# diff7/tts-king

Measured on AMD Instinct MI355X. Metric: FS2 train mel-frames/sec/GPU + HiFi-GAN RTF (22.05 kHz), batch=16, higher is better.
Workload: dtype bf16

## Files before the change

tts_king_amd/csrc/batchnorm.hip:

```cpp
#include "common.h"

namespace {

struct BnCommon {
  const void* x;
  const float* mean;
  const float* rstd;
  const float* gamma;
  const float* beta;
  const uint64_t* rng;
  int rows, C, use_tanh;
  float p;
  unsigned site;
  int x_f32;
  const int* frame_limit;
  int seg_len;
  uint8_t* keep;
  const long long* lens;
};
__device__ __forceinline__ float tanh_fast(float x) { return 1.f - 2.f * __frcp_rn(__expf(2.f * x) + 1.f); }
__device__ __forceinline__ bool bn_live(const int* frame_limit, int seg_len, int r) {
  return !frame_limit || (r % seg_len) < frame_limit[0];
}
__device__ __forceinline__ int bn_rows(const int* frame_limit, int seg_len, int rows) {
  return frame_limit ? (rows / seg_len) * frame_limit[0] : rows;
}

__device__ __forceinline__ void ld4(const bf16_t* p, float v[4]) {
  const uint2 u = *(const uint2*)p;
  v[0] = __uint_as_float(u.x << 16); v[1] = __uint_as_float(u.x & 0xFFFF0000u);
  v[2] = __uint_as_float(u.y << 16); v[3] = __uint_as_float(u.y & 0xFFFF0000u);
}
__device__ __forceinline__ void ldx4(const void* x, int x_f32, int64_t off, float v[4]) {
  if (x_f32) {
    const f32x4 t = *(const f32x4*)((const float*)x + off);
    v[0] = t[0]; v[1] = t[1]; v[2] = t[2]; v[3] = t[3];
  } else {
    ld4((const bf16_t*)x + off, v);
  }
}
__device__ __forceinline__ uint4 bits4(const uint64_t* rng, unsigned site, unsigned e4) {
  const uint64_t seed = rng[0], step = rng[1];
  return Philox::gen(make_uint2((unsigned)seed, (unsigned)(seed >> 32)), make_uint4(e4, site, (unsigned)step, (unsigned)(step >> 32)));
}

__global__ __launch_bounds__(256) void bn_stats_kernel(const void* __restrict__ x, int x_f32, int rows, int C, float* __restrict__ partials,
                                                       const int* __restrict__ frame_limit, int seg_len) {
  extern __shared__ float red[];
  const int tpr = C >> 2, rpi = 256 / tpr;
  const int r0 = threadIdx.x / tpr, c4 = (threadIdx.x % tpr) * 4;
  const int per = (rows + gridDim.x - 1) / gridDim.x;
  const int rb = blockIdx.x * per;
  const int re = min(rb + per, rows);
  float s[4] = {0, 0, 0, 0}, q[4] = {0, 0, 0, 0};
  if (r0 < rpi)
    for (int r = rb + r0; r < re; r += rpi) {
      if (!bn_live(frame_limit, seg_len, r)) continue;
      float v[4];
      ldx4(x, x_f32, (int64_t)r * C + c4, v);
#pragma unroll
      for (int e = 0; e < 4; ++e) { s[e] += v[e]; q[e] += v[e] * v[e]; }
    }
  if (r0 < rpi) {
#pragma unroll
    for (int e = 0; e < 4; ++e) { red[r0 * C + c4 + e] = s[e]; red[rpi * C + r0 * C + c4 + e] = q[e]; }
  }
  __syncthreads();
  for (int c = threadIdx.x; c < C; c += 256) {
    float a = 0.f, b = 0.f;
    for (int k = 0; k < rpi; ++k) { a += red[k * C + c]; b += red[rpi * C + k * C + c]; }
    partials[(int64_t)blockIdx.x * 2 * C + c] = a;
    partials[(int64_t)blockIdx.x * 2 * C + C + c] = b;
  }
}

__global__ __launch_bounds__(256) void bn_finalize_kernel(const float* __restrict__ partials, int nblk, int C, int rows_all, float eps,
                                                          float momentum, float* __restrict__ mean, float* __restrict__ rstd,
                                                          float* __restrict__ run_mean, float* __restrict__ run_var,
                                                          long long* __restrict__ nbt, const int* __restrict__ frame_limit, int seg_len) {
  const int rows = bn_rows(frame_limit, seg_len, rows_all);
  __shared__ double rs[16][17], rq[16][17];
  const int cx = threadIdx.x & 15, gy = threadIdx.x >> 4;
  const int c = blockIdx.x * 16 + cx;
  if (blockIdx.x == 0 && threadIdx.x == 0 && nbt) nbt[0] += 1;
  double s = 0.0, q = 0.0;
  if (c < C) {
    double s1 = 0.0, q1 = 0.0, s2 = 0.0, q2 = 0.0, s3 = 0.0, q3 = 0.0;
    int b = gy;
    for (; b + 48 < nblk; b += 64) {
      const float a0 = partials[(int64_t)b * 2 * C + c], b0 = partials[(int64_t)b * 2 * C + C + c];
      const float a1 = partials[(int64_t)(b + 16) * 2 * C + c], b1 = partials[(int64_t)(b + 16) * 2 * C + C + c];
      const float a2 = partials[(int64_t)(b + 32) * 2 * C + c], b2 = partials[(int64_t)(b + 32) * 2 * C + C + c];
      const float a3 = partials[(int64_t)(b + 48) * 2 * C + c], b3 = partials[(int64_t)(b + 48) * 2 * C + C + c];
      s += a0; q += b0; s1 += a1; q1 += b1; s2 += a2; q2 += b2; s3 += a3; q3 += b3;
    }
    for (; b < nblk; b += 16) { s += partials[(int64_t)b * 2 * C + c]; q += partials[(int64_t)b * 2 * C + C + c]; }
    s = (s + s1) + (s2 + s3);
    q = (q + q1) + (q2 + q3);
  }
  rs[gy][cx] = s;
  rq[gy][cx] = q;
  __syncthreads();
  if (gy != 0 || c >= C) return;
  s = 0.0; q = 0.0;
#pragma unroll
  for (int k = 0; k < 16; ++k) { s += rs[k][cx]; q += rq[k][cx]; }
  const double m = s / rows;
  double var = q / rows - m * m;
  if (var < 0.0) var = 0.0;
  mean[c] = (float)m;
  rstd[c] = (float)(1.0 / sqrt(var + (double)eps));
  if (run_mean) {
    run_mean[c] = (1.f - momentum) * run_mean[c] + momentum * (float)m;
    run_var[c] = (1.f - momentum) * run_var[c] + momentum * (float)(var * rows / (rows > 1 ? rows - 1 : 1));
  }
}

__global__ __launch_bounds__(256) void rsqrt_eps_kernel(const float* __restrict__ var, float eps, float* __restrict__ rstd, int n) {
  const int i = blockIdx.x * 256 + threadIdx.x;
  if (i < n) rstd[i] = 1.f / sqrtf(var[i] + eps);
}

template <bool LENS>
__global__ __launch_bounds__(256) void bn_apply_kernel(const BnCommon a, const float* __restrict__ resid, bf16_t* __restrict__ out16,
                                                       float* __restrict__ out32) {
  const int tpr = a.C >> 2;
  const int64_t n = (int64_t)a.rows * tpr;
  const unsigned thr = keep_threshold(a.p);
  const float scale = a.p > 0.f ? 1.f / (1.f - a.p) : 1.f;
  for (int64_t i = blockIdx.x * 256 + threadIdx.x; i < n; i += (int64_t)gridDim.x * 256) {
    const int r = (int)(i / tpr), c4 = (int)(i - (int64_t)r * tpr) * 4;
    bool live = bn_live(a.frame_limit, a.seg_len, r);
    if (LENS) {
      const int u = r / a.seg_len;
      const long long len = a.lens[u];
      live = live && (r - u * a.seg_len) < (len < 0 ? 0 : (len > a.seg_len ? (long long)a.seg_len : len));
    }
    if (!live) {
      if (out16) *(uint2*)(out16 + (int64_t)r * a.C + c4) = make_uint2(0u, 0u);
      if (out32) *(f32x4*)(out32 + (int64_t)r * a.C + c4) = f32x4{0.f, 0.f, 0.f, 0.f};
      continue;
    }
    float v[4];
    ldx4(a.x, a.x_f32, (int64_t)r * a.C + c4, v);
    const f32x4 m = *(const f32x4*)(a.mean + c4), rs = *(const f32x4*)(a.rstd + c4);
    const f32x4 g = *(const f32x4*)(a.gamma + c4), b = *(const f32x4*)(a.beta + c4);
#pragma unroll
    for (int e = 0; e < 4; ++e) {
      v[e] = (v[e] - m[e]) * rs[e] * g[e] + b[e];
      if (a.use_tanh) v[e] = tanh_fast(v[e]);
    }
    if (a.p > 0.f) {
      const uint4 bb = bits4(a.rng, a.site, (unsigned)i);
      v[0] = bb.x >= thr ? v[0] * scale : 0.f; v[1] = bb.y >= thr ? v[1] * scale : 0.f;
      v[2] = bb.z >= thr ? v[2] * scale : 0.f; v[3] = bb.w >= thr ? v[3] * scale : 0.f;
    }
    if (resid) {
      const f32x4 rr = *(const f32x4*)(resid + (int64_t)r * a.C + c4);
#pragma unroll
      for (int e = 0; e < 4; ++e) v[e] += rr[e];
    }
    if (out16) *(uint2*)(out16 + (int64_t)r * a.C + c4) = make_uint2(pack_bf2(v[0], v[1]), pack_bf2(v[2], v[3]));
    if (out32) *(f32x4*)(out32 + (int64_t)r * a.C + c4) = f32x4{v[0], v[1], v[2], v[3]};
  }
}

__device__ __forceinline__ void bn_dy(const BnCommon& a, const void* dout, int dout_f32, int r, int c4, int64_t i, unsigned thr,
                                      float scale, float xh[4], float dy[4]) {
  float v[4];
  ldx4(a.x, a.x_f32, (int64_t)r * a.C + c4, v);
  const f32x4 m = *(const f32x4*)(a.mean + c4), rs = *(const f32x4*)(a.rstd + c4);
  if (dout_f32) {
    const f32x4 d = *(const f32x4*)((const float*)dout + (int64_t)r * a.C + c4);
    dy[0] = d[0]; dy[1] = d[1]; dy[2] = d[2]; dy[3] = d[3];
  } else {
    ld4((const bf16_t*)dout + (int64_t)r * a.C + c4, dy);
  }
  if (a.p > 0.f) {
    if (a.keep) {
      const unsigned kb = a.keep[i];
#pragma unroll
      for (int e = 0; e < 4; ++e) dy[e] = ((kb >> e) & 1u) ? dy[e] * scale : 0.f;
    } else {
      const uint4 bb = bits4(a.rng, a.site, (unsigned)i);
      dy[0] = bb.x >= thr ? dy[0] * scale : 0.f; dy[1] = bb.y >= thr ? dy[1] * scale : 0.f;
      dy[2] = bb.z >= thr ? dy[2] * scale : 0.f; dy[3] = bb.w >= thr ? dy[3] * scale : 0.f;
    }
  }
#pragma unroll
  for (int e = 0; e < 4; ++e) xh[e] = (v[e] - m[e]) * rs[e];
  if (a.use_tanh) {
    const f32x4 g = *(const f32x4*)(a.gamma + c4), b = *(const f32x4*)(a.beta + c4);
#pragma unroll
    for (int e = 0; e < 4; ++e) { const float t = tanh_fast(xh[e] * g[e] + b[e]); dy[e] *= 1.f - t * t; }
  }
  if (!bn_live(a.frame_limit, a.seg_len, r)) {
#pragma unroll
    for (int e = 0; e < 4; ++e) { xh[e] = 0.f; dy[e] = 0.f; }
  }
}

__global__ __launch_bounds__(256) void bn_bwd_stats_kernel(const BnCommon a, const void* __restrict__ dout, int dout_f32,
                                                           float* __restrict__ partials) {
  extern __shared__ float red[];
  const int C = a.C, tpr = C >> 2, rpi = 256 / tpr;
  const int r0 = threadIdx.x / tpr, c4 = (threadIdx.x % tpr) * 4;
  const int per = (a.rows + gridDim.x - 1) / gridDim.x;
  const int rb = blockIdx.x * per;
  const int re = min(rb + per, a.rows);
  const unsigned thr = keep_threshold(a.p);
  const float scale = a.p > 0.f ? 1.f / (1.f - a.p) : 1.f;
  float s[4] = {0, 0, 0, 0}, q[4] = {0, 0, 0, 0};
  if (r0 < rpi)
    for (int r = rb + r0; r < re; r += rpi) {
      float xh[4], dy[4];
      bn_dy(a, dout, dout_f32, r, c4, (int64_t)r * tpr + (c4 >> 2), thr, scale, xh, dy);
#pragma unroll
      for (int e = 0; e < 4; ++e) { s[e] += dy[e]; q[e] += dy[e] * xh[e]; }
    }
  if (r0 < rpi) {
#pragma unroll
    for (int e = 0; e < 4; ++e) { red[r0 * C + c4 + e] = s[e]; red[rpi * C + r0 * C + c4 + e] = q[e]; }
  }
  __syncthreads();
  for (int c = threadIdx.x; c < C; c += 256) {
    float x1 = 0.f, x2 = 0.f;
    for (int k = 0; k < rpi; ++k) { x1 += red[k * C + c]; x2 += red[rpi * C + k * C + c]; }
    partials[(int64_t)blockIdx.x * 2 * C + c] = x1;
    partials[(int64_t)blockIdx.x * 2 * C + C + c] = x2;
  }
}

__global__ __launch_bounds__(256) void bn_bwd_apply_kernel(const BnCommon a, const void* __restrict__ dout, int dout_f32,
                                                           const float* __restrict__ sums, bf16_t* __restrict__ dx,
                                                           float* __restrict__ dgamma, float* __restrict__ dbeta, int accumulate) {
  const int tpr = a.C >> 2;
  const int64_t n = (int64_t)a.rows * tpr;
  const unsigned thr = keep_threshold(a.p);
  const float scale = a.p > 0.f ? 1.f / (1.f - a.p) : 1.f;
  const float inv_n = 1.f / bn_rows(a.frame_limit, a.seg_len, a.rows);
  if (blockIdx.x == 0 && dgamma)
    for (int c = threadIdx.x; c < a.C; c += 256) {
      dbeta[c] = accumulate ? dbeta[c] + sums[c] : sums[c];
      dgamma[c] = accumulate ? dgamma[c] + sums[a.C + c] : sums[a.C + c];
    }
  for (int64_t i = blockIdx.x * 256 + threadIdx.x; i < n; i += (int64_t)gridDim.x * 256) {
    const int r = (int)(i / tpr), c4 = (int)(i - (int64_t)r * tpr) * 4;
    float xh[4], dy[4];
    bn_dy(a, dout, dout_f32, r, c4, i, thr, scale, xh, dy);
    const f32x4 g = *(const f32x4*)(a.gamma + c4), rs = *(const f32x4*)(a.rstd + c4);
    const f32x4 s1 = *(const f32x4*)(sums + c4), s2 = *(const f32x4*)(sums + a.C + c4);
    float o[4];
#pragma unroll
    for (int e = 0; e < 4; ++e) o[e] = g[e] * rs[e] * (dy[e] - s1[e] * inv_n - xh[e] * s2[e] * inv_n);
    if (!bn_live(a.frame_limit, a.seg_len, r)) o[0] = o[1] = o[2] = o[3] = 0.f;
    *(uint2*)(dx + (int64_t)r * a.C + c4) = make_uint2(pack_bf2(o[0], o[1]), pack_bf2(o[2], o[3]));
  }
}


constexpr int BN_MAX_CHUNKS = 64;
__host__ __device__ inline int bn_slab(int C) { return (C % 64 == 0) ? 64 : C; }

struct BnSlab {
  int c0, slab, tpr, rpi, r_in, cq, rb, re;
  __device__ BnSlab(int C, int rows) {
    slab = bn_slab(C);
    c0 = blockIdx.x * slab;
    tpr = slab >> 2;
    rpi = 256 / tpr;
    r_in = threadIdx.x / tpr;
    cq = threadIdx.x % tpr;
    const int per = (rows + gridDim.y - 1) / gridDim.y;
    rb = blockIdx.y * per;
    re = min(rb + per, rows);
  }
};

__device__ __forceinline__ void bn_slab_store(const BnSlab& g, int C, const float s[4], const float q[4], float* red, float* partials) {
  if (g.r_in < g.rpi) {
#pragma unroll
    for (int e = 0; e < 4; ++e) { red[g.r_in * g.slab + g.cq * 4 + e] = s[e]; red[(g.rpi + g.r_in) * g.slab + g.cq * 4 + e] = q[e]; }
  }
  __syncthreads();
  for (int v = threadIdx.x; v < 2 * g.slab; v += 256) {
    const int half = v >= g.slab, c = v - half * g.slab;
    float acc = 0.f;
    for (int k = 0; k < g.rpi; ++k) acc += red[(half * g.rpi + k) * g.slab + c];
    partials[(int64_t)blockIdx.y * 2 * C + half * C + g.c0 + c] = acc;
  }
}

constexpr int BN_TOT = 256 + 1024;
__device__ __forceinline__ void bn_slab_totals(const float* __restrict__ partials, int nblk, int C, int c0, int slab, double* tot ) {
  const int nq = slab >> 1, groups = 256 / nq;
  const int t = threadIdx.x;
  if (t < groups * nq) {
    const int q = t % nq, g0 = t / nq;
    const int v0 = q * 4;
    const int col = v0 < slab ? c0 + v0 : C + c0 + (v0 - slab);
    double a[4] = {0.0, 0.0, 0.0, 0.0};
    for (int b = g0; b < nblk; b += 16 * groups) {
      f32x4 f[16];
#pragma unroll
      for (int u = 0; u < 16; ++u) {
        const int bb = b + u * groups;
        f[u] = *(const f32x4*)(partials + (int64_t)min(bb, nblk - 1) * 2 * C + col);
        if (bb >= nblk) f[u] = f32x4{0.f, 0.f, 0.f, 0.f};
      }
#pragma unroll
      for (int u = 0; u < 16; ++u)
#pragma unroll
        for (int e = 0; e < 4; ++e) a[e] += f[u][e];
    }
#pragma unroll
    for (int e = 0; e < 4; ++e) tot[256 + t * 4 + e] = a[e];
  }
  __syncthreads();
  if (t < 2 * slab) {
    double sum = 0.0;
    for (int k = 0; k < groups; ++k) sum += tot[256 + (k * nq + (t >> 2)) * 4 + (t & 3)];
    tot[t] = sum;
  }
  __syncthreads();
}

__global__ __launch_bounds__(256) void bn_stats2_kernel(const void* __restrict__ x, int x_f32, int rows, int C, float* __restrict__ partials,
                                                        const int* __restrict__ frame_limit, int seg_len) {
  extern __shared__ float red[];
  const BnSlab g(C, rows);
  const int c4 = g.c0 + g.cq * 4;
  float s[4] = {0, 0, 0, 0}, q[4] = {0, 0, 0, 0};
  if (g.r_in < g.rpi)
    for (int r0 = g.rb + g.r_in; r0 < g.re; r0 += 8 * g.rpi) {
      float v[8][4];
#pragma unroll
      for (int u = 0; u < 8; ++u) {
        const int r = r0 + u * g.rpi, rc = min(r, g.re - 1);
        ldx4(x, x_f32, (int64_t)rc * C + c4, v[u]);
        if (r >= g.re || !bn_live(frame_limit, seg_len, rc)) v[u][0] = v[u][1] = v[u][2] = v[u][3] = 0.f;
      }
#pragma unroll
      for (int u = 0; u < 8; ++u)
#pragma unroll
        for (int e = 0; e < 4; ++e) { s[e] += v[u][e]; q[e] += v[u][e] * v[u][e]; }
    }
  bn_slab_store(g, C, s, q, red, partials);
}

struct BnTrain {
  const float* partials;
  int nblk;
  float eps, momentum;
  float* mean;
  float* rstd;
  float* run_mean;
  float* run_var;
  long long* nbt;
};

template <bool RESID>
__global__ __launch_bounds__(256, RESID ? 3 : 4) void bn_apply2_kernel(const BnCommon a, const BnTrain t, const float* __restrict__ resid,
                                                        bf16_t* __restrict__ out16, float* __restrict__ out32) {
  __shared__ double tot[BN_TOT];
  __shared__ float ms[128], rs[128];
  const BnSlab g(a.C, a.rows);
  const int cl = g.cq * 4, c4 = g.c0 + cl, tprC = a.C >> 2;
  const bool act = g.r_in < g.rpi;
  float v[4][4], rr[RESID ? 4 : 1][4];
  bool live[4];
#pragma unroll
  for (int u = 0; u < 4; ++u) {
    const int r = g.rb + g.r_in + u * g.rpi, rc = max(min(r, g.re - 1), 0);
    live[u] = act && r < g.re && bn_live(a.frame_limit, a.seg_len, r);
    if (act) {
      ldx4(a.x, a.x_f32, (int64_t)rc * a.C + c4, v[u]);
      if constexpr (RESID) { const f32x4 q = *(const f32x4*)(resid + (int64_t)rc * a.C + c4); rr[u][0] = q[0]; rr[u][1] = q[1]; rr[u][2] = q[2]; rr[u][3] = q[3]; }
    }
  }
  f32x4 gm = f32x4{0.f, 0.f, 0.f, 0.f}, bt = gm;
  if (act) { gm = *(const f32x4*)(a.gamma + c4); bt = *(const f32x4*)(a.beta + c4); }
  bn_slab_totals(t.partials, t.nblk, a.C, g.c0, g.slab, tot);
  if ((int)threadIdx.x < g.slab) {
    const int c = threadIdx.x;
    const int n = bn_rows(a.frame_limit, a.seg_len, a.rows);
    const double m = tot[c] / n;
    double var = tot[g.slab + c] / n - m * m;
    if (var < 0.0) var = 0.0;
    ms[c] = (float)m;
    rs[c] = (float)(1.0 / sqrt(var + (double)t.eps));
    if (blockIdx.y == 0) {
      t.mean[g.c0 + c] = ms[c];
      t.rstd[g.c0 + c] = rs[c];
      if (t.run_mean) {
        t.run_mean[g.c0 + c] = (1.f - t.momentum) * t.run_mean[g.c0 + c] + t.momentum * (float)m;
        t.run_var[g.c0 + c] = (1.f - t.momentum) * t.run_var[g.c0 + c] + t.momentum * (float)(var * n / (n > 1 ? n - 1 : 1));
      }
      if (blockIdx.x == 0 && c == 0 && t.nbt) t.nbt[0] += 1;
    }
  }
  __syncthreads();
  if (!act) return;
  const unsigned thr = keep_threshold(a.p);
  const float scale = a.p > 0.f ? 1.f / (1.f - a.p) : 1.f;
#pragma unroll
  for (int u = 0; u < 4; ++u) {
    const int r = g.rb + g.r_in + u * g.rpi;
    if (r >= g.re) break;
    const int64_t i = (int64_t)r * tprC + (c4 >> 2);
    if (!live[u]) {
      if (out16) *(uint2*)(out16 + (int64_t)r * a.C + c4) = make_uint2(0u, 0u);
      if (out32) *(f32x4*)(out32 + (int64_t)r * a.C + c4) = f32x4{0.f, 0.f, 0.f, 0.f};
      if (a.keep) a.keep[i] = 0;
      continue;
    }
#pragma unroll
    for (int e = 0; e < 4; ++e) {
      v[u][e] = (v[u][e] - ms[cl + e]) * rs[cl + e] * gm[e] + bt[e];
      if (a.use_tanh) v[u][e] = tanh_fast(v[u][e]);
    }
    if (a.p > 0.f) {
      const uint4 bb = bits4(a.rng, a.site, (unsigned)i);
      const bool k0 = bb.x >= thr, k1 = bb.y >= thr, k2 = bb.z >= thr, k3 = bb.w >= thr;
      v[u][0] = k0 ? v[u][0] * scale : 0.f; v[u][1] = k1 ? v[u][1] * scale : 0.f;
      v[u][2] = k2 ? v[u][2] * scale : 0.f; v[u][3] = k3 ? v[u][3] * scale : 0.f;
      if (a.keep) a.keep[i] = (uint8_t)((int)k0 | ((int)k1 << 1) | ((int)k2 << 2) | ((int)k3 << 3));
    }
    if constexpr (RESID) {
#pragma unroll
      for (int e = 0; e < 4; ++e) v[u][e] += rr[u][e];
    }
    if (out16) *(uint2*)(out16 + (int64_t)r * a.C + c4) = make_uint2(pack_bf2(v[u][0], v[u][1]), pack_bf2(v[u][2], v[u][3]));
    if (out32) *(f32x4*)(out32 + (int64_t)r * a.C + c4) = f32x4{v[u][0], v[u][1], v[u][2], v[u][3]};
  }
}

__global__ __launch_bounds__(256) void bn_bwd_stats2_kernel(const BnCommon a, const void* __restrict__ dout, int dout_f32,
                                                            float* __restrict__ partials) {
  extern __shared__ float red[];
  const BnSlab g(a.C, a.rows);
  const int c4 = g.c0 + g.cq * 4, tprC = a.C >> 2;
  const unsigned thr = keep_threshold(a.p);
  const float scale = a.p > 0.f ? 1.f / (1.f - a.p) : 1.f;
  float s[4] = {0, 0, 0, 0}, q[4] = {0, 0, 0, 0};
  if (g.r_in < g.rpi)
    for (int r0 = g.rb + g.r_in; r0 < g.re; r0 += 8 * g.rpi) {
      float xh[8][4], dy[8][4];
#pragma unroll
      for (int u = 0; u < 8; ++u) {
        const int r = r0 + u * g.rpi, rc = min(r, g.re - 1);
        bn_dy(a, dout, dout_f32, rc, c4, (int64_t)rc * tprC + (c4 >> 2), thr, scale, xh[u], dy[u]);
        if (r >= g.re) { xh[u][0] = xh[u][1] = xh[u][2] = xh[u][3] = 0.f; dy[u][0] = dy[u][1] = dy[u][2] = dy[u][3] = 0.f; }
      }
#pragma unroll
      for (int u = 0; u < 8; ++u)
#pragma unroll
        for (int e = 0; e < 4; ++e) { s[e] += dy[u][e]; q[e] += dy[u][e] * xh[u][e]; }
    }
  bn_slab_store(g, a.C, s, q, red, partials);
}

__global__ __launch_bounds__(256, 4) void bn_bwd_apply2_kernel(const BnCommon a, const void* __restrict__ dout, int dout_f32,
                                                            const float* __restrict__ partials, int nblk, bf16_t* __restrict__ dx,
                                                            float* __restrict__ dgamma, float* __restrict__ dbeta, int accumulate) {
  __shared__ double tot[BN_TOT];
  __shared__ float s1s[128], s2s[128];
  const BnSlab g(a.C, a.rows);
  const int cl = g.cq * 4, c4 = g.c0 + cl, tprC = a.C >> 2;
  const bool act = g.r_in < g.rpi;
  const unsigned thr = keep_threshold(a.p);
  const float scale = a.p > 0.f ? 1.f / (1.f - a.p) : 1.f;
  float xh[4][4], dy[4][4];
#pragma unroll
  for (int u = 0; u < 4; ++u) {
    const int rc = max(min(g.rb + g.r_in + u * g.rpi, g.re - 1), 0);
    if (act) bn_dy(a, dout, dout_f32, rc, c4, (int64_t)rc * tprC + (c4 >> 2), thr, scale, xh[u], dy[u]);
  }
  bn_slab_totals(partials, nblk, a.C, g.c0, g.slab, tot);
  if ((int)threadIdx.x < g.slab) {
    const int c = threadIdx.x;
    s1s[c] = (float)tot[c];
    s2s[c] = (float)tot[g.slab + c];
    if (blockIdx.y == 0 && dgamma) {
      dbeta[g.c0 + c] = accumulate ? dbeta[g.c0 + c] + s1s[c] : s1s[c];
      dgamma[g.c0 + c] = accumulate ? dgamma[g.c0 + c] + s2s[c] : s2s[c];
    }
  }
  __syncthreads();
  if (!act) return;
  const float inv_n = 1.f / bn_rows(a.frame_limit, a.seg_len, a.rows);
  const f32x4 gm = *(const f32x4*)(a.gamma + c4), rsd = *(const f32x4*)(a.rstd + c4);
#pragma unroll
  for (int u = 0; u < 4; ++u) {
    const int r = g.rb + g.r_in + u * g.rpi;
    if (r >= g.re) break;
    float o[4];
#pragma unroll
    for (int e = 0; e < 4; ++e) o[e] = gm[e] * rsd[e] * (dy[u][e] - s1s[cl + e] * inv_n - xh[u][e] * s2s[cl + e] * inv_n);
    if (!bn_live(a.frame_limit, a.seg_len, r)) o[0] = o[1] = o[2] = o[3] = 0.f;
    *(uint2*)(dx + (int64_t)r * a.C + c4) = make_uint2(pack_bf2(o[0], o[1]), pack_bf2(o[2], o[3]));
  }
}

inline int bn_chunks(int rows) { int n = (rows + 15) / 16; return n > BN_MAX_CHUNKS ? BN_MAX_CHUNKS : (n < 1 ? 1 : n); }
inline int bn_apply_chunks(int rows, int C) { const int rpi = 256 / (bn_slab(C) >> 2); int n = (rows + 4 * rpi - 1) / (4 * rpi); return n < 1 ? 1 : n; }

inline int bn_blocks(int rows) { int n = (rows + 15) / 16; return n > 1024 ? 1024 : (n < 1 ? 1 : n); }

}

extern "C" int ttsk_bn_nblocks(int rows) { return bn_blocks(rows); }

static int bn_check(int rows, int C) {
  TTSK_REQUIRE(rows > 0 && C >= 4 && C <= 1024 && (C & 3) == 0, "batchnorm: C must be a multiple of 4, <= 1024 (got %d)", C);
  return 0;
}

static int limit_check(const int32_t* frame_limit, int seg_len, int rows) {
  TTSK_REQUIRE(!frame_limit || (seg_len > 0 && rows % seg_len == 0), "batchnorm: frame_limit needs rows %% seg_len == 0");
  return 0;
}

extern "C" int ttsk_bn_stats(const void* x, int x_is_f32, int rows, int C, float* partials, const int32_t* frame_limit, int seg_len,
                             void* stream) {
  TTSK_REQUIRE(x && partials, "bn_stats: null pointer");
  if (int rc = limit_check(frame_limit, seg_len, rows)) return rc;
  if (int rc = bn_check(rows, C)) return rc;
  const int rpi = 256 / (C >> 2);
  hipLaunchKernelGGL(bn_stats_kernel, dim3(bn_blocks(rows)), dim3(256), 2 * rpi * C * sizeof(float), (hipStream_t)stream,
                     x, x_is_f32, rows, C, partials, frame_limit, seg_len > 0 ? seg_len : 1);
  TTSK_CHECK_LAUNCH();
  return TTSK_OK;
}

extern "C" int ttsk_bn_finalize(const float* partials, int nblk, int C, int rows, float eps, float momentum, float* mean,
                                float* rstd, float* running_mean, float* running_var, int64_t* num_batches_tracked,
                                const int32_t* frame_limit, int seg_len, void* stream) {
  if (int rc = limit_check(frame_limit, seg_len, rows)) return rc;
  TTSK_REQUIRE(partials && mean && rstd && nblk > 0, "bn_finalize: null pointer");
  TTSK_REQUIRE((running_mean == nullptr) == (running_var == nullptr), "bn_finalize: running stats come in pairs");
  hipLaunchKernelGGL(bn_finalize_kernel, dim3((C + 15) / 16), dim3(256), 0, (hipStream_t)stream, partials, nblk, C, rows, eps,
                     momentum, mean, rstd, running_mean, running_var, (long long*)num_batches_tracked, frame_limit, seg_len > 0 ? seg_len : 1);
  TTSK_CHECK_LAUNCH();
  return TTSK_OK;
}

extern "C" int ttsk_rsqrt_eps(const float* var, float eps, float* rstd, int n, void* stream) {
  TTSK_REQUIRE(var && rstd && n > 0, "rsqrt_eps: bad arguments");
  hipLaunchKernelGGL(rsqrt_eps_kernel, dim3((n + 255) / 256), dim3(256), 0, (hipStream_t)stream, var, eps, rstd, n);
  TTSK_CHECK_LAUNCH();
  return TTSK_OK;
}

extern "C" int ttsk_bn_apply(const void* x, int x_is_f32, const float* mean, const float* rstd, const float* gamma, const float* beta,
                             int rows, int C, int use_tanh, float p, uint32_t site, const uint64_t* rng, const float* resid_f32,
                             void* out_bf16, float* out_f32, const int32_t* frame_limit, int seg_len, void* stream) {
  if (int rc = limit_check(frame_limit, seg_len, rows)) return rc;
  TTSK_REQUIRE(x && mean && rstd && gamma && beta && (out_bf16 || out_f32), "bn_apply: null pointer");
  TTSK_REQUIRE(p == 0.f || rng, "bn_apply: dropout needs rng");
  if (int rc = bn_check(rows, C)) return rc;
  BnCommon a{x, mean, rstd, gamma, beta, rng, rows, C, use_tanh, p, site, x_is_f32, frame_limit, seg_len > 0 ? seg_len : 1};
  int64_t n = (int64_t)rows * (C >> 2);
  int blocks = (int)((n + 255) / 256);
  if (blocks > 4096) blocks = 4096;
  hipLaunchKernelGGL(bn_apply_kernel<false>, dim3(blocks), dim3(256), 0, (hipStream_t)stream, a, resid_f32, (bf16_t*)out_bf16, out_f32);
  TTSK_CHECK_LAUNCH();
  return TTSK_OK;
}

extern "C" int ttsk_bn_apply_lens(const void* x, int x_is_f32, const float* mean, const float* rstd, const float* gamma, const float* beta,
                                  int rows, int C, int use_tanh, const float* resid_f32, void* out_bf16, float* out_f32,
                                  const int64_t* lens, int seg_len, void* stream) {
  TTSK_REQUIRE(x && mean && rstd && gamma && beta && lens && (out_bf16 || out_f32), "bn_apply_lens: null pointer");
  TTSK_REQUIRE(seg_len > 0 && rows % seg_len == 0, "bn_apply_lens: rows %% seg_len != 0");
  if (int rc = bn_check(rows, C)) return rc;
  BnCommon a{x, mean, rstd, gamma, beta, nullptr, rows, C, use_tanh, 0.f, 0u, x_is_f32, nullptr, seg_len, nullptr, (const long long*)lens};
  int64_t n = (int64_t)rows * (C >> 2);
  int blocks = (int)((n + 255) / 256);
  if (blocks > 4096) blocks = 4096;
  hipLaunchKernelGGL(bn_apply_kernel<true>, dim3(blocks), dim3(256), 0, (hipStream_t)stream, a, resid_f32, (bf16_t*)out_bf16, out_f32);
  TTSK_CHECK_LAUNCH();
  return TTSK_OK;
}

extern "C" int ttsk_bn_bwd_stats(const void* dout, int dout_is_f32, const void* x, int x_is_f32, const float* mean, const float* rstd,
                                 const float* gamma, const float* beta, int rows, int C, int use_tanh, float p, uint32_t site,
                                 const uint64_t* rng, float* partials, const int32_t* frame_limit, int seg_len, void* stream) {
  if (int rc = limit_check(frame_limit, seg_len, rows)) return rc;
  TTSK_REQUIRE(dout && x && mean && rstd && gamma && beta && partials, "bn_bwd_stats: null pointer");
  TTSK_REQUIRE(p == 0.f || rng, "bn_bwd_stats: dropout needs rng");
  if (int rc = bn_check(rows, C)) return rc;
  BnCommon a{x, mean, rstd, gamma, beta, rng, rows, C, use_tanh, p, site, x_is_f32, frame_limit, seg_len > 0 ? seg_len : 1};
  const int rpi = 256 / (C >> 2);
  hipLaunchKernelGGL(bn_bwd_stats_kernel, dim3(bn_blocks(rows)), dim3(256), 2 * rpi * C * sizeof(float), (hipStream_t)stream, a,
                     dout, dout_is_f32, partials);
  TTSK_CHECK_LAUNCH();
  return TTSK_OK;
}

extern "C" int ttsk_bn_bwd_apply(const void* dout, int dout_is_f32, const void* x, int x_is_f32, const float* mean, const float* rstd,
                                 const float* gamma, const float* beta, int rows, int C, int use_tanh, float p, uint32_t site,
                                 const uint64_t* rng, const float* sums, void* dx_bf16, float* dgamma, float* dbeta, int accumulate,
                                 const int32_t* frame_limit, int seg_len, void* stream) {
  if (int rc = limit_check(frame_limit, seg_len, rows)) return rc;
  TTSK_REQUIRE(dout && x && mean && rstd && gamma && beta && sums && dx_bf16, "bn_bwd_apply: null pointer");
  TTSK_REQUIRE((dgamma == nullptr) == (dbeta == nullptr), "bn_bwd_apply: dgamma/dbeta come in pairs");
  if (int rc = bn_check(rows, C)) return rc;
  BnCommon a{x, mean, rstd, gamma, beta, rng, rows, C, use_tanh, p, site, x_is_f32, frame_limit, seg_len > 0 ? seg_len : 1};
  int64_t n = (int64_t)rows * (C >> 2);
  int blocks = (int)((n + 255) / 256);
  if (blocks > 4096) blocks = 4096;
  hipLaunchKernelGGL(bn_bwd_apply_kernel, dim3(blocks), dim3(256), 0, (hipStream_t)stream, a, dout, dout_is_f32, sums,
                     (bf16_t*)dx_bf16, dgamma, dbeta, accumulate);
  TTSK_CHECK_LAUNCH();
  return TTSK_OK;
}

static int bn2_check(int rows, int C) {
  if (int rc = bn_check(rows, C)) return rc;
  TTSK_REQUIRE(C % 64 == 0 || C <= 128, "batchnorm (slab path): C must be a multiple of 64 or <= 128 (got %d)", C);
  return 0;
}

extern "C" int ttsk_bn_nchunks(int rows) { return bn_chunks(rows); }

extern "C" int ttsk_bn_stats_slab(const void* x, int x_is_f32, int rows, int C, float* partials, const int32_t* frame_limit, int seg_len,
                                  void* stream) {
  TTSK_REQUIRE(x && partials, "bn_stats_slab: null pointer");
  if (int rc = limit_check(frame_limit, seg_len, rows)) return rc;
  if (int rc = bn2_check(rows, C)) return rc;
  const int slab = bn_slab(C), rpi = 256 / (slab >> 2);
  hipLaunchKernelGGL(bn_stats2_kernel, dim3(C / slab, bn_chunks(rows)), dim3(256), 2 * rpi * slab * sizeof(float), (hipStream_t)stream,
                     x, x_is_f32, rows, C, partials, frame_limit, seg_len > 0 ? seg_len : 1);
  TTSK_CHECK_LAUNCH();
  return TTSK_OK;
}

extern "C" int ttsk_bn_train_apply(const void* x, int x_is_f32, const float* partials, int nblk, float eps, float momentum, float* mean,
                                   float* rstd, float* running_mean, float* running_var, int64_t* num_batches_tracked,
                                   const float* gamma, const float* beta, int rows, int C, int use_tanh, float p, uint32_t site,
                                   const uint64_t* rng, const float* resid_f32, void* out_bf16, float* out_f32, uint8_t* keep_out,
                                   const int32_t* frame_limit, int seg_len, void* stream) {
  if (int rc = limit_check(frame_limit, seg_len, rows)) return rc;
  TTSK_REQUIRE(x && partials && nblk > 0 && mean && rstd && gamma && beta && (out_bf16 || out_f32), "bn_train_apply: null pointer");
  TTSK_REQUIRE((running_mean == nullptr) == (running_var == nullptr), "bn_train_apply: running stats come in pairs");
  TTSK_REQUIRE(p == 0.f || rng, "bn_train_apply: dropout needs rng");
  if (int rc = bn2_check(rows, C)) return rc;
  BnCommon a{x, nullptr, nullptr, gamma, beta, rng, rows, C, use_tanh, p, site, x_is_f32, frame_limit, seg_len > 0 ? seg_len : 1, keep_out};
  BnTrain t{partials, nblk, eps, momentum, mean, rstd, running_mean, running_var, (long long*)num_batches_tracked};
  const dim3 grid(C / bn_slab(C), bn_apply_chunks(rows, C));
  if (resid_f32) hipLaunchKernelGGL(bn_apply2_kernel<true>, grid, dim3(256), 0, (hipStream_t)stream, a, t, resid_f32, (bf16_t*)out_bf16, out_f32);
  else hipLaunchKernelGGL(bn_apply2_kernel<false>, grid, dim3(256), 0, (hipStream_t)stream, a, t, resid_f32, (bf16_t*)out_bf16, out_f32);
  TTSK_CHECK_LAUNCH();
  return TTSK_OK;
}

extern "C" int ttsk_bn_bwd_stats_slab(const void* dout, int dout_is_f32, const void* x, int x_is_f32, const float* mean, const float* rstd,
                                      const float* gamma, const float* beta, int rows, int C, int use_tanh, float p, uint32_t site,
                                      const uint64_t* rng, const uint8_t* keep, float* partials, const int32_t* frame_limit, int seg_len,
                                      void* stream) {
  if (int rc = limit_check(frame_limit, seg_len, rows)) return rc;
  TTSK_REQUIRE(dout && x && mean && rstd && gamma && beta && partials, "bn_bwd_stats_slab: null pointer");
  TTSK_REQUIRE(p == 0.f || rng || keep, "bn_bwd_stats_slab: dropout needs rng or the forward's keep bits");
  if (int rc = bn2_check(rows, C)) return rc;
  BnCommon a{x, mean, rstd, gamma, beta, rng, rows, C, use_tanh, p, site, x_is_f32, frame_limit, seg_len > 0 ? seg_len : 1, (uint8_t*)keep};
  const int slab = bn_slab(C), rpi = 256 / (slab >> 2);
  hipLaunchKernelGGL(bn_bwd_stats2_kernel, dim3(C / slab, bn_chunks(rows)), dim3(256), 2 * rpi * slab * sizeof(float), (hipStream_t)stream,
                     a, dout, dout_is_f32, partials);
  TTSK_CHECK_LAUNCH();
  return TTSK_OK;
}

extern "C" int ttsk_bn_bwd_apply_slab(const void* dout, int dout_is_f32, const void* x, int x_is_f32, const float* mean, const float* rstd,
                                      const float* gamma, const float* beta, int rows, int C, int use_tanh, float p, uint32_t site,
                                      const uint64_t* rng, const uint8_t* keep, const float* partials, int nblk, void* dx_bf16, float* dgamma,
                                      float* dbeta, int accumulate, const int32_t* frame_limit, int seg_len, void* stream) {
  if (int rc = limit_check(frame_limit, seg_len, rows)) return rc;
  TTSK_REQUIRE(dout && x && mean && rstd && gamma && beta && partials && nblk > 0 && dx_bf16, "bn_bwd_apply_slab: null pointer");
  TTSK_REQUIRE((dgamma == nullptr) == (dbeta == nullptr), "bn_bwd_apply_slab: dgamma/dbeta come in pairs");
  TTSK_REQUIRE(p == 0.f || rng || keep, "bn_bwd_apply_slab: dropout needs rng or the forward's keep bits");
  if (int rc = bn2_check(rows, C)) return rc;
  BnCommon a{x, mean, rstd, gamma, beta, rng, rows, C, use_tanh, p, site, x_is_f32, frame_limit, seg_len > 0 ? seg_len : 1, (uint8_t*)keep};
  hipLaunchKernelGGL(bn_bwd_apply2_kernel, dim3(C / bn_slab(C), bn_apply_chunks(rows, C)), dim3(256), 0, (hipStream_t)stream, a, dout,
                     dout_is_f32, partials, nblk, (bf16_t*)dx_bf16, dgamma, dbeta, accumulate);
  TTSK_CHECK_LAUNCH();
  return TTSK_OK;
}
```

tts_king_amd/csrc/common.h:

```cpp
#pragma once
#include <hip/hip_runtime.h>
#include <stdint.h>
#include <stdio.h>
#include <stdarg.h>
#include "../../include/ttsk.h"

typedef unsigned short bf16_t;
typedef __attribute__((ext_vector_type(8))) short bf16x8;
typedef __attribute__((ext_vector_type(4))) short bf16x4;
typedef __attribute__((ext_vector_type(4))) float f32x4;

__device__ __forceinline__ float bf2f(bf16_t v) { return __uint_as_float(((unsigned)v) << 16); }
__device__ __forceinline__ bf16_t f2bf(float f) {
  __bf16 b = (__bf16)f;
  return *reinterpret_cast<bf16_t*>(&b);
}
__device__ __forceinline__ unsigned pack_bf2(float a, float b) {
  return (unsigned)f2bf(a) | ((unsigned)f2bf(b) << 16);
}
template <int CTRL>
__device__ __forceinline__ float dpp_f32(float v) {
  return __builtin_bit_cast(float, __builtin_amdgcn_update_dpp(0, __builtin_bit_cast(int, v), CTRL, 0xF, 0xF, true));
}
__device__ __forceinline__ float quad16_max(float v) {
  v = fmaxf(v, dpp_f32<0xB1>(v));
  v = fmaxf(v, dpp_f32<0x4E>(v));
  v = fmaxf(v, dpp_f32<0x141>(v));
  v = fmaxf(v, dpp_f32<0x140>(v));
  return v;
}
__device__ __forceinline__ float quad16_sum(float v) {
  v += dpp_f32<0xB1>(v);
  v += dpp_f32<0x4E>(v);
  v += dpp_f32<0x141>(v);
  v += dpp_f32<0x140>(v);
  return v;
}

__device__ __forceinline__ float wave_sum(float v) {
  v = quad16_sum(v);
  v += __shfl_xor(v, 16, 64);
  v += __shfl_xor(v, 32, 64);
  return v;
}
__device__ __forceinline__ float wave_max(float v) {
  v = quad16_max(v);
  v = fmaxf(v, __shfl_xor(v, 16, 64));
  v = fmaxf(v, __shfl_xor(v, 32, 64));
  return v;
}

typedef _Float16 half8 __attribute__((ext_vector_type(8)));
typedef _Float16 half2v __attribute__((ext_vector_type(2)));
template <bool F16> __device__ __forceinline__ void unpack2(unsigned w, float& lo, float& hi) {
  if constexpr (F16) {
    const half2v h = __builtin_bit_cast(half2v, w);
    lo = (float)h[0]; hi = (float)h[1];
  } else {
    lo = __uint_as_float(w << 16); hi = __uint_as_float(w & 0xFFFF0000u);
  }
}
template <bool F16> __device__ __forceinline__ unsigned pack2(float lo, float hi) {
  if constexpr (F16) {
    half2v h; h[0] = (_Float16)lo; h[1] = (_Float16)hi;
    return __builtin_bit_cast(unsigned, h);
  } else {
    return pack_bf2(lo, hi);
  }
}
template <bool F16> __device__ __forceinline__ float unpack1(bf16_t v) {
  if constexpr (F16) return (float)__builtin_bit_cast(_Float16, v);
  else return bf2f(v);
}
template <bool F16> __device__ __forceinline__ bf16_t pack1(float f) {
  if constexpr (F16) return __builtin_bit_cast(bf16_t, (_Float16)f);
  else return f2bf(f);
}
template <bool F16> __device__ __forceinline__ unsigned lrelu2(unsigned w, float sl) {
  float lo, hi;
  unpack2<F16>(w, lo, hi);
  lo = lo > 0.f ? lo : lo * sl;
  hi = hi > 0.f ? hi : hi * sl;
  return pack2<F16>(lo, hi);
}
template <bool F16> __device__ __forceinline__ uint4 lrelu8(uint4 v, float sl) {
  return make_uint4(lrelu2<F16>(v.x, sl), lrelu2<F16>(v.y, sl), lrelu2<F16>(v.z, sl), lrelu2<F16>(v.w, sl));
}
template <bool F16> __device__ __forceinline__ unsigned lrelu2_fast(unsigned w, float sl) {
  if constexpr (F16) {
    float lo, hi;
    asm("v_fma_mix_f32 %0, %1, %2, 0 op_sel_hi:[1,0,0]" : "=v"(lo) : "v"(w), "v"(sl));
    asm("v_fma_mix_f32 %0, %1, %2, 0 op_sel:[1,0,0] op_sel_hi:[1,0,0]" : "=v"(hi) : "v"(w), "v"(sl));
    const unsigned p = pack2<true>(lo, hi);
    unsigned r;
    asm("v_pk_max_f16 %0, %1, %2" : "=v"(r) : "v"(w), "v"(p));
    return r;
  } else {
    return lrelu2<false>(w, sl);
  }
}

template <bool F16> __device__ __forceinline__ uint4 lrelu8_fast(uint4 v, float sl) {
  return make_uint4(lrelu2_fast<F16>(v.x, sl), lrelu2_fast<F16>(v.y, sl), lrelu2_fast<F16>(v.z, sl), lrelu2_fast<F16>(v.w, sl));
}
template <bool F16> __device__ __forceinline__ f32x4 mfma16(bf16x8 a, bf16x8 b, f32x4 c) {
  if constexpr (F16) return __builtin_amdgcn_mfma_f32_16x16x32_f16(__builtin_bit_cast(half8, a), __builtin_bit_cast(half8, b), c, 0, 0, 0);
  else return __builtin_amdgcn_mfma_f32_16x16x32_bf16(a, b, c, 0, 0, 0);
}

struct Philox {
  __device__ static __forceinline__ uint4 gen(uint2 key, uint4 ctr) {
#pragma unroll
    for (int r = 0; r < 10; ++r) {
      unsigned hi0 = __umulhi(0xD2511F53u, ctr.x), lo0 = 0xD2511F53u * ctr.x;
      unsigned hi1 = __umulhi(0xCD9E8D57u, ctr.z), lo1 = 0xCD9E8D57u * ctr.z;
      ctr = make_uint4(hi1 ^ ctr.y ^ key.x, lo1, hi0 ^ ctr.w ^ key.y, lo0);
      key.x += 0x9E3779B9u;
      key.y += 0xBB67AE85u;
    }
    return ctr;
  }
};
__device__ __forceinline__ uint4 dropout_bits(uint64_t seed, unsigned site, unsigned e4) {
  return Philox::gen(make_uint2((unsigned)seed, (unsigned)(seed >> 32)), make_uint4(e4, site, 0x5eedu, 0u));
}
__device__ __forceinline__ unsigned keep_threshold(float p) {
  double t = (double)p * 4294967296.0;
  return t >= 4294967295.0 ? 0xFFFFFFFFu : (unsigned)t;
}

void ttsk_set_error(const char* fmt, ...);
#define TTSK_REQUIRE(cond, ...)                 \
  do {                                          \
    if (!(cond)) {                              \
      ttsk_set_error(__VA_ARGS__);              \
      return TTSK_EINVAL;                       \
    }                                           \
  } while (0)
#define TTSK_CHECK_LAUNCH()                                                    \
  do {                                                                         \
    hipError_t e__ = hipGetLastError();                                        \
    if (e__ != hipSuccess) {                                                   \
      ttsk_set_error("%s: launch failed: %s", __func__, hipGetErrorString(e__)); \
      return TTSK_ELAUNCH;                                                     \
    }                                                                          \
  } while (0)
```

tts_king_amd/csrc/cwt.hip:

```cpp
#include "common.h"
#include <math.h>

namespace {

constexpr int NH = TTSK_CWT_CHANNELS;
constexpr int NBIN = TTSK_CNNSCALAR_BINS;
constexpr int O_W1 = 0, O_B1 = 256, O_G1 = 264, O_BE1 = 296, O_W2 = 328, O_B2 = 344, O_G2 = 352, O_BE2 = 384, O_LW = 416, O_LB = 448;
static_assert(O_LB + 8 == TTSK_CNNSCALAR_FLOATS, "CNNscalar block layout");

__device__ __forceinline__ void load4(const bf16_t* p, float v[4]) {
  const uint2 u = *(const uint2*)p;
  v[0] = __uint_as_float(u.x << 16); v[1] = __uint_as_float(u.x & 0xFFFF0000u);
  v[2] = __uint_as_float(u.y << 16); v[3] = __uint_as_float(u.y & 0xFFFF0000u);
}
__device__ __forceinline__ void store4(bf16_t* p, const float v[4]) {
  *(uint2*)p = make_uint2(pack_bf2(v[0], v[1]), pack_bf2(v[2], v[3]));
}
__device__ __forceinline__ void drop4(float v[4], uint64_t seed, uint64_t step, unsigned site, unsigned e4, unsigned thr, float scale) {
  const uint4 b = Philox::gen(make_uint2((unsigned)seed, (unsigned)(seed >> 32)),
                              make_uint4(e4, site, (unsigned)step, (unsigned)(step >> 32)));
  v[0] = b.x >= thr ? v[0] * scale : 0.f;
  v[1] = b.y >= thr ? v[1] * scale : 0.f;
  v[2] = b.z >= thr ? v[2] * scale : 0.f;
  v[3] = b.w >= thr ? v[3] * scale : 0.f;
}

struct HeadArgs {
  const bf16_t* y;
  const float* gamma; const float* beta;
  const long long* lens;
  const uint64_t* rng;
  const float* head_w;
  const float* head_b;
  float* mean; float* rstd;
  float* head_out;
  int rows, seg_len;
  float p_post, eps;
  unsigned site_post;
};

__global__ __launch_bounds__(256) void ln_head_fwd_kernel(const HeadArgs a) {
  const int lane = threadIdx.x & 63;
  const int row = blockIdx.x * 4 + (threadIdx.x >> 6);
  if (row >= a.rows) return;
  constexpr int D = 256;
  const uint64_t seed = a.rng ? a.rng[0] : 0, step = a.rng ? a.rng[1] : 0;
  const int c = lane * 4;
  float z[4];
  load4(a.y + (int64_t)row * D + c, z);
  const float mean = wave_sum(z[0] + z[1] + z[2] + z[3]) / D;
  float q = 0.f;
#pragma unroll
  for (int e = 0; e < 4; ++e) { const float d = z[e] - mean; q += d * d; }
  const float rstd = rsqrtf(wave_sum(q) / D + a.eps);
  if (lane == 0) { a.mean[row] = mean; a.rstd[row] = rstd; }
  const int b = row / a.seg_len, t = row - b * a.seg_len;
  const bool masked = t >= a.lens[b];
  const f32x4 g = *(const f32x4*)(a.gamma + c), bt = *(const f32x4*)(a.beta + c);
  float o[4];
#pragma unroll
  for (int e = 0; e < 4; ++e) o[e] = (z[e] - mean) * rstd * g[e] + bt[e];
  if (a.p_post > 0.f)
    drop4(o, seed, step, a.site_post, (unsigned)(((int64_t)row * D + c) >> 2), keep_threshold(a.p_post), 1.f / (1.f - a.p_post));
#pragma unroll
  for (int k = 0; k < NH; ++k) {
    const f32x4 w = *(const f32x4*)(a.head_w + k * D + c);
    const float hs = wave_sum(o[0] * w[0] + o[1] * w[1] + o[2] * w[2] + o[3] * w[3]);
    if (lane == 0) a.head_out[(int64_t)row * NH + k] = masked ? 0.f : hs + a.head_b[k];
  }
}

struct HeadBwdArgs {
  const float* dhead;
  const float* head_w;
  const bf16_t* z;
  const float* mean; const float* rstd;
  const float* gamma; const float* beta;
  const long long* lens;
  const uint64_t* rng;
  bf16_t* dz;
  float* partials;
  int rows, seg_len;
  float p_post;
  unsigned site_post;
};

constexpr int HB_WAVES = 4;
constexpr int HB_NCOL = (3 + NH) * 256 + NH;

__global__ __launch_bounds__(HB_WAVES * 64) void ln_head_bwd_kernel(const HeadBwdArgs a) {
  __shared__ float red[HB_WAVES][256];
  __shared__ float redb[HB_WAVES][NH];
  constexpr int D = 256;
  const int lane = threadIdx.x & 63, wave = threadIdx.x >> 6;
  const uint64_t seed = a.rng ? a.rng[0] : 0, step = a.rng ? a.rng[1] : 0;
  const int c = lane * 4;
  float dg[4] = {0, 0, 0, 0}, db[4] = {0, 0, 0, 0}, dbias[4] = {0, 0, 0, 0};
  float dhw[NH][4];
  float dhb[NH];
#pragma unroll
  for (int k = 0; k < NH; ++k) { dhb[k] = 0.f; dhw[k][0] = dhw[k][1] = dhw[k][2] = dhw[k][3] = 0.f; }
  const f32x4 gm = *(const f32x4*)(a.gamma + c), bt = *(const f32x4*)(a.beta + c);
  for (int row = blockIdx.x * HB_WAVES + wave; row < a.rows; row += gridDim.x * HB_WAVES) {
    const int b = row / a.seg_len, t = row - b * a.seg_len;
    const bool masked = t >= a.lens[b];
    const float mean = a.mean[row], rstd = a.rstd[row];
    float zz[4];
    load4(a.z + (int64_t)row * D + c, zz);
    float xh[4], o[4], d[4] = {0, 0, 0, 0};
#pragma unroll
    for (int e = 0; e < 4; ++e) { xh[e] = (zz[e] - mean) * rstd; o[e] = xh[e] * gm[e] + bt[e]; }
    if (a.p_post > 0.f)
      drop4(o, seed, step, a.site_post, (unsigned)(((int64_t)row * D + c) >> 2), keep_threshold(a.p_post), 1.f / (1.f - a.p_post));
#pragma unroll
    for (int k = 0; k < NH; ++k) {
      const float dh = masked ? 0.f : a.dhead[(int64_t)row * NH + k];
      const f32x4 w = *(const f32x4*)(a.head_w + k * D + c);
#pragma unroll
      for (int e = 0; e < 4; ++e) { d[e] += dh * w[e]; dhw[k][e] += dh * o[e]; }
      dhb[k] += dh;
    }
    if (a.p_post > 0.f)
      drop4(d, seed, step, a.site_post, (unsigned)(((int64_t)row * D + c) >> 2), keep_threshold(a.p_post), 1.f / (1.f - a.p_post));
    float g[4], c1 = 0.f, c2 = 0.f;
#pragma unroll
    for (int e = 0; e < 4; ++e) {
      dg[e] += d[e] * xh[e];
      db[e] += d[e];
      g[e] = d[e] * gm[e];
      c1 += g[e];
      c2 += g[e] * xh[e];
    }
    c1 = wave_sum(c1) / D;
    c2 = wave_sum(c2) / D;
    float dzv[4];
#pragma unroll
    for (int e = 0; e < 4; ++e) {
      dzv[e] = zz[e] > 0.f ? rstd * (g[e] - c1 - xh[e] * c2) : 0.f;
      dbias[e] += dzv[e];
    }
    store4(a.dz + (int64_t)row * D + c, dzv);
  }
  float* P = a.partials + (int64_t)blockIdx.x * HB_NCOL;
  for (int qn = 0; qn < 3 + NH; ++qn) {
#pragma unroll
    for (int e = 0; e < 4; ++e) {
      float v;
      if (qn == 0) v = dbias[e];
      else if (qn == 1) v = dg[e];
      else if (qn == 2) v = db[e];
      else {
        v = 0.f;
#pragma unroll
        for (int k = 0; k < NH; ++k) if (qn == 3 + k) v = dhw[k][e];
      }
      red[wave][c + e] = v;
    }
    __syncthreads();
    {
      const int cc = threadIdx.x;
      float t = 0.f;
#pragma unroll
      for (int w = 0; w < HB_WAVES; ++w) t += red[w][cc];
      P[qn * D + cc] = t;
    }
    __syncthreads();
  }
  if (lane == 0) {
#pragma unroll
    for (int k = 0; k < NH; ++k) redb[wave][k] = dhb[k];
  }
  __syncthreads();
  if (threadIdx.x < NH) {
    float t = 0.f;
#pragma unroll
    for (int w = 0; w < HB_WAVES; ++w) t += redb[w][threadIdx.x];
    P[(3 + NH) * D + threadIdx.x] = t;
  }
}

__device__ __forceinline__ int bin_start(int i, int L) { return (int)(((int64_t)i * L) / NBIN); }
__device__ __forceinline__ int bin_end(int i, int L) { return (int)((((int64_t)(i + 1)) * L + NBIN - 1) / NBIN); }

struct CnnArgs {
  const bf16_t* x;
  const float* cwt;
  const float* params;
  float* rowdot;
  float* pooled;
  float* stats;
  float* pre;
  float* out;
  const float* dout;
  float* partials;
  int B, L;
};

__global__ __launch_bounds__(256) void cnn_heads_fwd_kernel(const CnnArgs a) {
  __shared__ float sp[4][NBIN];
  const int b = blockIdx.x, L = a.L;
  const int lane = threadIdx.x & 63, wave = threadIdx.x >> 6;
  const float* P0 = a.params;
  const float* P1 = a.params + TTSK_CNNSCALAR_FLOATS;
  float* rd = a.rowdot + (int64_t)b * 4 * L;
  const int c = lane * 4;
  const f32x4 w0 = *(const f32x4*)(P0 + O_W1 + c), w1 = *(const f32x4*)(P1 + O_W1 + c);
  for (int l = wave; l < L; l += 4) {
    float v[4];
    load4(a.x + ((int64_t)b * L + l) * 256 + c, v);
    const float s0 = wave_sum(v[0] * w0[0] + v[1] * w0[1] + v[2] * w0[2] + v[3] * w0[3]);
    const float s1 = wave_sum(v[0] * w1[0] + v[1] * w1[1] + v[2] * w1[2] + v[3] * w1[3]);
    if (lane == 0) { rd[0 * L + l] = s0 + P0[O_B1]; rd[2 * L + l] = s1 + P1[O_B1]; }
  }
  for (int l = threadIdx.x; l < L; l += 256) {
    const float* cr = a.cwt + ((int64_t)b * L + l) * NH;
    float s0 = 0.f, s1 = 0.f;
#pragma unroll
    for (int k = 0; k < NH; ++k) { const float v = cr[k]; s0 += v * P0[O_W2 + k]; s1 += v * P1[O_W2 + k]; }
    rd[1 * L + l] = s0 + P0[O_B2]; rd[3 * L + l] = s1 + P1[O_B2];
  }
  __syncthreads();
  if (threadIdx.x < 4 * NBIN) {
    const int q = threadIdx.x / NBIN, i = threadIdx.x - q * NBIN;
    const int s = bin_start(i, L), e = bin_end(i, L);
    float t = 0.f;
    for (int l = s; l < e; ++l) t += rd[q * L + l];
    t /= (float)(e - s);
    sp[q][i] = t;
    a.pooled[((int64_t)b * 4 + q) * NBIN + i] = t;
  }
  __syncthreads();
  {
    const int q = wave;
    const float* Pq = (q >> 1) ? P1 : P0;
    const int og = (q & 1) ? O_G2 : O_G1, ob = (q & 1) ? O_BE2 : O_BE1;
    const float v = lane < NBIN ? sp[q][lane] : 0.f;
    const float mean = wave_sum(v) / NBIN;
    const float d = lane < NBIN ? v - mean : 0.f;
    const float rstd = rsqrtf(wave_sum(d * d) / NBIN + 1e-5f);
    __syncthreads();
    if (lane < NBIN) sp[q][lane] = fmaxf(d * rstd * Pq[og + lane] + Pq[ob + lane], 0.f);
    if (lane == 0) { a.stats[((int64_t)b * 4 + q) * 2] = mean; a.stats[((int64_t)b * 4 + q) * 2 + 1] = rstd; }
  }
  __syncthreads();
  if (wave < 2) {
    const int h = wave;
    const float* Ph = h ? P1 : P0;
    const float v = lane < NBIN ? (sp[2 * h][lane] + sp[2 * h + 1][lane]) * Ph[O_LW + lane] : 0.f;
    const float pre = wave_sum(v) + Ph[O_LB];
    if (lane == 0) { a.pre[b * 2 + h] = pre; a.out[h * a.B + b] = fmaxf(pre, 0.f); }
  }
}

__global__ __launch_bounds__(256) void cnn_heads_bwd_kernel(const CnnArgs a) {
  __shared__ float dp[4][NBIN];
  __shared__ float red[4][2][256];
  __shared__ float red2[2][NH + 1][4];
  const int b = blockIdx.x, L = a.L;
  const int lane = threadIdx.x & 63, wave = threadIdx.x >> 6;
  const float* P0 = a.params;
  const float* P1 = a.params + TTSK_CNNSCALAR_FLOATS;
  float* part = a.partials + (int64_t)b * 2 * TTSK_CNNSCALAR_FLOATS;
  float* rd = a.rowdot + (int64_t)b * 4 * L;
  for (int i = threadIdx.x; i < 2 * TTSK_CNNSCALAR_FLOATS; i += 256) part[i] = 0.f;
  __syncthreads();
  {
    const int q = wave, h = q >> 1, f = q & 1;
    const float* Ph = h ? P1 : P0;
    float* ph = part + h * TTSK_CNNSCALAR_FLOATS;
    const int og = f ? O_G2 : O_G1, ob = f ? O_BE2 : O_BE1;
    const float pre = a.pre[b * 2 + h];
    const float dpre = pre > 0.f ? a.dout[h * a.B + b] : 0.f;
    const float mean = a.stats[((int64_t)b * 4 + q) * 2], rstd = a.stats[((int64_t)b * 4 + q) * 2 + 1];
    const bool on = lane < NBIN;
    const float p = on ? a.pooled[((int64_t)b * 4 + q) * NBIN + lane] : 0.f;
    const float gam = on ? Ph[og + lane] : 0.f, bet = on ? Ph[ob + lane] : 0.f;
    const float xh = on ? (p - mean) * rstd : 0.f;
    const float y = xh * gam + bet;
    const float dy = (on && y > 0.f) ? dpre * Ph[O_LW + lane] : 0.f;
    const float gx = dy * gam;
    const float c1 = wave_sum(gx) / NBIN, c2 = wave_sum(gx * xh) / NBIN;
    if (on) {
      ph[og + lane] = dy * xh;
      ph[ob + lane] = dy;
      const int cnt = bin_end(lane, L) - bin_start(lane, L);
      dp[q][lane] = rstd * (gx - c1 - xh * c2) / (float)cnt;
    }
    if (f == 0) {
      const int q2 = q + 1;
      const float m2 = a.stats[((int64_t)b * 4 + q2) * 2], r2 = a.stats[((int64_t)b * 4 + q2) * 2 + 1];
      const float p2 = on ? a.pooled[((int64_t)b * 4 + q2) * NBIN + lane] : 0.f;
      const float y2 = on ? (p2 - m2) * r2 * Ph[O_G2 + lane] + Ph[O_BE2 + lane] : 0.f;
      if (on) ph[O_LW + lane] = dpre * (fmaxf(y, 0.f) + fmaxf(y2, 0.f));
      if (lane == 0) ph[O_LB] = dpre;
    }
  }
  __syncthreads();
  for (int l = threadIdx.x; l < L; l += 256) {
    float t[4] = {0.f, 0.f, 0.f, 0.f};
    for (int i = 0; i < NBIN; ++i)
      if (l >= bin_start(i, L) && l < bin_end(i, L)) {
#pragma unroll
        for (int q = 0; q < 4; ++q) t[q] += dp[q][i];
      }
#pragma unroll
    for (int q = 0; q < 4; ++q) rd[q * L + l] = t[q];
  }
  __syncthreads();
  {
    const int c = lane * 4;
    float acc0[4] = {0, 0, 0, 0}, acc1[4] = {0, 0, 0, 0};
    for (int l = wave; l < L; l += 4) {
      float v[4];
      load4(a.x + ((int64_t)b * L + l) * 256 + c, v);
      const float d0 = rd[0 * L + l], d1 = rd[2 * L + l];
#pragma unroll
      for (int e = 0; e < 4; ++e) { acc0[e] += d0 * v[e]; acc1[e] += d1 * v[e]; }
    }
#pragma unroll
    for (int e = 0; e < 4; ++e) { red[wave][0][c + e] = acc0[e]; red[wave][1][c + e] = acc1[e]; }
    if (lane <= NH) {
      float s0 = 0.f, s1 = 0.f, t0 = 0.f, t1 = 0.f;
      for (int l = wave; l < L; l += 4) {
        const float d0 = rd[1 * L + l], d1 = rd[3 * L + l];
        if (lane < NH) {
          const float v = a.cwt[((int64_t)b * L + l) * NH + lane];
          s0 += d0 * v; s1 += d1 * v;
        } else {
          s0 += d0; s1 += d1; t0 += rd[0 * L + l]; t1 += rd[2 * L + l];
        }
      }
      red2[0][lane][wave] = s0; red2[1][lane][wave] = s1;
      if (lane == NH) { dp[0][wave] = t0; dp[1][wave] = t1; }
    }
  }
  __syncthreads();
  {
    const int cc = threadIdx.x;
#pragma unroll
    for (int h = 0; h < 2; ++h)
      part[h * TTSK_CNNSCALAR_FLOATS + O_W1 + cc] = red[0][h][cc] + red[1][h][cc] + red[2][h][cc] + red[3][h][cc];
    if (cc < 2 * (NH + 1)) {
      const int h = cc / (NH + 1), k = cc - h * (NH + 1);
      const float t = red2[h][k][0] + red2[h][k][1] + red2[h][k][2] + red2[h][k][3];
      part[h * TTSK_CNNSCALAR_FLOATS + (k < NH ? O_W2 + k : O_B2)] = t;
    }
    if (cc < 2) part[cc * TTSK_CNNSCALAR_FLOATS + O_B1] = dp[cc][0] + dp[cc][1] + dp[cc][2] + dp[cc][3];
  }
}

struct CwtW { double w[10]; };

__device__ __forceinline__ double cwt_sum(const float* __restrict__ c, const CwtW& w) {
  double s = 0.0;
#pragma unroll
  for (int i = 0; i < 10; ++i) s += (double)c[i] * w.w[i];
  return s;
}

__device__ __forceinline__ void cwt_pitch_row(double s, double m, double sd, int b, int l, const float* __restrict__ heads, const float* __restrict__ bins,
                                              int nb, float p_control, float* __restrict__ pitch, int* __restrict__ idx, int B, int L) {
  const double z = (s - m) / sd;
  const float p = (float)(z * (double)heads[B + b] + (double)heads[b]);
  pitch[(int64_t)b * L + l] = p;
  const float x = p * p_control;
  int lo = 0, hi = nb;
  while (lo < hi) { const int mid = (lo + hi) >> 1; if (bins[mid] < x) lo = mid + 1; else hi = mid; }
  idx[(int64_t)b * L + l] = (x != x) ? nb : lo;
}

constexpr int CP_WAVES = 8, CP_MAXB = 64;
__global__ __launch_bounds__(64 * CP_WAVES) void cwt_pitch_lds_kernel(const float* __restrict__ cwt, const float* __restrict__ heads,
                                                                      const float* __restrict__ bins, int nb, float p_control,
                                                                      float* __restrict__ pitch, int* __restrict__ idx, int B, int L, const CwtW w) {
  __shared__ double sdat[CP_MAXB][64];
  const int lane = threadIdx.x & 63, wave = threadIdx.x >> 6;
  const int l = blockIdx.x * 64 + lane;
  const bool on = l < L;
  for (int b = wave; b < B; b += CP_WAVES) sdat[b][lane] = on ? cwt_sum(cwt + ((int64_t)b * L + l) * NH, w) : 0.0;
  __syncthreads();
  if (!on) return;
  double m = 0.0;
  for (int b = 0; b < B; ++b) m += sdat[b][lane];
  m /= (double)B;
  double v = 0.0;
  for (int b = 0; b < B; ++b) { const double d = sdat[b][lane] - m; v += d * d; }
  const double sd = sqrt(v / (double)B) + 1e-12;
  for (int b = wave; b < B; b += CP_WAVES) cwt_pitch_row(sdat[b][lane], m, sd, b, l, heads, bins, nb, p_control, pitch, idx, B, L);
}

__global__ __launch_bounds__(64) void cwt_pitch_kernel(const float* __restrict__ cwt, const float* __restrict__ heads, const float* __restrict__ bins,
                                                       int nb, float p_control, float* __restrict__ pitch, int* __restrict__ idx, int B, int L,
                                                       const CwtW w) {
  const int l = blockIdx.x * 64 + threadIdx.x;
  if (l >= L) return;
  double m = 0.0;
  for (int b = 0; b < B; ++b) m += cwt_sum(cwt + ((int64_t)b * L + l) * NH, w);
  m /= (double)B;
  double v = 0.0;
  for (int b = 0; b < B; ++b) { const double d = cwt_sum(cwt + ((int64_t)b * L + l) * NH, w) - m; v += d * d; }
  const double sd = sqrt(v / (double)B) + 1e-12;
  for (int b = 0; b < B; ++b)
    cwt_pitch_row(cwt_sum(cwt + ((int64_t)b * L + l) * NH, w), m, sd, b, l, heads, bins, nb, p_control, pitch, idx, B, L);
}

constexpr int CL_WAVES = 16;
__global__ __launch_bounds__(64 * CL_WAVES) void cwt_loss_kernel(const float* __restrict__ cwt, const float* __restrict__ cwt_t,
                                                                 const float* __restrict__ heads, const float* __restrict__ mean_t,
                                                                 const float* __restrict__ std_t, const long long* __restrict__ src_lens, int B, int L,
                                                                 float grad_scale, float* __restrict__ dcwt, float* __restrict__ dheads,
                                                                 float* __restrict__ losses) {
  __shared__ double red[3][CL_WAVES];
  const int lane = threadIdx.x & 63, wave = threadIdx.x >> 6;
  float nv = 0.f;
  for (int b = 0; b < B; ++b) nv += (float)src_lens[b];
  const float gv = grad_scale * 2.f / (nv * NH);
  const float gh = grad_scale * 2.f / (float)B;
  float acc = 0.f, am = 0.f, as = 0.f;
  const int rows = B * L;
  for (int r = threadIdx.x; r < rows; r += 64 * CL_WAVES) {
    const int b = r / L, l = r - b * L;
    const bool ok = l < src_lens[b];
    const float* c = cwt + (int64_t)r * NH;
    const float* t = cwt_t + (int64_t)r * NH;
    float* g = dcwt + (int64_t)r * NH;
#pragma unroll
// ... 103 lines not shown
```

tts_king_amd/csrc/gemm_ln.hip:

```cpp
#include "gemm_common.h"
#include "proj32.h"
#include "tapring.h"

namespace {

constexpr int BM = 32, BN = 256, BK = 64, NSTAGE = 4;
constexpr int A_BYTES = BM * BK * 2;
constexpr int B_BYTES = BN * BK * 2;
constexpr int STAGE = A_BYTES + B_BYTES;
constexpr int CS_LD = 260;
constexpr int SMEM = NSTAGE * STAGE;
constexpr int OOB = 0x7FFFFFFF;
constexpr int WL_SPLIT_MAX_TILES = 64;

struct GemmLnArgs {
  const bf16_t* A;
  const bf16_t* W;
  const float* bias;
  const bf16_t* res;
  const float* gamma;
  const float* beta;
  bf16_t* out;
  bf16_t* z_save;
  float* mean;
  float* rstd;
  const long long* lens;
  const uint64_t* rng;
  int M, K, lda, ldw, seg_len;
  float p_pre, eps;
  unsigned site_pre;
  const bf16_t* pw;
  const float* pbias;
  bf16_t* pout;
  int pCout;
#ifdef TTSK_STAMPS
  unsigned long long* stamps;
#endif
};
#ifdef TTSK_STAMPS
#define WL_STAMP(i)                                                                                              \
  do {                                                                                                           \
    if (a.stamps && threadIdx.x == 0) a.stamps[(int64_t)blockIdx.x * 8 + (i)] = __builtin_amdgcn_s_memrealtime(); \
  } while (0)
#else
#define WL_STAMP(i) do {} while (0)
#endif

__device__ __forceinline__ void drop4(float v[4], uint64_t seed, uint64_t step, unsigned site, unsigned e4, unsigned thr, float scale) {
  const uint4 b = Philox::gen(make_uint2((unsigned)seed, (unsigned)(seed >> 32)),
                              make_uint4(e4, site, (unsigned)step, (unsigned)(step >> 32)));
  v[0] = b.x >= thr ? v[0] * scale : 0.f;
  v[1] = b.y >= thr ? v[1] * scale : 0.f;
  v[2] = b.z >= thr ? v[2] * scale : 0.f;
  v[3] = b.w >= thr ? v[3] * scale : 0.f;
}

template <int RW>
__device__ __forceinline__ void ln_rows_epilogue(const GemmLnArgs& a, const float* cs, int m0, int wave, int lane, const uint2 (&resv)[RW],
                                                 unsigned char* xs2 = nullptr, bool write = true ) {
  const int M = a.M, c = lane * 4;
  const uint64_t seed = a.rng ? a.rng[0] : 0, step = a.rng ? a.rng[1] : 0;
  const f32x4 bi = *(const f32x4*)(a.bias + c);
  const f32x4 g = *(const f32x4*)(a.gamma + c), bt = *(const f32x4*)(a.beta + c);
  const unsigned thr = keep_threshold(a.p_pre);
  const float scale = 1.f / (1.f - a.p_pre);
  float z[RW][4];
  float s[RW];
#pragma unroll
  for (int rr = 0; rr < RW; ++rr) {
    const int lr = wave * RW + rr;
    const int row = m0 + lr;
    const bool live = row < M;
    const f32x4 v = *(const f32x4*)(cs + lr * CS_LD + c);
#pragma unroll
    for (int e = 0; e < 4; ++e) z[rr][e] = v[e] + bi[e];
    if (a.p_pre > 0.f) drop4(z[rr], seed, step, a.site_pre, (unsigned)(((int64_t)row * BN + c) >> 2), thr, scale);
    z[rr][0] += __uint_as_float(resv[rr].x << 16); z[rr][1] += __uint_as_float(resv[rr].x & 0xFFFF0000u);
    z[rr][2] += __uint_as_float(resv[rr].y << 16); z[rr][3] += __uint_as_float(resv[rr].y & 0xFFFF0000u);
    if (a.z_save && live && write) *(uint2*)(a.z_save + (int64_t)row * BN + c) = make_uint2(pack_bf2(z[rr][0], z[rr][1]), pack_bf2(z[rr][2], z[rr][3]));
    s[rr] = z[rr][0] + z[rr][1] + z[rr][2] + z[rr][3];
  }
#pragma unroll
  for (int rr = 0; rr < RW; ++rr) s[rr] = wave_sum(s[rr]);
  float q[RW];
#pragma unroll
  for (int rr = 0; rr < RW; ++rr) {
    s[rr] *= (1.f / BN);
    q[rr] = 0.f;
#pragma unroll
    for (int e = 0; e < 4; ++e) { const float d = z[rr][e] - s[rr]; q[rr] += d * d; }
  }
#pragma unroll
  for (int rr = 0; rr < RW; ++rr) q[rr] = wave_sum(q[rr]);
#pragma unroll
  for (int rr = 0; rr < RW; ++rr) {
    const int row = m0 + wave * RW + rr;
    if (row >= M) {
      if (xs2) *(uint2*)(xs2 + (wave * RW + rr) * P32_RS + c * 2) = make_uint2(0u, 0u);
      continue;
    }
    const float mean = s[rr], rstd = rsqrtf(q[rr] * (1.f / BN) + a.eps);
    if (lane == 0 && write) { a.mean[row] = mean; a.rstd[row] = rstd; }
    bool masked = false;
    if (a.lens) { const int b = row / a.seg_len, t = row - b * a.seg_len; masked = t >= a.lens[b]; }
    float o4[4];
#pragma unroll
    for (int e = 0; e < 4; ++e) o4[e] = masked ? 0.f : (z[rr][e] - mean) * rstd * g[e] + bt[e];
    const uint2 ov = make_uint2(pack_bf2(o4[0], o4[1]), pack_bf2(o4[2], o4[3]));
    if (write) *(uint2*)(a.out + (int64_t)row * BN + c) = ov;
    if (xs2) *(uint2*)(xs2 + (wave * RW + rr) * P32_RS + c * 2) = ov;
  }
}

template <int NW, bool STAGGER>
__global__ __launch_bounds__(NW * 64, 1) void gemm_ln_kernel(const GemmLnArgs a) {
  constexpr int WC = BN / NW;
  constexpr int NJ = WC / 16;
  constexpr int NBP = 32 / NW;
  constexpr int RW = BM / NW;
  __shared__ __attribute__((aligned(16))) unsigned char smem[SMEM];
  const int tid = threadIdx.x, lane = tid & 63, wave = tid >> 6;
  const int l15 = lane & 15, lg = lane >> 4;
  const int m0 = blockIdx.x * BM;
  const int M = a.M, K = a.K;
  const int K8 = (K + 7) & ~7;
  const __amdgpu_buffer_rsrc_t rsA = __builtin_amdgcn_make_buffer_rsrc((void*)a.A, 0, 0x7FFFFFF0, 0x00020000);
  const __amdgpu_buffer_rsrc_t rsW = __builtin_amdgcn_make_buffer_rsrc((void*)a.W, 0, 0x7FFFFFF0, 0x00020000);
  const int nk = (K + BK - 1) / BK;
  const int c = lane * 4;

  uint2 resv[RW];
#pragma unroll
  for (int rr = 0; rr < RW; ++rr) {
    const int row = m0 + wave * RW + rr;
    resv[rr] = (a.res && row < M) ? *(const uint2*)(a.res + (int64_t)row * BN + c) : make_uint2(0u, 0u);
  }

  const int prow = lane >> 3, kch = ((lane & 7) ^ (lane >> 3)) * 8;
  const int a_row = m0 + (wave & 3) * 8 + prow;
  const int a_off = a_row < M ? (a_row * a.lda + kch) * 2 : OOB;
  int w_off[NBP];
#pragma unroll
  for (int i = 0; i < NBP; ++i) w_off[i] = (((i * NW + wave) * 8 + prow) * a.ldw + kch) * 2;
  const unsigned lds0 = __builtin_amdgcn_readfirstlane((unsigned)(uintptr_t)(lds_ptr)smem + wave * 1024);
  const bool has_a = wave < 4;
  const int kshift = STAGGER ? (int)((blockIdx.x * 5u) % (unsigned)nk) : 0;

  auto issue_tile = [&](int kt) __attribute__((always_inline)) {
    const unsigned st = lds0 + (kt % NSTAGE) * STAGE;
    int kk = kt + kshift;
    if (kk >= nk) kk -= nk;
    const int kbase = kk * BK;
    const bool kok = kbase + kch < K8;
    if (has_a) dma16(rsA, st, (kok && a_off != OOB) ? a_off + kbase * 2 : OOB);
#pragma unroll
    for (int i = 0; i < NBP; ++i) dma16(rsW, st + A_BYTES + i * (NW * 1024), kok ? w_off[i] + kbase * 2 : OOB);
  };

  f32x4 acc[2][NJ];
#pragma unroll
  for (int i = 0; i < 2; ++i)
#pragma unroll
    for (int j = 0; j < NJ; ++j) acc[i][j] = f32x4{0.f, 0.f, 0.f, 0.f};

#pragma unroll
  for (int t = 0; t < NSTAGE - 1; ++t)
    if (t < nk) issue_tile(t);

  for (int kt = 0; kt < nk; ++kt) {
    const int younger = nk - 1 - kt;
    if (younger >= 2) {
      if (has_a) asm volatile("s_waitcnt vmcnt(%0)" ::"n"(2 * (NBP + 1)) : "memory");
      else asm volatile("s_waitcnt vmcnt(%0)" ::"n"(2 * NBP) : "memory");
    } else if (younger == 1) {
      if (has_a) asm volatile("s_waitcnt vmcnt(%0)" ::"n"(NBP + 1) : "memory");
      else asm volatile("s_waitcnt vmcnt(%0)" ::"n"(NBP) : "memory");
    } else asm volatile("s_waitcnt vmcnt(0)" ::: "memory");
    __builtin_amdgcn_s_barrier();
    if (kt + NSTAGE - 1 < nk) issue_tile(kt + NSTAGE - 1);
    const unsigned char* sa = smem + (kt % NSTAGE) * STAGE;
    const unsigned char* sb = sa + A_BYTES;
#pragma unroll
    for (int ks = 0; ks < 2; ++ks) {
      bf16x8 af[2], bfr[NJ];
#pragma unroll
      for (int i = 0; i < 2; ++i) {
        const int row = i * 16 + l15;
        af[i] = *(const bf16x8*)(sa + row * 128 + (((ks * 4 + lg) ^ (row & 7)) << 4));
      }
#pragma unroll
      for (int j = 0; j < NJ; ++j) {
        const int row = wave * WC + j * 16 + l15;
        bfr[j] = *(const bf16x8*)(sb + row * 128 + (((ks * 4 + lg) ^ (row & 7)) << 4));
      }
#pragma unroll
      for (int i = 0; i < 2; ++i)
#pragma unroll
        for (int j = 0; j < NJ; ++j) acc[i][j] = __builtin_amdgcn_mfma_f32_16x16x32_bf16(af[i], bfr[j], acc[i][j], 0, 0, 0);
    }
  }
  __syncthreads();

  float* cs = (float*)smem;
#pragma unroll
  for (int i = 0; i < 2; ++i)
#pragma unroll
    for (int j = 0; j < NJ; ++j)
#pragma unroll
      for (int r = 0; r < 4; ++r) cs[(i * 16 + lg * 4 + r) * CS_LD + wave * WC + j * 16 + l15] = acc[i][j][r];
  __syncthreads();

  ln_rows_epilogue<RW>(a, cs, m0, wave, lane, resv);
}


template <int CIN, bool PROJ, int SPLIT = 1>
__global__ __launch_bounds__(512, (CIN == 256 && !PROJ) ? 2 : 1) void win_ln_kernel(const GemmLnArgs a) {
  constexpr int TT = BM, RS = CIN * 2 + 32, NT = 512, CH8 = CIN / 8, KH = 4, CT = 2, NF = TT / 16, NS = CIN / 128, RW = BM / 8;
  constexpr int XBYTES = TT * RS, CBYTES = BM * CS_LD * 4;
  static_assert(BM == P32_TT && BN == P32_D && NT == P32_NT, "proj32.h tile");
  __shared__ __attribute__((aligned(16))) unsigned char smem[XBYTES > CBYTES ? XBYTES : CBYTES];
  __shared__ __attribute__((aligned(16))) unsigned char ptile[PROJ ? 2 * P32_TT * P32_RS : 16];
  const int tid = threadIdx.x, lane = tid & 63, wave = tid >> 6;
  const int l15 = lane & 15, q = lane >> 4;
  const int part = SPLIT > 1 ? (int)blockIdx.x % SPLIT : 0;
  const int m0 = (SPLIT > 1 ? (int)blockIdx.x / SPLIT : (int)blockIdx.x) * BM;
  const int M = a.M;
  WL_STAMP(0);
  const __amdgpu_buffer_rsrc_t wres = weights_rsrc(a.W, CIN * BN * 2);
  const int wlane = (wave * CT) * 1024 + lane * 16;
  constexpr int kstep_bytes = (BN / 16) * 1024;
  bf16x8 wa[KH][CT], wb[KH][CT], wc[KH][CT];
  auto load_w = [&](int g, bf16x8 (&w)[KH][CT]) __attribute__((always_inline)) { frags_load<KH, CT>(w, wres, wlane, g * KH * kstep_bytes, kstep_bytes); };
  uint2 resv[RW];
  {
    constexpr int NCH = (TT * CH8 + NT - 1) / NT;
    uint4 xv[NCH];
#pragma unroll
    for (int it = 0; it < NCH; ++it) {
      const int idx = it * NT + tid;
      const int row = idx / CH8, ch = idx - row * CH8;
      xv[it] = make_uint4(0, 0, 0, 0);
      if (idx < TT * CH8 && m0 + row < M) xv[it] = *(const uint4*)(a.A + (int64_t)(m0 + row) * a.lda + ch * 8);
    }
    load_w(0, wa);
    if (1 < NS) load_w(1, wb);
    if (2 < NS) load_w(2, wc);
#pragma unroll
    for (int rr = 0; rr < RW; ++rr) {
      const int row = m0 + wave * RW + rr;
      resv[rr] = (a.res && row < M) ? *(const uint2*)(a.res + (int64_t)row * BN + lane * 4) : make_uint2(0u, 0u);
    }
#pragma unroll
    for (int it = 0; it < NCH; ++it) {
      const int idx = it * NT + tid;
      const int row = idx / CH8, ch = idx - row * CH8;
      if (idx < TT * CH8) *(uint4*)(smem + row * RS + ch * 16) = xv[it];
    }
  }
  WL_STAMP(1);
  __syncthreads();
  WL_STAMP(2);
  f32x4 acc[CT][NF];
#pragma unroll
  for (int cc = 0; cc < CT; ++cc)
#pragma unroll
    for (int i = 0; i < NF; ++i) acc[cc][i] = f32x4{0.f, 0.f, 0.f, 0.f};
  {
    const int inl = l15 * RS + q * 16;
    bf16x8 ring[KH][NF];
    ring_prime_step<NF, RS, KH>(ring, smem, inl);
    auto step = [&](int g, const bf16x8 (&w)[KH][CT]) __attribute__((always_inline)) {
      tap_ring_step<false, KH, CT, NF, RS>(acc, ring, w, smem, inl + (g + 1 < NS ? g + 1 : g) * (KH * 64));
    };
#pragma unroll
    for (int g = 0; g < NS; g += 3) {
      step(g, wa);
      __builtin_amdgcn_sched_barrier(0);
      if (g + 3 < NS) load_w(g + 3, wa);
      __builtin_amdgcn_sched_barrier(0);
      if (g + 1 < NS) {
        step(g + 1, wb);
        __builtin_amdgcn_sched_barrier(0);
        if (g + 4 < NS) load_w(g + 4, wb);
        __builtin_amdgcn_sched_barrier(0);
      }
      if (g + 2 < NS) {
        step(g + 2, wc);
        __builtin_amdgcn_sched_barrier(0);
        if (g + 5 < NS) load_w(g + 5, wc);
        __builtin_amdgcn_sched_barrier(0);
      }
    }
  }
  WL_STAMP(3);
  Proj32W PW;
  if (PROJ) proj32_prefetch(a.pw, a.pCout, wave, lane, PW, part * (3 / SPLIT));
  __syncthreads();
  WL_STAMP(4);
  float* cs = (float*)smem;
#pragma unroll
  for (int i = 0; i < NF; ++i)
#pragma unroll
    for (int cc = 0; cc < CT; ++cc) *(f32x4*)(cs + (i * 16 + l15) * CS_LD + (wave * CT + cc) * 16 + q * 4) = acc[cc][i];
  __syncthreads();
  ln_rows_epilogue<RW>(a, cs, m0, wave, lane, resv, PROJ ? ptile : nullptr, part == 0);
  WL_STAMP(5);
  if (PROJ) {
    __syncthreads();
    proj32_run<3 / SPLIT>(ptile, ptile + P32_TT * P32_RS, a.pw, a.pCout, a.pbias, PW, tid, [&](int cg, int rr, int ch, uint4 v, int) __attribute__((always_inline)) {
      if (m0 + rr < M) *(uint4*)(a.pout + (int64_t)(m0 + rr) * a.pCout + cg * BN + ch * 8) = v;
    }, Proj32NoPre(), part * (3 / SPLIT));
  }
  WL_STAMP(6);
}

}

#ifdef TTSK_STAMPS
static unsigned long long* g_wl_stamps = nullptr;
extern "C" int ttsk_win_ln_set_stamps(void* dev_buffer) {
  g_wl_stamps = (unsigned long long*)dev_buffer;
  return TTSK_OK;
}
#endif

extern "C" int ttsk_gemm_ln_fwd(const void* A, int lda, const void* W, int ldw, const float* bias, const void* res,
                                const float* gamma, const float* beta, void* out, void* z_save, float* mean, float* rstd,
                                const int64_t* lens, int seg_len, int M, int K, int D, float eps, float p_pre, uint32_t site_pre,
                                const void* rng, void* stream) {
  TTSK_REQUIRE(A && W && bias && gamma && beta && out && mean && rstd, "ttsk_gemm_ln_fwd: null pointer");
  TTSK_REQUIRE(D == BN, "ttsk_gemm_ln_fwd: the fused kernel is built for D = 256 (got %d); use ttsk_gemm + ttsk_layernorm_fwd", D);
  TTSK_REQUIRE(M > 0 && K > 0 && (K & 7) == 0 && (lda & 7) == 0 && (ldw & 7) == 0, "ttsk_gemm_ln_fwd: K, lda, ldw must be multiples of 8");
  TTSK_REQUIRE((((uintptr_t)A | (uintptr_t)W | (uintptr_t)out | (uintptr_t)res | (uintptr_t)z_save) & 15) == 0, "ttsk_gemm_ln_fwd: operands must be 16-byte aligned");
  TTSK_REQUIRE(((int64_t)M * lda + K) * 2 < ((int64_t)1 << 31) && ((int64_t)BN * ldw + K) * 2 < ((int64_t)1 << 31), "ttsk_gemm_ln_fwd: operand extent exceeds 2 GiB");
  TTSK_REQUIRE(!(p_pre > 0.f) || rng, "ttsk_gemm_ln_fwd: dropout needs the rng state");
  TTSK_REQUIRE(p_pre >= 0.f && p_pre < 1.f, "ttsk_gemm_ln_fwd: p_pre must be in [0, 1)");
  TTSK_REQUIRE(!lens || (seg_len > 0 && M % seg_len == 0), "ttsk_gemm_ln_fwd: lens needs M %% seg_len == 0");
  GemmLnArgs a{(const bf16_t*)A, (const bf16_t*)W, bias, (const bf16_t*)res, gamma, beta, (bf16_t*)out, (bf16_t*)z_save, mean, rstd,
               (const long long*)lens, (const uint64_t*)rng, M, K, lda, ldw, seg_len > 0 ? seg_len : 1, p_pre, eps, site_pre};
  hipLaunchKernelGGL((gemm_ln_kernel<8, true>), dim3((M + BM - 1) / BM), dim3(512), 0, (hipStream_t)stream, a);
  TTSK_CHECK_LAUNCH();
  return TTSK_OK;
}

extern "C" int ttsk_win_ln_supported(int K, int D) { return D == BN && (K == 256 || K == 1024); }

static int win_ln_launch(const void* A, int lda, const void* W_packed, const float* bias, const void* res, const float* gamma,
                         const float* beta, void* out, void* z_save, float* mean, float* rstd, const int64_t* lens, int seg_len, int M,
                         int K, int D, float eps, float p_pre, uint32_t site_pre, const void* rng, const void* proj_w, const float* proj_bias,
                         int proj_Cout, void* proj_out, void* stream) {
  TTSK_REQUIRE(A && W_packed && bias && gamma && beta && out && mean && rstd, "ttsk_win_ln_fwd: null pointer");
  TTSK_REQUIRE(ttsk_win_ln_supported(K, D), "ttsk_win_ln_fwd: built for D = 256, K = 256 or 1024 (got K=%d D=%d)", K, D);
  TTSK_REQUIRE(M > 0 && (lda & 7) == 0 && lda >= K, "ttsk_win_ln_fwd: bad M / lda");
  TTSK_REQUIRE((((uintptr_t)A | (uintptr_t)W_packed | (uintptr_t)out | (uintptr_t)res | (uintptr_t)z_save) & 15) == 0, "ttsk_win_ln_fwd: operands must be 16-byte aligned");
  TTSK_REQUIRE(!(p_pre > 0.f) || rng, "ttsk_win_ln_fwd: dropout needs the rng state");
  TTSK_REQUIRE(p_pre >= 0.f && p_pre < 1.f, "ttsk_win_ln_fwd: p_pre must be in [0, 1)");
  TTSK_REQUIRE(!lens || (seg_len > 0 && M % seg_len == 0), "ttsk_win_ln_fwd: lens needs M %% seg_len == 0");
  TTSK_REQUIRE(!proj_w || (proj_out && proj_Cout == 768 && (((uintptr_t)proj_w | (uintptr_t)proj_out | (uintptr_t)proj_bias) & 15) == 0),
               "ttsk_win_ln_proj_fwd: the projection is built for 768 output channels (q|k|v), 16-byte aligned operands");
  GemmLnArgs a{(const bf16_t*)A, (const bf16_t*)W_packed, bias, (const bf16_t*)res, gamma, beta, (bf16_t*)out, (bf16_t*)z_save, mean, rstd,
               (const long long*)lens, (const uint64_t*)rng, M, K, lda, 0, seg_len > 0 ? seg_len : 1, p_pre, eps, site_pre,
               (const bf16_t*)proj_w, proj_bias, (bf16_t*)proj_out, proj_Cout};
#ifdef TTSK_STAMPS
  a.stamps = g_wl_stamps;
#endif
  const dim3 grid((M + BM - 1) / BM);
  if (proj_w) {
    if (K == 256) hipLaunchKernelGGL((win_ln_kernel<256, true>), grid, dim3(512), 0, (hipStream_t)stream, a);
    else if (grid.x <= WL_SPLIT_MAX_TILES) hipLaunchKernelGGL((win_ln_kernel<1024, true, 3>), dim3(grid.x * 3), dim3(512), 0, (hipStream_t)stream, a);
    else hipLaunchKernelGGL((win_ln_kernel<1024, true>), grid, dim3(512), 0, (hipStream_t)stream, a);
  } else {
    if (K == 256) hipLaunchKernelGGL((win_ln_kernel<256, false>), grid, dim3(512), 0, (hipStream_t)stream, a);
    else hipLaunchKernelGGL((win_ln_kernel<1024, false>), grid, dim3(512), 0, (hipStream_t)stream, a);
  }
  TTSK_CHECK_LAUNCH();
  return TTSK_OK;
}

extern "C" int ttsk_win_ln_fwd(const void* A, int lda, const void* W_packed, const float* bias, const void* res, const float* gamma,
                               const float* beta, void* out, void* z_save, float* mean, float* rstd, const int64_t* lens, int seg_len, int M,
                               int K, int D, float eps, float p_pre, uint32_t site_pre, const void* rng, void* stream) {
  return win_ln_launch(A, lda, W_packed, bias, res, gamma, beta, out, z_save, mean, rstd, lens, seg_len, M, K, D, eps, p_pre, site_pre, rng,
                       nullptr, nullptr, 0, nullptr, stream);
}

extern "C" int ttsk_win_ln_proj_fwd(const void* A, int lda, const void* W_packed, const float* bias, const void* res, const float* gamma,
                                    const float* beta, void* out, void* z_save, float* mean, float* rstd, const int64_t* lens, int seg_len,
                                    int M, int K, int D, float eps, float p_pre, uint32_t site_pre, const void* rng, const void* proj_w_packed,
                                    const float* proj_bias, int proj_Cout, void* proj_out, void* stream) {
  TTSK_REQUIRE(proj_w_packed && proj_out, "ttsk_win_ln_proj_fwd: null pointer");
  return win_ln_launch(A, lda, W_packed, bias, res, gamma, beta, out, z_save, mean, rstd, lens, seg_len, M, K, D, eps, p_pre, site_pre, rng,
                       proj_w_packed, proj_bias, proj_Cout, proj_out, stream);
}
```

tts_king_amd/csrc/layernorm.hip:

```cpp
#include "common.h"
#include "proj32.h"

namespace {

constexpr int MAXJ = 4;

struct LnArgs {
  const bf16_t* y;
  const bf16_t* res;
  const float* gamma;
  const float* beta;
  bf16_t* out;
  bf16_t* z_save;
  float* mean;
  float* rstd;
  const long long* lens;
  const uint64_t* rng;
  const float* head_w;
  const float* head_b;
  float* head_out;
  int rows, D, seg_len;
  float p_pre, p_post, eps;
  unsigned site_pre, site_post;
  int group_rows;
  long long pstride;
  unsigned site_stride;
};

__device__ __forceinline__ void load4(const bf16_t* p, float v[4]) {
  const uint2 u = *(const uint2*)p;
  v[0] = __uint_as_float(u.x << 16); v[1] = __uint_as_float(u.x & 0xFFFF0000u);
  v[2] = __uint_as_float(u.y << 16); v[3] = __uint_as_float(u.y & 0xFFFF0000u);
}
__device__ __forceinline__ void store4(bf16_t* p, const float v[4]) {
  *(uint2*)p = make_uint2(pack_bf2(v[0], v[1]), pack_bf2(v[2], v[3]));
}
__device__ __forceinline__ void drop4(float v[4], uint64_t seed, uint64_t step, unsigned site, unsigned e4, unsigned thr, float scale) {
  const uint4 b = Philox::gen(make_uint2((unsigned)seed, (unsigned)(seed >> 32)),
                              make_uint4(e4, site, (unsigned)step, (unsigned)(step >> 32)));
  v[0] = b.x >= thr ? v[0] * scale : 0.f;
  v[1] = b.y >= thr ? v[1] * scale : 0.f;
  v[2] = b.z >= thr ? v[2] * scale : 0.f;
  v[3] = b.w >= thr ? v[3] * scale : 0.f;
}

__global__ __launch_bounds__(256) void ln_fwd_kernel(const LnArgs a) {
  const int lane = threadIdx.x & 63;
  const int row = blockIdx.x * 4 + (threadIdx.x >> 6);
  if (row >= a.rows) return;
  const int D = a.D, nj = D >> 8;
  const uint64_t seed = a.rng ? a.rng[0] : 0, step = a.rng ? a.rng[1] : 0;
  const int grp = a.group_rows > 0 ? row / a.group_rows : 0;
  const int lrow = row - grp * a.group_rows;
  const float* gamma = a.gamma + grp * a.pstride;
  const float* beta = a.beta + grp * a.pstride;
  const unsigned site_pre = a.site_pre + grp * a.site_stride, site_post = a.site_post + grp * a.site_stride;
  float z[MAXJ][4];
  float s = 0.f;
#pragma unroll
  for (int j = 0; j < MAXJ; ++j) {
    if (j < nj) {
      const int c = j * 256 + lane * 4;
      load4(a.y + (int64_t)row * D + c, z[j]);
      if (a.p_pre > 0.f)
        drop4(z[j], seed, step, site_pre, (unsigned)(((int64_t)lrow * D + c) >> 2), keep_threshold(a.p_pre), 1.f / (1.f - a.p_pre));
      if (a.res) {
        float r[4];
        load4(a.res + (int64_t)row * D + c, r);
#pragma unroll
        for (int e = 0; e < 4; ++e) z[j][e] += r[e];
      }
      if (a.z_save) {
        store4(a.z_save + (int64_t)row * D + c, z[j]);
      }
      s += z[j][0] + z[j][1] + z[j][2] + z[j][3];
    }
  }
  const float mean = wave_sum(s) / D;
  float q = 0.f;
#pragma unroll
  for (int j = 0; j < MAXJ; ++j)
    if (j < nj)
#pragma unroll
      for (int e = 0; e < 4; ++e) { const float d = z[j][e] - mean; q += d * d; }
  const float rstd = rsqrtf(wave_sum(q) / D + a.eps);
  if (lane == 0) { a.mean[row] = mean; a.rstd[row] = rstd; }
  bool masked = false;
  if (a.lens) { const int b = lrow / a.seg_len, t = lrow - b * a.seg_len; masked = t >= a.lens[b]; }
  float hs = 0.f;
#pragma unroll
  for (int j = 0; j < MAXJ; ++j) {
    if (j < nj) {
      const int c = j * 256 + lane * 4;
      const f32x4 g = *(const f32x4*)(gamma + c), bt = *(const f32x4*)(beta + c);
      float o[4];
#pragma unroll
      for (int e = 0; e < 4; ++e) o[e] = (z[j][e] - mean) * rstd * g[e] + bt[e];
      if (a.p_post > 0.f)
        drop4(o, seed, step, site_post, (unsigned)(((int64_t)lrow * D + c) >> 2), keep_threshold(a.p_post), 1.f / (1.f - a.p_post));
      if (masked) o[0] = o[1] = o[2] = o[3] = 0.f;
      if (a.out) store4(a.out + (int64_t)row * D + c, o);
      if (a.head_w) {
        const f32x4 w = *(const f32x4*)(a.head_w + grp * a.pstride + c);
        hs += o[0] * w[0] + o[1] * w[1] + o[2] * w[2] + o[3] * w[3];
      }
    }
  }
  if (a.head_w) {
    hs = wave_sum(hs);
    if (lane == 0) a.head_out[row] = masked ? 0.f : hs + a.head_b[grp * a.pstride];
  }
}

struct LnBwdArgs {
  const bf16_t* dout;
  const float* dhead;
  const float* head_w;
  const bf16_t* z;
  const float* mean;
  const float* rstd;
  const float* gamma;
  const float* beta;
  const long long* lens;
  const uint64_t* rng;
  bf16_t* dz;
  bf16_t* dy;
  float* partials;
  int rows, D, seg_len, relu_in;
  float p_pre, p_post;
  unsigned site_pre, site_post;
  int group_rows, nblk_group;
  long long pstride;
  unsigned site_stride;
  const float* slabs;
  const bf16_t* R;
  long long slab_stride;
  int nsplit;
};

constexpr int LNB_WAVES = 8;
template <int MJ>
__global__ __launch_bounds__(LNB_WAVES * 64) void ln_bwd_kernel(const LnBwdArgs a) {
  __shared__ float red[LNB_WAVES][MJ * 256];
  __shared__ float redb[LNB_WAVES];
  const int lane = threadIdx.x & 63, wave = threadIdx.x >> 6;
  const int D = a.D, nj = D >> 8;
  const uint64_t seed = a.rng ? a.rng[0] : 0, step = a.rng ? a.rng[1] : 0;
  const bool head = a.dhead != nullptr;
  float dg[MJ][4], db[MJ][4], dbias[MJ][4], dhw[MJ][4];
  float dhb = 0.f;
#pragma unroll
  for (int j = 0; j < MJ; ++j)
#pragma unroll
    for (int e = 0; e < 4; ++e) dg[j][e] = db[j][e] = dbias[j][e] = dhw[j][e] = 0.f;

  const int grp = a.group_rows > 0 ? blockIdx.x / a.nblk_group : 0;
  const int lblk = blockIdx.x - grp * a.nblk_group;
  const int grows = a.group_rows > 0 ? a.group_rows : a.rows;
  const float* gamma = a.gamma + grp * a.pstride;
  const float* beta = a.beta ? a.beta + grp * a.pstride : nullptr;
  const float* head_w = a.head_w ? a.head_w + grp * a.pstride : nullptr;
  const unsigned site_pre = a.site_pre + grp * a.site_stride, site_post = a.site_post + grp * a.site_stride;
  struct RowIn { uint2 z[MJ]; f32x4 d[MJ]; float mean, rstd, dh; bool masked; };
  auto fetch = [&](int lr, RowIn& r) __attribute__((always_inline)) {
    const int rw = grp * grows + lr;
    r.masked = false;
    if (a.lens) { const int b = lr / a.seg_len, t = lr - b * a.seg_len; r.masked = t >= a.lens[b]; }
    r.mean = a.mean[rw]; r.rstd = a.rstd[rw];
    r.dh = head ? (r.masked ? 0.f : a.dhead[rw]) : 0.f;
#pragma unroll
    for (int j = 0; j < MJ; ++j)
      if (j < nj) {
        const int c = j * 256 + lane * 4;
        r.z[j] = *(const uint2*)(a.z + (int64_t)rw * D + c);
        f32x4 d = {0.f, 0.f, 0.f, 0.f};
        if (!r.masked) {
          if (a.slabs) {
            const float* sp = a.slabs + (int64_t)rw * D + c;
            for (int q = 0; q < a.nsplit; ++q) d += *(const f32x4*)(sp + q * a.slab_stride);
            if (a.R) {
              const uint2 u = *(const uint2*)(a.R + (int64_t)rw * D + c);
              d += f32x4{__uint_as_float(u.x << 16), __uint_as_float(u.x & 0xFFFF0000u), __uint_as_float(u.y << 16), __uint_as_float(u.y & 0xFFFF0000u)};
            }
          } else if (a.dout) {
            const uint2 u = *(const uint2*)(a.dout + (int64_t)rw * D + c);
            d = f32x4{__uint_as_float(u.x << 16), __uint_as_float(u.x & 0xFFFF0000u), __uint_as_float(u.y << 16), __uint_as_float(u.y & 0xFFFF0000u)};
          }
        }
        r.d[j] = d;
      }
  };
  const int rstride = a.nblk_group * LNB_WAVES;
  RowIn cur;
  if (lblk * LNB_WAVES + wave < grows) fetch(lblk * LNB_WAVES + wave, cur);
  for (int lrow = lblk * LNB_WAVES + wave; lrow < grows; lrow += rstride) {
    const int row = grp * grows + lrow;
    RowIn nxt;
    const bool more = lrow + rstride < grows;
    if (more) fetch(lrow + rstride, nxt);
    const bool masked = cur.masked;
    const float mean = cur.mean, rstd = cur.rstd, dh = cur.dh;
    float xh[MJ][4], g[MJ][4];
    float c1 = 0.f, c2 = 0.f;
    unsigned closed = 0;
#pragma unroll
    for (int j = 0; j < MJ; ++j) {
      if (j < nj) {
        const int c = j * 256 + lane * 4;
        const float zz[4] = {__uint_as_float(cur.z[j].x << 16), __uint_as_float(cur.z[j].x & 0xFFFF0000u),
                             __uint_as_float(cur.z[j].y << 16), __uint_as_float(cur.z[j].y & 0xFFFF0000u)};
        float d[4] = {cur.d[j][0], cur.d[j][1], cur.d[j][2], cur.d[j][3]};
        const f32x4 gm = *(const f32x4*)(gamma + c);
#pragma unroll
        for (int e = 0; e < 4; ++e) xh[j][e] = (zz[e] - mean) * rstd;
        if (head) {
          const f32x4 w = *(const f32x4*)(head_w + c), bt = *(const f32x4*)(beta + c);
          float o[4];
#pragma unroll
          for (int e = 0; e < 4; ++e) { o[e] = xh[j][e] * gm[e] + bt[e]; d[e] += dh * w[e]; }
          if (a.p_post > 0.f)
            drop4(o, seed, step, site_post, (unsigned)(((int64_t)lrow * D + c) >> 2), keep_threshold(a.p_post), 1.f / (1.f - a.p_post));
#pragma unroll
          for (int e = 0; e < 4; ++e) dhw[j][e] += dh * o[e];
        }
        if (a.p_post > 0.f)
          drop4(d, seed, step, site_post, (unsigned)(((int64_t)lrow * D + c) >> 2), keep_threshold(a.p_post), 1.f / (1.f - a.p_post));
#pragma unroll
        for (int e = 0; e < 4; ++e) {
          dg[j][e] += d[e] * xh[j][e];
          db[j][e] += d[e];
          g[j][e] = d[e] * gm[e];
          c1 += g[j][e];
          c2 += g[j][e] * xh[j][e];
        }
        if (a.relu_in) {
#pragma unroll
          for (int e = 0; e < 4; ++e) if (!(zz[e] > 0.f)) closed |= 1u << (j * 4 + e);
        }
      }
    }
    if (lane == 0) dhb += dh;
    c1 = wave_sum(c1) / D;
    c2 = wave_sum(c2) / D;
#pragma unroll
    for (int j = 0; j < MJ; ++j) {
      if (j < nj) {
        const int c = j * 256 + lane * 4;
        float dzv[4];
#pragma unroll
        for (int e = 0; e < 4; ++e) {
          dzv[e] = ((closed >> (j * 4 + e)) & 1u) ? 0.f : rstd * (g[j][e] - c1 - xh[j][e] * c2);
        }
        if (a.dz) store4(a.dz + (int64_t)row * D + c, dzv);
        if (a.p_pre > 0.f) {
          drop4(dzv, seed, step, site_pre, (unsigned)(((int64_t)lrow * D + c) >> 2), keep_threshold(a.p_pre), 1.f / (1.f - a.p_pre));
          if (a.dy) store4(a.dy + (int64_t)row * D + c, dzv);
        }
#pragma unroll
        for (int e = 0; e < 4; ++e) dbias[j][e] += dzv[e];
      }
    }
    if (more) cur = nxt;
  }
  const int nq = head ? 4 : 3;
  float* P = a.partials + (int64_t)blockIdx.x * (nq * D + (head ? 1 : 0));
  for (int qn = 0; qn < nq; ++qn) {
#pragma unroll
    for (int j = 0; j < MJ; ++j)
      if (j < nj)
#pragma unroll
        for (int e = 0; e < 4; ++e) {
          const float v = qn == 0 ? dbias[j][e] : qn == 1 ? dg[j][e] : qn == 2 ? db[j][e] : dhw[j][e];
          red[wave][j * 256 + lane * 4 + e] = v;
        }
    __syncthreads();
    for (int c = threadIdx.x; c < D; c += LNB_WAVES * 64) {
      float t = 0.f;
#pragma unroll
      for (int w = 0; w < LNB_WAVES; ++w) t += red[w][c];
      P[qn * D + c] = t;
    }
    __syncthreads();
  }
  if (head) {
    dhb = wave_sum(dhb);
    if (lane == 0) redb[wave] = dhb;
    __syncthreads();
    if (threadIdx.x == 0) {
      float t = 0.f;
#pragma unroll
      for (int w = 0; w < LNB_WAVES; ++w) t += redb[w];
      P[nq * D] = t;
    }
  }
}

__device__ __forceinline__ void unpack8(uint4 u, float* v) {
  v[0] = __uint_as_float(u.x << 16); v[1] = __uint_as_float(u.x & 0xFFFF0000u);
  v[2] = __uint_as_float(u.y << 16); v[3] = __uint_as_float(u.y & 0xFFFF0000u);
  v[4] = __uint_as_float(u.z << 16); v[5] = __uint_as_float(u.z & 0xFFFF0000u);
  v[6] = __uint_as_float(u.w << 16); v[7] = __uint_as_float(u.w & 0xFFFF0000u);
}
__device__ __forceinline__ uint4 pack8f(const float* v) {
  return make_uint4(pack_bf2(v[0], v[1]), pack_bf2(v[2], v[3]), pack_bf2(v[4], v[5]), pack_bf2(v[6], v[7]));
}
__device__ __forceinline__ float group16_sum(float v) { return quad16_sum(v); }

__device__ __forceinline__ void lnb256_row(const LnBwdArgs& a, int row, int c0, const float gam[16], uint64_t seed, uint64_t step,
                                           unsigned thr, float dscale, float sbias[16], float sgam[16], float sbeta[16], float dzv[16],
                                           const float* dl = nullptr ) {
  constexpr int D = 256;
  const bool live = row < a.rows;
  bool masked = !live;
  if (live && a.lens) { const int b = row / a.seg_len, t = row - b * a.seg_len; masked = t >= a.lens[b]; }
  float zz[16], d[16];
#pragma unroll
  for (int e = 0; e < 16; ++e) { zz[e] = 0.f; d[e] = 0.f; }
  float mean = 0.f, rstd = 0.f;
  if (live) {
    const bf16_t* zp = a.z + (int64_t)row * D + c0;
    unpack8(*(const uint4*)zp, zz); unpack8(*(const uint4*)(zp + 8), zz + 8);
    mean = a.mean[row]; rstd = a.rstd[row];
    if (!masked) {
      if (dl || a.slabs) {
        if (dl) {
#pragma unroll
          for (int i = 0; i < 4; ++i) {
            const f32x4 t = *(const f32x4*)(dl + c0 + 4 * i);
            d[4 * i] = t[0]; d[4 * i + 1] = t[1]; d[4 * i + 2] = t[2]; d[4 * i + 3] = t[3];
          }
        } else {
          const float* sp = a.slabs + (int64_t)row * D + c0;
          for (int q = 0; q < a.nsplit; ++q) {
#pragma unroll
            for (int i = 0; i < 4; ++i) {
              const f32x4 t = *(const f32x4*)(sp + q * a.slab_stride + 4 * i);
              d[4 * i] += t[0]; d[4 * i + 1] += t[1]; d[4 * i + 2] += t[2]; d[4 * i + 3] += t[3];
            }
          }
        }
        if (a.R) {
          float r[16];
          const bf16_t* rp = a.R + (int64_t)row * D + c0;
          unpack8(*(const uint4*)rp, r); unpack8(*(const uint4*)(rp + 8), r + 8);
#pragma unroll
          for (int e = 0; e < 16; ++e) d[e] += r[e];
        }
      } else {
        const bf16_t* dp = a.dout + (int64_t)row * D + c0;
        unpack8(*(const uint4*)dp, d); unpack8(*(const uint4*)(dp + 8), d + 8);
      }
    }
  }
  float xh[16], g[16];
  float c1 = 0.f, c2 = 0.f;
#pragma unroll
  for (int e = 0; e < 16; ++e) {
    xh[e] = __fmul_rn(__fsub_rn(zz[e], mean), rstd);
    g[e] = __fmul_rn(d[e], gam[e]);
    c1 = __fadd_rn(c1, g[e]); c2 = __fmaf_rn(g[e], xh[e], c2);
    sgam[e] = __fmaf_rn(d[e], xh[e], sgam[e]);
    sbeta[e] = __fadd_rn(sbeta[e], d[e]);
  }
  c1 = __fmul_rn(group16_sum(c1), 1.f / D);
  c2 = __fmul_rn(group16_sum(c2), 1.f / D);
#pragma unroll
  for (int e = 0; e < 16; ++e) dzv[e] = __fmul_rn(rstd, __fmaf_rn(-xh[e], c2, __fsub_rn(g[e], c1)));
  if (live && a.dz) {
    bf16_t* op = a.dz + (int64_t)row * D + c0;
    *(uint4*)op = pack8f(dzv); *(uint4*)(op + 8) = pack8f(dzv + 8);
  }
  if (a.p_pre > 0.f) {
#pragma unroll
    for (int i = 0; i < 4; ++i) drop4(dzv + 4 * i, seed, step, a.site_pre, (unsigned)(((int64_t)row * D + c0 + 4 * i) >> 2), thr, dscale);
    if (live && a.dy) {
      bf16_t* op = a.dy + (int64_t)row * D + c0;
      *(uint4*)op = pack8f(dzv); *(uint4*)(op + 8) = pack8f(dzv + 8);
    }
  }
  if (live) {
#pragma unroll
    for (int e = 0; e < 16; ++e) sbias[e] += dzv[e];
  }
}

__device__ __forceinline__ float rows4_sum(float v) {
  const unsigned u = __float_as_uint(v);
  const auto r = __builtin_amdgcn_permlane16_swap(u, u, false, false);
  const unsigned w = __float_as_uint(__uint_as_float(r[0]) + __uint_as_float(r[1]));
  const auto q = __builtin_amdgcn_permlane32_swap(w, w, false, false);
  return __uint_as_float(q[0]) + __uint_as_float(q[1]);
}

constexpr int LNB_RED_LD = 16 * 17, LNB_RED = 3 * LNB_RED_LD;
__device__ __forceinline__ void lnb256_partials(const LnBwdArgs& a, float sbias[16], float sgam[16], float sbeta[16], float (*red)[LNB_RED],
                                                int wave, int grp, int c0, int pblock = -1, bool write = true) {
  constexpr int D = 256;
#pragma unroll
  for (int e = 0; e < 16; ++e) { sbias[e] = rows4_sum(sbias[e]); sgam[e] = rows4_sum(sgam[e]); sbeta[e] = rows4_sum(sbeta[e]); }
  const int l = c0 >> 4;
#pragma unroll
  for (int g = 0; g < 4; ++g) {
    if (grp == g) {
#pragma unroll
      for (int j = 0; j < 4; ++j) {
        const int e = 4 * g + j;
        red[wave][e * 17 + l] = sbias[e]; red[wave][LNB_RED_LD + e * 17 + l] = sgam[e]; red[wave][2 * LNB_RED_LD + e * 17 + l] = sbeta[e];
      }
    }
  }
  __syncthreads();
  if (!write) return;
  float* P = a.partials + (int64_t)(pblock < 0 ? (int)blockIdx.x : pblock) * 3 * D;
  for (int c = threadIdx.x; c < 3 * D; c += LNB_WAVES * 64) {
    const int pos = (c >> 8) * LNB_RED_LD + (c & 15) * 17 + ((c & 255) >> 4);
    float t = 0.f;
#pragma unroll
    for (int w = 0; w < LNB_WAVES; ++w) t += red[w][pos];
    P[c] = t;
  }
}

__global__ __launch_bounds__(LNB_WAVES * 64) void ln_bwd256_kernel(const LnBwdArgs a) {
  constexpr int D = 256;
  __shared__ float red[LNB_WAVES][LNB_RED];
  const int lane = threadIdx.x & 63, wave = threadIdx.x >> 6;
  const int grp = lane >> 4, l = lane & 15, c0 = l * 16;
  const uint64_t seed = a.rng ? a.rng[0] : 0, step = a.rng ? a.rng[1] : 0;
  const unsigned thr = keep_threshold(a.p_pre);
  const float dscale = a.p_pre > 0.f ? 1.f / (1.f - a.p_pre) : 1.f;
  float gam[16];
#pragma unroll
  for (int i = 0; i < 4; ++i) { const f32x4 t = *(const f32x4*)(a.gamma + c0 + 4 * i); gam[4 * i] = t[0]; gam[4 * i + 1] = t[1]; gam[4 * i + 2] = t[2]; gam[4 * i + 3] = t[3]; }
  float sbias[16], sgam[16], sbeta[16];
#pragma unroll
  for (int e = 0; e < 16; ++e) sbias[e] = sgam[e] = sbeta[e] = 0.f;
  const int rows_per_sweep = gridDim.x * LNB_WAVES * 4;
  for (int row = (blockIdx.x * LNB_WAVES + wave) * 4 + grp; row < a.rows + 3; row += rows_per_sweep) {
    float dzv[16];
    lnb256_row(a, row, c0, gam, seed, step, thr, dscale, sbias, sgam, sbeta, dzv);
  }
  lnb256_partials(a, sbias, sgam, sbeta, red, wave, grp, c0);
}

constexpr int PRE_K = 768, PRE_RS = PRE_K * 2 + 32, PRE_DT_LD = 260;
__device__ __forceinline__ void pre768_gemm(const bf16_t* __restrict__ pre_x, const bf16_t* __restrict__ pre_w, int m0, int rows,
                                            unsigned char* as, float* dtile) {
  constexpr int D = 256, PK = PRE_K, PRS = PRE_RS, DT_LD = PRE_DT_LD;
  constexpr int KH = P32_KH, CT = P32_CT, NS = PK / 128, NF = P32_TT / 16, CH8 = PK / 8;
  const int tid = threadIdx.x, lane = tid & 63, wave = tid >> 6;
  const int l15 = lane & 15, q = lane >> 4;
  const bf16_t* wrow[CT];
#pragma unroll
  for (int cc = 0; cc < CT; ++cc) wrow[cc] = pre_w + ((int64_t)(wave * CT + cc) * 64 + lane) * 8;
  constexpr int64_t kstep_stride = (D / 16) * 512;
  constexpr int NCH = P32_TT * CH8 / P32_NT;
  uint4 xv[NCH];
#pragma unroll
  for (int it = 0; it < NCH; ++it) {
    const int idx = it * P32_NT + tid, row = idx / CH8, ch = idx - row * CH8;
    xv[it] = make_uint4(0, 0, 0, 0);
    if (m0 + row < rows) xv[it] = *(const uint4*)(pre_x + (int64_t)(m0 + row) * PK + ch * 8);
  }
  bf16x8 wv[NS][KH][CT];
#pragma unroll
  for (int g = 0; g < NS; ++g)
#pragma unroll
    for (int ks = 0; ks < KH; ++ks)
#pragma unroll
      for (int cc = 0; cc < CT; ++cc) wv[g][ks][cc] = *(const bf16x8*)(wrow[cc] + (int64_t)(g * KH + ks) * kstep_stride);
#pragma unroll
  for (int it = 0; it < NCH; ++it) {
    const int idx = it * P32_NT + tid, row = idx / CH8, ch = idx - row * CH8;
    *(uint4*)(as + row * PRS + ch * 16) = xv[it];
  }
  __syncthreads();
  f32x4 acc[CT][NF];
#pragma unroll
  for (int cc = 0; cc < CT; ++cc)
#pragma unroll
    for (int i = 0; i < NF; ++i) acc[cc][i] = f32x4{0.f, 0.f, 0.f, 0.f};
  const unsigned char* inl = as + l15 * PRS + q * 16;
  {
    FragStream<NS * KH * NF, 4, 1, CT> bs;
    auto frag = [&](int i) __attribute__((always_inline)) { return *(const bf16x8*)(inl + (i % NF) * 16 * PRS + (i / NF) * 64); };
    bs.prime(frag);
    bs.run(frag, [&](int i, bf16x8 Bf) __attribute__((always_inline)) {
      const int nf = i % NF, ks = (i / NF) % KH, g = i / (NF * KH);
#pragma unroll
      for (int cc = 0; cc < CT; ++cc) acc[cc][nf] = __builtin_amdgcn_mfma_f32_16x16x32_bf16(wv[g][ks][cc], Bf, acc[cc][nf], 0, 0, 0);
    });
  }
#pragma unroll
  for (int i = 0; i < NF; ++i)
#pragma unroll
    for (int cc = 0; cc < CT; ++cc) *(f32x4*)(dtile + (i * 16 + l15) * DT_LD + (wave * CT + cc) * 16 + q * 4) = acc[cc][i];
  __syncthreads();
}

__global__ __launch_bounds__(LNB_WAVES * 64, 1) void pre768_kernel(const bf16_t* __restrict__ x, const bf16_t* __restrict__ w,
                                                                   const bf16_t* __restrict__ R, bf16_t* __restrict__ out, int rows) {
  __shared__ __attribute__((aligned(16))) unsigned char as[P32_TT * PRE_RS];
  __shared__ __attribute__((aligned(16))) float dtile[P32_TT * PRE_DT_LD];
  const int m0 = blockIdx.x * P32_TT;
  pre768_gemm(x, w, m0, rows, as, dtile);
  const int rl = threadIdx.x >> 4, c0 = (threadIdx.x & 15) * 16, row = m0 + rl;
  if (row >= rows) return;
  float v[16];
#pragma unroll
  for (int i = 0; i < 4; ++i) {
    const f32x4 t = *(const f32x4*)(dtile + rl * PRE_DT_LD + c0 + 4 * i);
    v[4 * i] = t[0]; v[4 * i + 1] = t[1]; v[4 * i + 2] = t[2]; v[4 * i + 3] = t[3];
  }
  if (R) {
    float r[16];
    const bf16_t* rp = R + (int64_t)row * 256 + c0;
    unpack8(*(const uint4*)rp, r); unpack8(*(const uint4*)(rp + 8), r + 8);
#pragma unroll
    for (int e = 0; e < 16; ++e) v[e] += r[e];
  }
  bf16_t* op = out + (int64_t)row * 256 + c0;
  *(uint4*)op = pack8f(v); *(uint4*)(op + 8) = pack8f(v + 8);
}

struct LnbProjArgs {
  LnBwdArgs ln;
  const bf16_t* w;
  bf16_t* out;
  const bf16_t* gate;
  const float* o32;
  float* delta;
  int Cout;
  const bf16_t* pre_x;
  const bf16_t* pre_w;
#ifdef TTSK_STAMPS
  unsigned long long* stamps;
#endif
};
#ifdef TTSK_STAMPS
#define LNB_STAMP(i)                                                                                   \
  do {                                                                                                 \
    if (SPLIT == 1 && p.stamps && threadIdx.x == 0) p.stamps[(int64_t)blockIdx.x * 8 + (i)] = __builtin_amdgcn_s_memrealtime();  \
  } while (0)
#else
#define LNB_STAMP(i) do {} while (0)
#endif

constexpr int LNB_SPLIT_MAX_TILES = 63, LNB_SPLIT = 2;
template <int NG, bool PRE, int SPLIT = 1>
__global__ __launch_bounds__(LNB_WAVES * 64, 1) void ln_bwd256_proj_kernel(const LnbProjArgs p) {
  constexpr int D = 256;
  static_assert(LNB_WAVES * 64 == P32_NT && P32_D == D, "proj32.h is built for 8 waves and 256 channels");
  constexpr int PRS = PRE_RS, DT_LD = PRE_DT_LD;
  constexpr int MAIN_BYTES = LNB_WAVES * LNB_RED * 4 + 2 * P32_TT * P32_RS;
  constexpr int PRE_BYTES = P32_TT * PRS;
  __shared__ __attribute__((aligned(16))) unsigned char smem[(PRE && PRE_BYTES > MAIN_BYTES) ? PRE_BYTES : MAIN_BYTES];
  __shared__ __attribute__((aligned(16))) float dtile[PRE ? P32_TT * DT_LD : 4];
  float (*red)[LNB_RED] = (float (*)[LNB_RED])smem;
  unsigned char* xs = smem + LNB_WAVES * LNB_RED * 4;
  unsigned char* os = xs + P32_TT * P32_RS;
  static_assert(NG % SPLIT == 0, "whole groups per workgroup");
  const int part = (int)blockIdx.x % SPLIT, tile = (int)blockIdx.x / SPLIT;
  LnBwdArgs a = p.ln;
  if (SPLIT > 1 && part != 0) a.dz = a.dy = nullptr;
  const int tid = threadIdx.x, lane = tid & 63, wave = tid >> 6;
  const int grp = lane >> 4, l = lane & 15, c0 = l * 16;
  const int m0 = tile * P32_TT;
  Proj32W W;
  LNB_STAMP(0);
  if (PRE) pre768_gemm(p.pre_x, p.pre_w, m0, a.rows, smem, dtile);
  LNB_STAMP(1);
  {
    const uint64_t seed = a.rng ? a.rng[0] : 0, step = a.rng ? a.rng[1] : 0;
    const unsigned thr = keep_threshold(a.p_pre);
    const float dscale = a.p_pre > 0.f ? 1.f / (1.f - a.p_pre) : 1.f;
    float gam[16];
#pragma unroll
    for (int i = 0; i < 4; ++i) { const f32x4 t = *(const f32x4*)(a.gamma + c0 + 4 * i); gam[4 * i] = t[0]; gam[4 * i + 1] = t[1]; gam[4 * i + 2] = t[2]; gam[4 * i + 3] = t[3]; }
    float sbias[16], sgam[16], sbeta[16], dzv[16];
#pragma unroll
    for (int e = 0; e < 16; ++e) sbias[e] = sgam[e] = sbeta[e] = 0.f;
    const int rl = wave * 4 + grp;
    lnb256_row(a, m0 + rl, c0, gam, seed, step, thr, dscale, sbias, sgam, sbeta, dzv, PRE ? dtile + rl * DT_LD : nullptr);
    {
      const uint4 lo = pack8f(dzv), hi = pack8f(dzv + 8);
      const int up = (l >> 2) & 1;
      unsigned char* dst = xs + rl * P32_RS + c0 * 2;
      *(uint4*)(dst + up * 16) = up ? hi : lo;
      *(uint4*)(dst + (up ^ 1) * 16) = up ? lo : hi;
    }
    LNB_STAMP(2);
    proj32_prefetch(p.w, p.Cout, wave, lane, W, part * (NG / SPLIT));
    lnb256_partials(a, sbias, sgam, sbeta, red, wave, grp, c0, tile, part == 0);
    LNB_STAMP(3);
  }
  uint4 gpre[2] = {make_uint4(0, 0, 0, 0), make_uint4(0, 0, 0, 0)};
  f32x4 ypre[2][2];
#pragma unroll
  for (int it = 0; it < 2; ++it) { ypre[it][0] = f32x4{0.f, 0.f, 0.f, 0.f}; ypre[it][1] = f32x4{0.f, 0.f, 0.f, 0.f}; }
  auto pre = [&](int cg) __attribute__((always_inline)) {
    if (NG == 1 && p.delta) {
#pragma unroll
      for (int it = 0; it < 2; ++it) {
        const int idx = it * P32_NT + tid, rr = idx >> 5, ch = idx & 31;
        if (m0 + rr < a.rows) {
          const float* op = p.o32 + (int64_t)(m0 + rr) * D + ch * 8;
          ypre[it][0] = *(const f32x4*)op; ypre[it][1] = *(const f32x4*)(op + 4);
        }
      }
    }
    if (p.gate) {
#pragma unroll
      for (int it = 0; it < 2; ++it) {
        const int idx = it * P32_NT + tid, rr = idx >> 5, ch = idx & 31;
        if (m0 + rr < a.rows) gpre[it] = *(const uint4*)(p.gate + (int64_t)(m0 + rr) * p.Cout + cg * D + ch * 8);
      }
    }
  };
  proj32_run<NG / SPLIT>(xs, os, p.w, p.Cout, nullptr, W, tid, [&](int cg, int rr, int ch, uint4 v, int it) __attribute__((always_inline)) {
    const int row = m0 + rr;
    float dacc = 0.f;
    if (row < a.rows) {
      if (p.gate) {
        const uint4 gt = gpre[it];
        auto keep = [](unsigned w) {
          const unsigned lo = w & 0xFFFFu, hi = w >> 16;
          return ((lo - 1u) < 0x7FFFu ? 0xFFFFu : 0u) | ((hi - 1u) < 0x7FFFu ? 0xFFFF0000u : 0u);
        };
        v.x &= keep(gt.x); v.y &= keep(gt.y); v.z &= keep(gt.z); v.w &= keep(gt.w);
      }
      *(uint4*)(p.out + (int64_t)row * p.Cout + cg * D + ch * 8) = v;
      if (NG == 1 && p.delta) {
        const f32x4 y0 = ypre[it][0], y1 = ypre[it][1];
        dacc = __uint_as_float(v.x << 16) * y0[0] + __uint_as_float(v.x & 0xFFFF0000u) * y0[1] + __uint_as_float(v.y << 16) * y0[2] +
               __uint_as_float(v.y & 0xFFFF0000u) * y0[3] + __uint_as_float(v.z << 16) * y1[0] + __uint_as_float(v.z & 0xFFFF0000u) * y1[1] +
               __uint_as_float(v.w << 16) * y1[2] + __uint_as_float(v.w & 0xFFFF0000u) * y1[3];
      }
    }
    if (NG == 1 && p.delta) {
      dacc = quad16_sum(dacc);
      if (row < a.rows && (ch & 15) == 0) {
        const int b = row / a.seg_len, t = row - b * a.seg_len;
        p.delta[((int64_t)b * 2 + (ch >> 4)) * a.seg_len + t] = dacc;
      }
    }
  }, pre, part * (NG / SPLIT));
  LNB_STAMP(4);
}

__global__ __launch_bounds__(256) void colsum_finalize_kernel(const float* __restrict__ partials, int nblk, int ncols,
                                                              int ld, float* __restrict__ dst, int accumulate, float scale) {
  __shared__ float red[16][17];
  const int cx = threadIdx.x & 15, gy = threadIdx.x >> 4;
  const int c = blockIdx.x * 16 + cx;
  float s0 = 0.f, s1 = 0.f, s2 = 0.f, s3 = 0.f;
  if (c < ncols) {
    int b = gy;
    for (; b + 48 < nblk; b += 64) {
      s0 += partials[(int64_t)b * ld + c];
      s1 += partials[(int64_t)(b + 16) * ld + c];
      s2 += partials[(int64_t)(b + 32) * ld + c];
      s3 += partials[(int64_t)(b + 48) * ld + c];
    }
    for (; b < nblk; b += 16) s0 += partials[(int64_t)b * ld + c];
  }
  red[gy][cx] = (s0 + s1) + (s2 + s3);
  __syncthreads();
  if (gy == 0 && c < ncols) {
    float t = 0.f;
#pragma unroll
    for (int k = 0; k < 16; ++k) t += red[k][cx];
    t *= scale;
    dst[c] = accumulate ? dst[c] + t : t;
  }
}

struct FinalizeBatch {
  ttsk_finalize_item it[64];
};
__global__ __launch_bounds__(256) void colsum_finalize_batch_kernel(const FinalizeBatch fb) {
  __shared__ float red[16][17];
  const ttsk_finalize_item& it = fb.it[blockIdx.y];
  const int cx = threadIdx.x & 15, gy = threadIdx.x >> 4;
  for (int c0 = blockIdx.x * 16; c0 < it.ncols; c0 += gridDim.x * 16) {
    const int c = c0 + cx;
    float s0 = 0.f, s1 = 0.f, s2 = 0.f, s3 = 0.f;
    if (c < it.ncols) {
      int b = gy;
      for (; b + 48 < it.nblk; b += 64) {
        s0 += it.partials[(int64_t)b * it.ld + c];
        s1 += it.partials[(int64_t)(b + 16) * it.ld + c];
        s2 += it.partials[(int64_t)(b + 32) * it.ld + c];
        s3 += it.partials[(int64_t)(b + 48) * it.ld + c];
      }
      for (; b < it.nblk; b += 16) s0 += it.partials[(int64_t)b * it.ld + c];
    }
    red[gy][cx] = (s0 + s1) + (s2 + s3);
    __syncthreads();
    if (gy == 0 && c < it.ncols) {
      float t = 0.f;
#pragma unroll
      for (int k = 0; k < 16; ++k) t += red[k][cx];
      t *= it.scale;
      it.dst[c] = it.accumulate ? it.dst[c] + t : t;
    }
    __syncthreads();
  }
}

__device__ __forceinline__ int colsum_vec(int C, int ld, const void* x, bool f32) {
  return (!f32 && (C & 7) == 0 && (ld & 7) == 0 && (((uintptr_t)x) & 15) == 0) ? 8 : 4;
}
template <typename T>
__device__ __forceinline__ void colsum_body(const T* __restrict__ x, int rows, int C, int ld, float* __restrict__ partials, int blk, int nblk,
                                            float* red) {
  const int V = colsum_vec(C, ld, x, sizeof(T) == 4);
  const int tpr = (C + V - 1) / V;
  const int rpi = 256 / tpr;
  const int r0 = threadIdx.x / tpr, c0 = (threadIdx.x % tpr) * V;
  const int per = (rows + nblk - 1) / nblk;
  const int rb = blk * per;
  const int re = min(rb + per, rows);
  float s[8] = {0.f, 0.f, 0.f, 0.f, 0.f, 0.f, 0.f, 0.f};
  if (r0 < rpi) {
    if constexpr (sizeof(T) == 2) {
      if (V == 8) {
        auto add = [&](const uint4 u) __attribute__((always_inline)) {
          s[0] += __uint_as_float(u.x << 16); s[1] += __uint_as_float(u.x & 0xFFFF0000u);
          s[2] += __uint_as_float(u.y << 16); s[3] += __uint_as_float(u.y & 0xFFFF0000u);
          s[4] += __uint_as_float(u.z << 16); s[5] += __uint_as_float(u.z & 0xFFFF0000u);
          s[6] += __uint_as_float(u.w << 16); s[7] += __uint_as_float(u.w & 0xFFFF0000u);
        };
        typedef __attribute__((ext_vector_type(4))) unsigned u32x4_;
        const bf16_t* xp = (const bf16_t*)x + c0;
        int r = rb + r0;
        for (; r + 3 * rpi < re; r += 4 * rpi) {
          const u32x4_ a0 = __builtin_nontemporal_load((const u32x4_*)(xp + (int64_t)r * ld));
          const u32x4_ a1 = __builtin_nontemporal_load((const u32x4_*)(xp + (int64_t)(r + rpi) * ld));
          const u32x4_ a2 = __builtin_nontemporal_load((const u32x4_*)(xp + (int64_t)(r + 2 * rpi) * ld));
          const u32x4_ a3 = __builtin_nontemporal_load((const u32x4_*)(xp + (int64_t)(r + 3 * rpi) * ld));
          add(make_uint4(a0[0], a0[1], a0[2], a0[3])); add(make_uint4(a1[0], a1[1], a1[2], a1[3]));
          add(make_uint4(a2[0], a2[1], a2[2], a2[3])); add(make_uint4(a3[0], a3[1], a3[2], a3[3]));
        }
        for (; r < re; r += rpi) {
          const u32x4_ a0 = __builtin_nontemporal_load((const u32x4_*)(xp + (int64_t)r * ld));
          add(make_uint4(a0[0], a0[1], a0[2], a0[3]));
        }
      } else {
        for (int r = rb + r0; r < re; r += rpi) {
          const uint2 u = *(const uint2*)((const bf16_t*)x + (int64_t)r * ld + c0);
          s[0] += __uint_as_float(u.x << 16); s[1] += __uint_as_float(u.x & 0xFFFF0000u);
          s[2] += __uint_as_float(u.y << 16); s[3] += __uint_as_float(u.y & 0xFFFF0000u);
        }
      }
    } else {
      const float* xp = (const float*)x + c0;
      int r = rb + r0;
      for (; r + 3 * rpi < re; r += 4 * rpi) {
        const f32x4 a0 = __builtin_nontemporal_load((const f32x4*)(xp + (int64_t)r * ld));
        const f32x4 a1 = __builtin_nontemporal_load((const f32x4*)(xp + (int64_t)(r + rpi) * ld));
        const f32x4 a2 = __builtin_nontemporal_load((const f32x4*)(xp + (int64_t)(r + 2 * rpi) * ld));
        const f32x4 a3 = __builtin_nontemporal_load((const f32x4*)(xp + (int64_t)(r + 3 * rpi) * ld));
#pragma unroll
        for (int e = 0; e < 4; ++e) { s[e] += a0[e]; s[e] += a1[e]; s[e] += a2[e]; s[e] += a3[e]; }
      }
      for (; r < re; r += rpi) {
        const f32x4 u = __builtin_nontemporal_load((const f32x4*)(xp + (int64_t)r * ld));
#pragma unroll
        for (int e = 0; e < 4; ++e) s[e] += u[e];
      }
    }
    for (int e = 0; e < V; ++e) red[r0 * C + c0 + e] = s[e];
  }
  __syncthreads();
  for (int c = threadIdx.x; c < C; c += 256) {
    float t = 0.f;
    for (int k = 0; k < rpi; ++k) t += red[k * C + c];
    partials[(int64_t)blk * C + c] = t;
  }
}

template <typename T>
__global__ __launch_bounds__(256) void colsum_kernel(const T* __restrict__ x, int rows, int C, int ld, float* __restrict__ partials) {
  extern __shared__ float red[];
  colsum_body<T>(x, rows, C, ld, partials, blockIdx.x, gridDim.x, red);
}

struct ColsumBatch {
  ttsk_colsum_item it[64];
};
__global__ __launch_bounds__(256) void colsum_batch_kernel(const ColsumBatch cb) {
  extern __shared__ float red[];
  const ttsk_colsum_item& it = cb.it[blockIdx.y];
  if ((int)blockIdx.x >= it.nblk) return;
  if (it.is_f32) colsum_body<float>((const float*)it.x, it.rows, it.C, it.ld, it.partials, blockIdx.x, it.nblk, red);
  else colsum_body<bf16_t>((const bf16_t*)it.x, it.rows, it.C, it.ld, it.partials, blockIdx.x, it.nblk, red);
}

}

extern "C" int ttsk_layernorm_fwd(const void* y, const void* res, const float* gamma, const float* beta, void* out,
                                  void* z_save, float* mean, float* rstd, const int64_t* lens, int seg_len, int rows, int D,
                                  float eps, float p_pre, uint32_t site_pre, float p_post, uint32_t site_post,
                                  const uint64_t* rng, const float* head_w, const float* head_b, float* head_out,
                                  void* stream) {
  TTSK_REQUIRE(y && gamma && beta && mean && rstd, "layernorm_fwd: null pointer");
  TTSK_REQUIRE(rows > 0 && D >= 256 && D <= 1024 && (D & 255) == 0, "layernorm_fwd: D must be 256..1024 step 256 (got %d)", D);
  TTSK_REQUIRE(!lens || seg_len > 0, "layernorm_fwd: lens needs seg_len");
  TTSK_REQUIRE((p_pre == 0.f && p_post == 0.f) || rng, "layernorm_fwd: dropout needs rng state");
  TTSK_REQUIRE(!head_w || (head_b && head_out), "layernorm_fwd: head needs bias and output");
  LnArgs a{(const bf16_t*)y, (const bf16_t*)res, gamma, beta, (bf16_t*)out, (bf16_t*)z_save, mean, rstd,
           (const long long*)lens, rng, head_w, head_b, head_out, rows, D, seg_len, p_pre, p_post, eps, site_pre, site_post, 0, 0, 0};
  hipLaunchKernelGGL(ln_fwd_kernel, dim3((rows + 3) / 4), dim3(256), 0, (hipStream_t)stream, a);
  TTSK_CHECK_LAUNCH();
  return TTSK_OK;
}

extern "C" int ttsk_layernorm_fwd_grouped(const void* y, const void* res, const float* gamma, const float* beta, void* out,
                                          void* z_save, float* mean, float* rstd, const int64_t* lens, int seg_len, int groups,
                                          int group_rows, int64_t param_stride, uint32_t site_stride, int D, float eps, float p_pre,
                                          uint32_t site_pre, float p_post, uint32_t site_post, const uint64_t* rng,
                                          const float* head_w, const float* head_b, float* head_out, void* stream) {
  TTSK_REQUIRE(y && gamma && beta && mean && rstd, "layernorm_fwd_grouped: null pointer");
  TTSK_REQUIRE(groups > 0 && group_rows > 0 && D >= 256 && D <= 1024 && (D & 255) == 0, "layernorm_fwd_grouped: bad sizes");
  TTSK_REQUIRE(!lens || (seg_len > 0 && group_rows % seg_len == 0), "layernorm_fwd_grouped: lens needs group_rows %% seg_len == 0");
  TTSK_REQUIRE((p_pre == 0.f && p_post == 0.f) || rng, "layernorm_fwd_grouped: dropout needs rng state");
  TTSK_REQUIRE(!head_w || (head_b && head_out), "layernorm_fwd_grouped: head needs bias and output");
  TTSK_REQUIRE((param_stride & 3) == 0, "layernorm_fwd_grouped: param_stride must keep 16-byte alignment");
  const int rows = groups * group_rows;
  LnArgs a{(const bf16_t*)y, (const bf16_t*)res, gamma, beta, (bf16_t*)out, (bf16_t*)z_save, mean, rstd,
           (const long long*)lens, rng, head_w, head_b, head_out, rows, D, seg_len, p_pre, p_post, eps, site_pre, site_post,
           group_rows, (long long)param_stride, site_stride};
  hipLaunchKernelGGL(ln_fwd_kernel, dim3((rows + 3) / 4), dim3(256), 0, (hipStream_t)stream, a);
  TTSK_CHECK_LAUNCH();
  return TTSK_OK;
}

extern "C" int ttsk_layernorm_bwd_nblocks(int rows) {
  int n = (rows + LNB_WAVES - 1) / LNB_WAVES;
  return n > 256 ? 256 : n;
}

extern "C" int ttsk_layernorm_bwd(const void* dout, const float* dhead, const float* head_w, const void* z,
                                  const float* mean, const float* rstd, const float* gamma, const float* beta,
                                  const int64_t* lens, int seg_len, int rows, int D, int relu_in, float p_pre,
                                  uint32_t site_pre, float p_post, uint32_t site_post, const uint64_t* rng, void* dz, void* dy,
                                  float* partials, void* stream) {
  TTSK_REQUIRE(z && mean && rstd && gamma && partials, "layernorm_bwd: null pointer");
  TTSK_REQUIRE(dout || dhead, "layernorm_bwd: need dout or dhead");
  TTSK_REQUIRE(!dhead || (head_w && beta), "layernorm_bwd: head mode needs head_w and beta");
  TTSK_REQUIRE(rows > 0 && D >= 256 && D <= 1024 && (D & 255) == 0, "layernorm_bwd: bad D %d", D);
  TTSK_REQUIRE((p_pre == 0.f && p_post == 0.f) || rng, "layernorm_bwd: dropout needs rng state");
  TTSK_REQUIRE(p_post == 0.f || beta, "layernorm_bwd: post dropout needs beta");
  const int nblk = ttsk_layernorm_bwd_nblocks(rows);
  LnBwdArgs a{(const bf16_t*)dout, dhead, head_w, (const bf16_t*)z, mean, rstd, gamma, beta, (const long long*)lens, rng,
              (bf16_t*)dz, (bf16_t*)dy, partials, rows, D, seg_len, relu_in, p_pre, p_post, site_pre, site_post, 0, nblk, 0, 0, nullptr, nullptr, 0, 0};
  if (D == 256 && !dhead && !relu_in && p_post == 0.f && dout)
    hipLaunchKernelGGL(ln_bwd256_kernel, dim3(nblk), dim3(LNB_WAVES * 64), 0, (hipStream_t)stream, a);
  else if (a.D <= 256)
    hipLaunchKernelGGL(ln_bwd_kernel<1>, dim3(nblk), dim3(LNB_WAVES * 64), 0, (hipStream_t)stream, a);
  else
    hipLaunchKernelGGL(ln_bwd_kernel<MAXJ>, dim3(nblk), dim3(LNB_WAVES * 64), 0, (hipStream_t)stream, a);
  TTSK_CHECK_LAUNCH();
  return TTSK_OK;
}

extern "C" int ttsk_layernorm_bwd_grouped(const void* dout, const float* dhead, const float* head_w, const void* z,
                                          const float* mean, const float* rstd, const float* gamma, const float* beta,
                                          const int64_t* lens, int seg_len, int groups, int group_rows, int64_t param_stride,
                                          uint32_t site_stride, int D, int relu_in, float p_pre, uint32_t site_pre, float p_post,
                                          uint32_t site_post, const uint64_t* rng, void* dz, void* dy, float* partials, void* stream) {
  TTSK_REQUIRE(z && mean && rstd && gamma && partials, "layernorm_bwd_grouped: null pointer");
  TTSK_REQUIRE(dout || dhead, "layernorm_bwd_grouped: need dout or dhead");
  TTSK_REQUIRE(!dhead || (head_w && beta), "layernorm_bwd_grouped: head mode needs head_w and beta");
  TTSK_REQUIRE(groups > 0 && group_rows > 0 && D >= 256 && D <= 1024 && (D & 255) == 0, "layernorm_bwd_grouped: bad sizes");
  TTSK_REQUIRE(!lens || (seg_len > 0 && group_rows % seg_len == 0), "layernorm_bwd_grouped: lens needs group_rows %% seg_len == 0");
// ... 165 lines not shown
```

tts_king_amd/csrc/rowops.hip:

```cpp
#include "common.h"

namespace {

constexpr int SM_MAXE = 16;

__global__ __launch_bounds__(256) void softmax_fwd_kernel(const float* __restrict__ s, bf16_t* __restrict__ p,
                                                          const long long* __restrict__ lens, int nrows, int S, int Sp,
                                                          int H) {
  const int lane = threadIdx.x & 63;
  const int row = blockIdx.x * 4 + (threadIdx.x >> 6);
  if (row >= nrows) return;
  const int z = row / S;
  const int len = lens ? (int)lens[z / H] : S;
  const float* sr = s + (int64_t)row * Sp;
  float v[SM_MAXE];
  float m = -INFINITY;
#pragma unroll
  for (int e = 0; e < SM_MAXE; ++e) {
    const int k = e * 64 + lane;
    v[e] = (k < S && k < len) ? sr[k] : -INFINITY;
    m = fmaxf(m, v[e]);
  }
  m = wave_max(m);
  float sum = 0.f;
// ... 390 lines not shown
                                                               const long long* __restrict__ lens) {
  const int64_t n = (int64_t)rows * q_per_row;
  for (int64_t i = blockIdx.x * 256 + threadIdx.x; i < n; i += (int64_t)gridDim.x * 256) {
    const int r = (int)(i / q_per_row), u = r / seg_len;
    if (r - u * seg_len >= clamp_len(lens, u, seg_len)) x[i] = make_uint4(0u, 0u, 0u, 0u);
  }
}

__global__ __launch_bounds__(256) void cast_bf16_kernel(const float* __restrict__ src, bf16_t* __restrict__ dst, int64_t n) {
  const int64_t n4 = n >> 2;
  for (int64_t i = blockIdx.x * 256 + threadIdx.x; i < n4; i += (int64_t)gridDim.x * 256) {
    const f32x4 v = *(const f32x4*)(src + i * 4);
    *(uint2*)(dst + i * 4) = make_uint2(pack_bf2(v[0], v[1]), pack_bf2(v[2], v[3]));
  }
  if (blockIdx.x == 0 && threadIdx.x < (n & 3)) dst[n4 * 4 + threadIdx.x] = f2bf(src[n4 * 4 + threadIdx.x]);
}

template <bool F16>
__global__ __launch_bounds__(256) void nct_to_ntc_kernel(const float* __restrict__ src, bf16_t* __restrict__ dst, int C, int T) {
  __shared__ float tile[32][33];
  const int b = blockIdx.z, c0 = blockIdx.y * 32, t0 = blockIdx.x * 32;
  const int tx = threadIdx.x & 31, ty = threadIdx.x >> 5;
  for (int r = ty; r < 32; r += 8) {
    const int c = c0 + r, t = t0 + tx;
    tile[r][tx] = (c < C && t < T) ? src[((int64_t)b * C + c) * T + t] : 0.f;
  }
  __syncthreads();
  for (int r = ty; r < 32; r += 8) {
    const int t = t0 + r, c = c0 + tx;
    if (t < T && c < C) dst[((int64_t)b * T + t) * C + c] = pack1<F16>(tile[tx][r]);
  }
}

__global__ __launch_bounds__(256) void to_int16_kernel(const float* __restrict__ src, short* __restrict__ dst, int64_t n, float scale) {
  for (int64_t i = blockIdx.x * 256 + threadIdx.x; i < n; i += (int64_t)gridDim.x * 256) {
    const int v = (int)(src[i] * scale);
    dst[i] = (short)v;
  }
}

__global__ __launch_bounds__(256) void zero_frames_kernel(uint4* __restrict__ x, int rows, int q_per_row, int seg_len, const int* __restrict__ frame_limit) {
  const int lim = frame_limit[0];
  const int64_t n = (int64_t)rows * q_per_row;
  for (int64_t i = blockIdx.x * 256 + threadIdx.x; i < n; i += (int64_t)gridDim.x * 256) {
    const int r = (int)(i / q_per_row);
    if (r % seg_len >= lim) x[i] = make_uint4(0u, 0u, 0u, 0u);
  }
}

__global__ __launch_bounds__(256) void add_f32_kernel(const float* __restrict__ a, const float* __restrict__ b, float sb,
                                                      float* __restrict__ o, int64_t n) {
  for (int64_t i = blockIdx.x * 256 + threadIdx.x; i < n; i += (int64_t)gridDim.x * 256) o[i] = a[i] + sb * b[i];
}

__global__ __launch_bounds__(256) void duration_round_kernel(const float* __restrict__ logd, float d_control, float* __restrict__ out, int n) {
  const int i = blockIdx.x * 256 + threadIdx.x;
  if (i < n) out[i] = fmaxf(rintf(expf(logd[i]) - 1.f) * d_control, 0.f);
}

__global__ __launch_bounds__(256) void length_mask_kernel(const long long* __restrict__ lens, unsigned char* __restrict__ mask, int B, int T) {
  const int i = blockIdx.x * 256 + threadIdx.x;
  if (i < B * T) { const int b = i / T, t = i - b * T; mask[i] = (float)t >= (float)lens[b] ? 1 : 0; }
}

}

static inline int grid_for(int64_t n, int cap = 2048) {
  int64_t b = (n + 255) / 256;
  return (int)(b > cap ? cap : (b < 1 ? 1 : b));
}

extern "C" int ttsk_softmax_fwd(const float* scores, void* probs_bf16, const int64_t* lens, int nz, int H, int S, int Sp,
                                void* stream) {
  TTSK_REQUIRE(scores && probs_bf16 && nz > 0 && H > 0, "softmax_fwd: bad arguments");
  TTSK_REQUIRE(S > 0 && S <= 1024 && Sp >= S && Sp <= 1024, "softmax_fwd: S=%d Sp=%d out of range (<=1024)", S, Sp);
  const int nrows = nz * S;
  hipLaunchKernelGGL(softmax_fwd_kernel, dim3((nrows + 3) / 4), dim3(256), 0, (hipStream_t)stream, scores,
                     (bf16_t*)probs_bf16, (const long long*)lens, nrows, S, Sp, H);
  TTSK_CHECK_LAUNCH();
  return TTSK_OK;
}

extern "C" int ttsk_softmax_bwd(const void* probs_bf16, const float* dprobs, void* dscores_bf16, int nz, int S, int Sp,
                                float alpha, void* stream) {
  TTSK_REQUIRE(probs_bf16 && dprobs && dscores_bf16 && nz > 0, "softmax_bwd: bad arguments");
  TTSK_REQUIRE(S > 0 && S <= 1024 && Sp >= S && Sp <= 1024, "softmax_bwd: S out of range");
  const int nrows = nz * S;
  hipLaunchKernelGGL(softmax_bwd_kernel, dim3((nrows + 3) / 4), dim3(256), 0, (hipStream_t)stream, (const bf16_t*)probs_bf16,
                     dprobs, (bf16_t*)dscores_bf16, nrows, S, Sp, alpha);
  TTSK_CHECK_LAUNCH();
  return TTSK_OK;
}

extern "C" int ttsk_bucketize(const float* values, const float* bins, int n_bins, float scale, int32_t* idx,
                              float* scaled_out, int n, void* stream) {
  TTSK_REQUIRE(values && bins && idx && n > 0 && n_bins > 0, "bucketize: bad arguments");
  hipLaunchKernelGGL(bucketize_kernel, dim3((n + 255) / 256), dim3(256), 0, (hipStream_t)stream, values, bins, n_bins, scale,
                     idx, scaled_out, n);
  TTSK_CHECK_LAUNCH();
  return TTSK_OK;
}

extern "C" int ttsk_gather_add(const void* in_bf16, const float* table, const void* idx, int idx_is_i64, int idx_div,
                               const float* pe, int pe_mod, void* out_bf16, int rows, int D, void* stream) {
  TTSK_REQUIRE(table && idx && out_bf16 && rows > 0 && D > 0 && (D & 3) == 0, "gather_add: bad arguments");
  TTSK_REQUIRE(idx_div > 0 && (!pe || pe_mod > 0), "gather_add: idx_div/pe_mod");
  hipLaunchKernelGGL(gather_add_kernel, dim3(grid_for((int64_t)rows * (D >> 2))), dim3(256), 0, (hipStream_t)stream,
                     (const bf16_t*)in_bf16, table, idx, idx_is_i64, idx_div, pe, pe_mod, (bf16_t*)out_bf16, rows, D);
  TTSK_CHECK_LAUNCH();
  return TTSK_OK;
}

extern "C" int ttsk_scatter_sum(const void* dx_bf16, const void* idx, int idx_is_i64, int idx_div, int n_idx, float* dtable,
                                int n_table_rows, int D, int skip_row, int accumulate, void* stream) {
  TTSK_REQUIRE(dx_bf16 && idx && dtable && n_idx > 0 && n_table_rows > 0, "scatter_sum: bad arguments");
  TTSK_REQUIRE(D > 0 && D <= 1024 && (D & 3) == 0 && idx_div > 0, "scatter_sum: D must be a multiple of 4, <= 1024");
  hipLaunchKernelGGL(scatter_sum_kernel, dim3(n_table_rows), dim3(256), 0, (hipStream_t)stream, (const bf16_t*)dx_bf16, idx,
                     idx_is_i64, idx_div, n_idx, dtable, D, skip_row, accumulate);
  TTSK_CHECK_LAUNCH();
  return TTSK_OK;
}

extern "C" int ttsk_scatter_sum_batch(const ttsk_scatter_item* items, int n, void* stream) {
  TTSK_REQUIRE(items && n > 0, "scatter_sum_batch: bad arguments");
  for (int base = 0; base < n; base += 8) {
    ScatterBatch sb;
    const int m = n - base < 8 ? n - base : 8;
    int max_rows = 1;
    for (int i = 0; i < m; ++i) {
      sb.it[i] = items[base + i];
      const ttsk_scatter_item& it = sb.it[i];
      TTSK_REQUIRE(it.dx && it.idx && it.dtable && it.n_idx > 0 && it.n_table_rows > 0 && it.D > 0 && it.D <= 1024 && (it.D & 3) == 0 && it.idx_div > 0,
                   "scatter_sum_batch: bad item %d", base + i);
      if (it.n_table_rows > max_rows) max_rows = it.n_table_rows;
    }
    hipLaunchKernelGGL(scatter_sum_batch_kernel, dim3(max_rows, m), dim3(256), 0, (hipStream_t)stream, sb);
    TTSK_CHECK_LAUNCH();
  }
  return TTSK_OK;
}

extern "C" int ttsk_cast_bf16(const float* src, void* dst_bf16, int64_t n, void* stream) {
  TTSK_REQUIRE(src && dst_bf16 && n > 0, "cast_bf16: bad arguments");
  TTSK_REQUIRE((((uintptr_t)src) & 15) == 0 && (((uintptr_t)dst_bf16) & 7) == 0, "cast_bf16: alignment");
  hipLaunchKernelGGL(cast_bf16_kernel, dim3(grid_for(n >> 2, 4096)), dim3(256), 0, (hipStream_t)stream, src, (bf16_t*)dst_bf16, n);
  TTSK_CHECK_LAUNCH();
  return TTSK_OK;
}

extern "C" int ttsk_nct_to_ntc(const float* src, void* dst16, int f16, int B, int C, int T, void* stream) {
  TTSK_REQUIRE(src && dst16 && B > 0 && C > 0 && T > 0 && B <= 65535, "nct_to_ntc: bad arguments");
  if (f16)
    hipLaunchKernelGGL(nct_to_ntc_kernel<true>, dim3((T + 31) / 32, (C + 31) / 32, B), dim3(256), 0, (hipStream_t)stream, src,
                       (bf16_t*)dst16, C, T);
  else
    hipLaunchKernelGGL(nct_to_ntc_kernel<false>, dim3((T + 31) / 32, (C + 31) / 32, B), dim3(256), 0, (hipStream_t)stream, src,
                       (bf16_t*)dst16, C, T);
  TTSK_CHECK_LAUNCH();
  return TTSK_OK;
}

extern "C" int ttsk_to_int16(const float* src, int16_t* dst, int64_t n, float scale, void* stream) {
  TTSK_REQUIRE(src && dst && n > 0, "to_int16: bad arguments");
  hipLaunchKernelGGL(to_int16_kernel, dim3(grid_for(n)), dim3(256), 0, (hipStream_t)stream, src, (short*)dst, n, scale);
  TTSK_CHECK_LAUNCH();
  return TTSK_OK;
}

extern "C" int ttsk_add_f32(const float* a, const float* b, float scale_b, float* out, int64_t n, void* stream) {
  TTSK_REQUIRE(a && b && out && n > 0, "add_f32: bad arguments");
  hipLaunchKernelGGL(add_f32_kernel, dim3(grid_for(n)), dim3(256), 0, (hipStream_t)stream, a, b, scale_b, out, n);
  TTSK_CHECK_LAUNCH();
  return TTSK_OK;
}

extern "C" int ttsk_duration_round(const float* logd, float d_control, float* out, int n, void* stream) {
  TTSK_REQUIRE(logd && out && n > 0, "duration_round: bad arguments");
  hipLaunchKernelGGL(duration_round_kernel, dim3((n + 255) / 256), dim3(256), 0, (hipStream_t)stream, logd, d_control, out, n);
  TTSK_CHECK_LAUNCH();
  return TTSK_OK;
}

extern "C" int ttsk_length_mask(const int64_t* lens, uint8_t* mask, int B, int T, void* stream) {
  TTSK_REQUIRE(lens && mask && B > 0 && T > 0, "length_mask: bad arguments");
  hipLaunchKernelGGL(length_mask_kernel, dim3((B * T + 255) / 256), dim3(256), 0, (hipStream_t)stream, (const long long*)lens, mask, B, T);
  TTSK_CHECK_LAUNCH();
  return TTSK_OK;
}

extern "C" int ttsk_va_embed(const void* x_bf16, const float* speaker_table, const int64_t* speakers, int L, const float* pitch_target,
                             const float* pitch_bins, const float* pitch_table, const float* energy_target, const float* energy_bins,
                             const float* energy_table, int n_bins_minus_1, void* x1_bf16, void* x2_bf16, void* x3_bf16, int32_t* pitch_idx,
                             int32_t* energy_idx, int rows, int D, const int64_t* row_limit, void* stream) {
  TTSK_REQUIRE(x_bf16 && speaker_table && speakers && pitch_target && pitch_bins && pitch_table && energy_target && energy_bins &&
                   energy_table && x1_bf16 && x2_bf16 && x3_bf16 && pitch_idx && energy_idx, "va_embed: null pointer");
  TTSK_REQUIRE(rows > 0 && L > 0 && rows % L == 0 && D > 0 && (D & 3) == 0 && n_bins_minus_1 > 0, "va_embed: bad sizes");
  hipLaunchKernelGGL(va_embed_kernel, dim3(grid_for((int64_t)rows * (D >> 2))), dim3(256), 0, (hipStream_t)stream, (const bf16_t*)x_bf16,
                     speaker_table, (const long long*)speakers, L, pitch_target, pitch_bins, pitch_table, energy_target, energy_bins,
                     energy_table, n_bins_minus_1, (bf16_t*)x1_bf16, (bf16_t*)x2_bf16, (bf16_t*)x3_bf16, pitch_idx, energy_idx, rows, D,
                     (const long long*)row_limit);
  TTSK_CHECK_LAUNCH();
  return TTSK_OK;
}

extern "C" int ttsk_va_combine(const void* dx3_bf16, const float* dxin, void* dx2_bf16, void* dx1_bf16, void* dx_bf16, int rows, int D,
                               int L, const int64_t* row_limit, void* stream) {
  TTSK_REQUIRE(dx3_bf16 && dxin && dx2_bf16 && dx1_bf16 && dx_bf16 && rows > 0 && D > 0 && (D & 3) == 0, "va_combine: bad arguments");
  TTSK_REQUIRE(!row_limit || (L > 0 && rows % L == 0), "va_combine: row_limit needs rows %% L == 0");
  const int64_t n4 = (int64_t)rows * D / 4;
  hipLaunchKernelGGL(va_combine_kernel, dim3(grid_for(n4)), dim3(256), 0, (hipStream_t)stream, (const bf16_t*)dx3_bf16, dxin,
                     (bf16_t*)dx2_bf16, (bf16_t*)dx1_bf16, (bf16_t*)dx_bf16, n4, (int64_t)rows * D, D / 4, L > 0 ? L : 1, (const long long*)row_limit);
  TTSK_CHECK_LAUNCH();
  return TTSK_OK;
}

extern "C" int ttsk_zero_frames_from(void* x, int elem_bytes, int rows, int C, int seg_len, const int32_t* frame_limit, void* stream) {
  TTSK_REQUIRE(x && frame_limit && rows > 0 && C > 0 && seg_len > 0 && rows % seg_len == 0, "zero_frames_from: bad arguments");
  TTSK_REQUIRE((elem_bytes == 2 || elem_bytes == 4) && ((int64_t)C * elem_bytes) % 16 == 0 && (((uintptr_t)x) & 15) == 0,
               "zero_frames_from: rows must be whole 16-byte pieces");
  const int q = C * elem_bytes / 16;
  hipLaunchKernelGGL(zero_frames_kernel, dim3(grid_for((int64_t)rows * q)), dim3(256), 0, (hipStream_t)stream, (uint4*)x, rows, q, seg_len,
                     frame_limit);
  TTSK_CHECK_LAUNCH();
  return TTSK_OK;
}

extern "C" int ttsk_gather_add_lens(const void* in_bf16, const float* table, const int64_t* idx, const int64_t* lens, int seg_len,
                                    void* out_bf16, int rows, int D, void* stream) {
  TTSK_REQUIRE(in_bf16 && table && idx && lens && out_bf16, "gather_add_lens: null pointer");
  TTSK_REQUIRE(rows > 0 && seg_len > 0 && rows % seg_len == 0 && D > 0 && (D & 3) == 0, "gather_add_lens: bad sizes");
  hipLaunchKernelGGL(gather_add_lens_kernel, dim3(grid_for((int64_t)rows * (D >> 2))), dim3(256), 0, (hipStream_t)stream,
                     (const bf16_t*)in_bf16, table, (const long long*)idx, (const long long*)lens, seg_len, (bf16_t*)out_bf16, rows, D);
  TTSK_CHECK_LAUNCH();
  return TTSK_OK;
}

extern "C" int ttsk_embed_step(const float* pred, const float* control, const float* bins, int n_bins, const float* table,
                               const void* x_bf16, const int64_t* lens, int seg_len, void* x_out_bf16, float* scaled_out,
                               int32_t* idx_out, int rows, int D, void* stream) {
  TTSK_REQUIRE(pred && control && bins && table && x_bf16 && lens && x_out_bf16 && scaled_out && idx_out, "embed_step: null pointer");
  TTSK_REQUIRE(rows > 0 && seg_len > 0 && rows % seg_len == 0 && D > 0 && (D & 3) == 0 && n_bins > 0, "embed_step: bad sizes");
  hipLaunchKernelGGL(embed_step_kernel, dim3(grid_for((int64_t)rows * (D >> 2))), dim3(256), 0, (hipStream_t)stream, pred, control, bins,
                     n_bins, table, (const bf16_t*)x_bf16, (const long long*)lens, seg_len, (bf16_t*)x_out_bf16, scaled_out, idx_out, rows, D);
  TTSK_CHECK_LAUNCH();
  return TTSK_OK;
}

extern "C" int ttsk_duration_round_dev(const float* logd, const float* d_control, int L, float* out, int n, void* stream) {
  TTSK_REQUIRE(logd && d_control && out && n > 0 && L > 0 && n % L == 0, "duration_round_dev: bad arguments");
  hipLaunchKernelGGL(duration_round_dev_kernel, dim3((n + 255) / 256), dim3(256), 0, (hipStream_t)stream, logd, d_control, L, out, n);
  TTSK_CHECK_LAUNCH();
  return TTSK_OK;
}

extern "C" int ttsk_embed_step_rows(const float* pred, const float* control, const float* value, const uint8_t* has, const float* bins,
                                    int n_bins, const float* table, const void* x_bf16, const int64_t* lens, int seg_len, void* x_out_bf16,
                                    float* scaled_out, int32_t* idx_out, int rows, int D, void* stream) {
  TTSK_REQUIRE(pred && control && value && has && bins && table && x_bf16 && lens && x_out_bf16 && scaled_out && idx_out,
               "embed_step_rows: null pointer");
  TTSK_REQUIRE(rows > 0 && seg_len > 0 && rows % seg_len == 0 && D > 0 && (D & 3) == 0 && n_bins > 0, "embed_step_rows: bad sizes");
  hipLaunchKernelGGL(embed_step_rows_kernel, dim3(grid_for((int64_t)rows * (D >> 2))), dim3(256), 0, (hipStream_t)stream, pred, control, value,
                     has, bins, n_bins, table, (const bf16_t*)x_bf16, (const long long*)lens, seg_len, (bf16_t*)x_out_bf16, scaled_out, idx_out,
                     rows, D);
  TTSK_CHECK_LAUNCH();
  return TTSK_OK;
}

extern "C" int ttsk_duration_rows(const float* logd, const float* d_control, const float* durations, const uint8_t* has, float* out, int n,
                                  void* stream) {
  TTSK_REQUIRE(logd && d_control && durations && has && out, "duration_rows: null pointer");
  TTSK_REQUIRE(n > 0, "duration_rows: n must be positive");
  hipLaunchKernelGGL(duration_rows_kernel, dim3((n + 255) / 256), dim3(256), 0, (hipStream_t)stream, logd, d_control, durations, has, out, n);
  TTSK_CHECK_LAUNCH();
  return TTSK_OK;
}

extern "C" int ttsk_duration_fit(const float* v, const uint8_t* has, const int32_t* target, const int64_t* lens, int seg_len, float* out,
                                 int B, void* stream) {
  TTSK_REQUIRE(v && has && target && lens && out, "duration_fit: null pointer");
  TTSK_REQUIRE(B > 0 && seg_len > 0 && seg_len <= FIT_MAXL, "duration_fit: B=%d seg_len=%d out of range (seg_len <= %d)", B, seg_len, FIT_MAXL);
  hipLaunchKernelGGL(duration_fit_kernel, dim3(B), dim3(256), 0, (hipStream_t)stream, v, has, (const int*)target, (const long long*)lens,
                     seg_len, out);
  TTSK_CHECK_LAUNCH();
  return TTSK_OK;
}

extern "C" int ttsk_zero_frames_lens(void* x, int elem_bytes, int rows, int C, int seg_len, const int64_t* lens, void* stream) {
  TTSK_REQUIRE(x && lens && rows > 0 && C > 0 && seg_len > 0 && rows % seg_len == 0, "zero_frames_lens: bad arguments");
  TTSK_REQUIRE((elem_bytes == 2 || elem_bytes == 4) && ((int64_t)C * elem_bytes) % 16 == 0 && (((uintptr_t)x) & 15) == 0,
               "zero_frames_lens: rows must be whole 16-byte pieces");
  const int q = C * elem_bytes / 16;
  hipLaunchKernelGGL(zero_frames_lens_kernel, dim3(grid_for((int64_t)rows * q)), dim3(256), 0, (hipStream_t)stream, (uint4*)x, rows, q, seg_len,
                     (const long long*)lens);
  TTSK_CHECK_LAUNCH();
  return TTSK_OK;
}

namespace {
__global__ __launch_bounds__(256) void dropout_keep_mask_kernel(const uint64_t* __restrict__ rng, unsigned site, int64_t n4, float p,
                                                                uint8_t* __restrict__ keep) {
  const uint64_t seed = rng[0], step = rng[1];
  const unsigned thr = keep_threshold(p);
  for (int64_t i = blockIdx.x * 256ll + threadIdx.x; i < n4; i += (int64_t)gridDim.x * 256) {
    const uint4 b = Philox::gen(make_uint2((unsigned)seed, (unsigned)(seed >> 32)), make_uint4((unsigned)i, site, (unsigned)step, (unsigned)(step >> 32)));
    *(uchar4*)(keep + i * 4) = make_uchar4(b.x >= thr, b.y >= thr, b.z >= thr, b.w >= thr);
  }
}
}

extern "C" int ttsk_dropout_keep_mask(const uint64_t* rng, uint32_t site, int64_t n, float p, uint8_t* keep, void* stream) {
  TTSK_REQUIRE(rng && keep && n > 0 && (n & 3) == 0 && p >= 0.f && p < 1.f, "dropout_keep_mask: n must be a positive multiple of 4, 0 <= p < 1");
  TTSK_REQUIRE(n / 4 <= 0xFFFFFFFFll && (((uintptr_t)keep) & 3) == 0, "dropout_keep_mask: element index exceeds the 32-bit counter word / alignment");
  hipLaunchKernelGGL(dropout_keep_mask_kernel, dim3(grid_for(n / 4)), dim3(256), 0, (hipStream_t)stream, rng, site, n / 4, p, keep);
  TTSK_CHECK_LAUNCH();
  return TTSK_OK;
}
```

Before: 2.522 million.

## Generate dropout keep masks early to overlap Philox with memory loads

```diff
diff --git a/tts_king_amd/csrc/batchnorm.hip b/tts_king_amd/csrc/batchnorm.hip
--- a/tts_king_amd/csrc/batchnorm.hip
+++ b/tts_king_amd/csrc/batchnorm.hip
@@ -39,9 +39,8 @@
     ld4((const bf16_t*)x + off, v);
   }
 }
-__device__ __forceinline__ uint4 bits4(const uint64_t* rng, unsigned site, unsigned e4) {
-  const uint64_t seed = rng[0], step = rng[1];
-  return Philox::gen(make_uint2((unsigned)seed, (unsigned)(seed >> 32)), make_uint4(e4, site, (unsigned)step, (unsigned)(step >> 32)));
+__device__ __forceinline__ unsigned bn_keep4(const uint64_t* rng, unsigned site, unsigned e4, unsigned thr) {
+  return keep4(rng[0], rng[1], site, e4, thr);
 }
 
 __global__ __launch_bounds__(256) void bn_stats_kernel(const void* __restrict__ x, int x_f32, int rows, int C, float* __restrict__ partials,
@@ -150,11 +149,7 @@
       v[e] = (v[e] - m[e]) * rs[e] * g[e] + b[e];
       if (a.use_tanh) v[e] = tanh_fast(v[e]);
     }
-    if (a.p > 0.f) {
-      const uint4 bb = bits4(a.rng, a.site, (unsigned)i);
-      v[0] = bb.x >= thr ? v[0] * scale : 0.f; v[1] = bb.y >= thr ? v[1] * scale : 0.f;
-      v[2] = bb.z >= thr ? v[2] * scale : 0.f; v[3] = bb.w >= thr ? v[3] * scale : 0.f;
-    }
+    if (a.p > 0.f) drop4(v, bn_keep4(a.rng, a.site, (unsigned)i, thr), scale);
     if (resid) {
       const f32x4 rr = *(const f32x4*)(resid + (int64_t)r * a.C + c4);
 #pragma unroll
@@ -177,15 +172,8 @@
     ld4((const bf16_t*)dout + (int64_t)r * a.C + c4, dy);
   }
   if (a.p > 0.f) {
-    if (a.keep) {
-      const unsigned kb = a.keep[i];
-#pragma unroll
-      for (int e = 0; e < 4; ++e) dy[e] = ((kb >> e) & 1u) ? dy[e] * scale : 0.f;
-    } else {
-      const uint4 bb = bits4(a.rng, a.site, (unsigned)i);
-      dy[0] = bb.x >= thr ? dy[0] * scale : 0.f; dy[1] = bb.y >= thr ? dy[1] * scale : 0.f;
-      dy[2] = bb.z >= thr ? dy[2] * scale : 0.f; dy[3] = bb.w >= thr ? dy[3] * scale : 0.f;
-    }
+    if (a.keep) drop4(dy, a.keep[i], scale);
+    else drop4(dy, bn_keep4(a.rng, a.site, (unsigned)i, thr), scale);
   }
 #pragma unroll
   for (int e = 0; e < 4; ++e) xh[e] = (v[e] - m[e]) * rs[e];
@@ -420,11 +408,9 @@
       if (a.use_tanh) v[u][e] = tanh_fast(v[u][e]);
     }
     if (a.p > 0.f) {
-      const uint4 bb = bits4(a.rng, a.site, (unsigned)i);
-      const bool k0 = bb.x >= thr, k1 = bb.y >= thr, k2 = bb.z >= thr, k3 = bb.w >= thr;
-      v[u][0] = k0 ? v[u][0] * scale : 0.f; v[u][1] = k1 ? v[u][1] * scale : 0.f;
-      v[u][2] = k2 ? v[u][2] * scale : 0.f; v[u][3] = k3 ? v[u][3] * scale : 0.f;
-      if (a.keep) a.keep[i] = (uint8_t)((int)k0 | ((int)k1 << 1) | ((int)k2 << 2) | ((int)k3 << 3));
+      const unsigned nib = bn_keep4(a.rng, a.site, (unsigned)i, thr);
+      drop4(v[u], nib, scale);
+      if (a.keep) a.keep[i] = (uint8_t)nib;
     }
     if constexpr (RESID) {
 #pragma unroll
diff --git a/tts_king_amd/csrc/common.h b/tts_king_amd/csrc/common.h
--- a/tts_king_amd/csrc/common.h
+++ b/tts_king_amd/csrc/common.h
@@ -112,21 +112,25 @@
   __device__ static __forceinline__ uint4 gen(uint2 key, uint4 ctr) {
 #pragma unroll
     for (int r = 0; r < 10; ++r) {
-      unsigned hi0 = __umulhi(0xD2511F53u, ctr.x), lo0 = 0xD2511F53u * ctr.x;
-      unsigned hi1 = __umulhi(0xCD9E8D57u, ctr.z), lo1 = 0xCD9E8D57u * ctr.z;
-      ctr = make_uint4(hi1 ^ ctr.y ^ key.x, lo1, hi0 ^ ctr.w ^ key.y, lo0);
+      const uint64_t p0 = (uint64_t)0xD2511F53u * ctr.x, p1 = (uint64_t)0xCD9E8D57u * ctr.z;
+      ctr = make_uint4((unsigned)(p1 >> 32) ^ ctr.y ^ key.x, (unsigned)p1, (unsigned)(p0 >> 32) ^ ctr.w ^ key.y, (unsigned)p0);
       key.x += 0x9E3779B9u;
       key.y += 0xBB67AE85u;
     }
     return ctr;
   }
 };
-__device__ __forceinline__ uint4 dropout_bits(uint64_t seed, unsigned site, unsigned e4) {
-  return Philox::gen(make_uint2((unsigned)seed, (unsigned)(seed >> 32)), make_uint4(e4, site, 0x5eedu, 0u));
-}
 __device__ __forceinline__ unsigned keep_threshold(float p) {
   double t = (double)p * 4294967296.0;
   return t >= 4294967295.0 ? 0xFFFFFFFFu : (unsigned)t;
+}
+__device__ __forceinline__ unsigned keep4(uint64_t seed, uint64_t step, unsigned site, unsigned e4, unsigned thr) {
+  const uint4 b = Philox::gen(make_uint2((unsigned)seed, (unsigned)(seed >> 32)), make_uint4(e4, site, (unsigned)step, (unsigned)(step >> 32)));
+  return (unsigned)(b.x >= thr) | ((unsigned)(b.y >= thr) << 1) | ((unsigned)(b.z >= thr) << 2) | ((unsigned)(b.w >= thr) << 3);
+}
+__device__ __forceinline__ void drop4(float v[4], unsigned nib, float scale) {
+#pragma unroll
+  for (int e = 0; e < 4; ++e) v[e] = ((nib >> e) & 1u) ? v[e] * scale : 0.f;
 }
 
 void ttsk_set_error(const char* fmt, ...);
diff --git a/tts_king_amd/csrc/cwt.hip b/tts_king_amd/csrc/cwt.hip
--- a/tts_king_amd/csrc/cwt.hip
+++ b/tts_king_amd/csrc/cwt.hip
@@ -15,14 +15,6 @@
 }
 __device__ __forceinline__ void store4(bf16_t* p, const float v[4]) {
   *(uint2*)p = make_uint2(pack_bf2(v[0], v[1]), pack_bf2(v[2], v[3]));
-}
-__device__ __forceinline__ void drop4(float v[4], uint64_t seed, uint64_t step, unsigned site, unsigned e4, unsigned thr, float scale) {
-  const uint4 b = Philox::gen(make_uint2((unsigned)seed, (unsigned)(seed >> 32)),
-                              make_uint4(e4, site, (unsigned)step, (unsigned)(step >> 32)));
-  v[0] = b.x >= thr ? v[0] * scale : 0.f;
-  v[1] = b.y >= thr ? v[1] * scale : 0.f;
-  v[2] = b.z >= thr ? v[2] * scale : 0.f;
-  v[3] = b.w >= thr ? v[3] * scale : 0.f;
 }
 
 struct HeadArgs {
@@ -61,7 +53,7 @@
 #pragma unroll
   for (int e = 0; e < 4; ++e) o[e] = (z[e] - mean) * rstd * g[e] + bt[e];
   if (a.p_post > 0.f)
-    drop4(o, seed, step, a.site_post, (unsigned)(((int64_t)row * D + c) >> 2), keep_threshold(a.p_post), 1.f / (1.f - a.p_post));
+    drop4(o, keep4(seed, step, a.site_post, (unsigned)(((int64_t)row * D + c) >> 2), keep_threshold(a.p_post)), 1.f / (1.f - a.p_post));
 #pragma unroll
   for (int k = 0; k < NH; ++k) {
     const f32x4 w = *(const f32x4*)(a.head_w + k * D + c);
@@ -110,8 +102,8 @@
     float xh[4], o[4], d[4] = {0, 0, 0, 0};
 #pragma unroll
     for (int e = 0; e < 4; ++e) { xh[e] = (zz[e] - mean) * rstd; o[e] = xh[e] * gm[e] + bt[e]; }
-    if (a.p_post > 0.f)
-      drop4(o, seed, step, a.site_post, (unsigned)(((int64_t)row * D + c) >> 2), keep_threshold(a.p_post), 1.f / (1.f - a.p_post));
+    const unsigned kpost = a.p_post > 0.f ? keep4(seed, step, a.site_post, (unsigned)(((int64_t)row * D + c) >> 2), keep_threshold(a.p_post)) : 0u;
+    if (a.p_post > 0.f) drop4(o, kpost, 1.f / (1.f - a.p_post));
 #pragma unroll
     for (int k = 0; k < NH; ++k) {
       const float dh = masked ? 0.f : a.dhead[(int64_t)row * NH + k];
@@ -120,8 +112,7 @@
       for (int e = 0; e < 4; ++e) { d[e] += dh * w[e]; dhw[k][e] += dh * o[e]; }
       dhb[k] += dh;
     }
-    if (a.p_post > 0.f)
-      drop4(d, seed, step, a.site_post, (unsigned)(((int64_t)row * D + c) >> 2), keep_threshold(a.p_post), 1.f / (1.f - a.p_post));
+    if (a.p_post > 0.f) drop4(d, kpost, 1.f / (1.f - a.p_post));
     float g[4], c1 = 0.f, c2 = 0.f;
 #pragma unroll
     for (int e = 0; e < 4; ++e) {
diff --git a/tts_king_amd/csrc/gemm_ln.hip b/tts_king_amd/csrc/gemm_ln.hip
--- a/tts_king_amd/csrc/gemm_ln.hip
+++ b/tts_king_amd/csrc/gemm_ln.hip
@@ -46,23 +46,41 @@
 #define WL_STAMP(i) do {} while (0)
 #endif
 
-__device__ __forceinline__ void drop4(float v[4], uint64_t seed, uint64_t step, unsigned site, unsigned e4, unsigned thr, float scale) {
-  const uint4 b = Philox::gen(make_uint2((unsigned)seed, (unsigned)(seed >> 32)),
-                              make_uint4(e4, site, (unsigned)step, (unsigned)(step >> 32)));
-  v[0] = b.x >= thr ? v[0] * scale : 0.f;
-  v[1] = b.y >= thr ? v[1] * scale : 0.f;
-  v[2] = b.z >= thr ? v[2] * scale : 0.f;
-  v[3] = b.w >= thr ? v[3] * scale : 0.f;
-}
-
+struct uint2x64 { uint64_t seed, step; };
+__device__ __forceinline__ uint2x64 ln_rng(const GemmLnArgs& a) {
+  uint2x64 r = {0, 0};
+  if (a.p_pre > 0.f) { r.seed = a.rng[0]; r.step = a.rng[1]; }
+  return r;
+}
 template <int RW>
-__device__ __forceinline__ void ln_rows_epilogue(const GemmLnArgs& a, const float* cs, int m0, int wave, int lane, const uint2 (&resv)[RW],
+__device__ __forceinline__ void ln_rows_res(const GemmLnArgs& a, int m0, int wave, int lane, uint2 (&resv)[RW]) {
+  const bf16_t* src = a.res ? a.res : (const bf16_t*)a.gamma;
+#pragma unroll
+  for (int rr = 0; rr < RW; ++rr) {
+    const int row = min(m0 + wave * RW + rr, a.M - 1);
+    resv[rr] = *(const uint2*)(src + (a.res ? (int64_t)row * BN : 0) + lane * 4);
+  }
+}
+template <int RW>
+__device__ __forceinline__ unsigned ln_rows_keep(const GemmLnArgs& a, uint2x64 rng, int m0, int wave, int lane) {
+  static_assert(RW <= 8, "one nibble per row in 32 bits");
+  unsigned kb = 0;
+  if (a.p_pre > 0.f) {
+    const uint64_t seed = rng.seed, step = rng.step;
+    const unsigned thr = keep_threshold(a.p_pre);
+#pragma unroll
+    for (int rr = 0; rr < RW; ++rr)
+      kb |= keep4(seed, step, a.site_pre, (unsigned)(((int64_t)(m0 + wave * RW + rr) * BN + lane * 4) >> 2), thr) << (4 * rr);
+  }
+  return kb;
+}
+
+template <int RW>
+__device__ __forceinline__ void ln_rows_epilogue(const GemmLnArgs& a, const float* cs, int m0, int wave, int lane, const uint2 (&resv)[RW], unsigned kb,
                                                  unsigned char* xs2 = nullptr, bool write = true ) {
   const int M = a.M, c = lane * 4;
-  const uint64_t seed = a.rng ? a.rng[0] : 0, step = a.rng ? a.rng[1] : 0;
   const f32x4 bi = *(const f32x4*)(a.bias + c);
   const f32x4 g = *(const f32x4*)(a.gamma + c), bt = *(const f32x4*)(a.beta + c);
-  const unsigned thr = keep_threshold(a.p_pre);
   const float scale = 1.f / (1.f - a.p_pre);
   float z[RW][4];
   float s[RW];
@@ -74,9 +92,10 @@
     const f32x4 v = *(const f32x4*)(cs + lr * CS_LD + c);
 #pragma unroll
     for (int e = 0; e < 4; ++e) z[rr][e] = v[e] + bi[e];
-    if (a.p_pre > 0.f) drop4(z[rr], seed, step, a.site_pre, (unsigned)(((int64_t)row * BN + c) >> 2), thr, scale);
-    z[rr][0] += __uint_as_float(resv[rr].x << 16); z[rr][1] += __uint_as_float(resv[rr].x & 0xFFFF0000u);
-    z[rr][2] += __uint_as_float(resv[rr].y << 16); z[rr][3] += __uint_as_float(resv[rr].y & 0xFFFF0000u);
+    if (a.p_pre > 0.f) drop4(z[rr], kb >> (4 * rr), scale);
+    const uint2 rv = (a.res && live) ? resv[rr] : make_uint2(0u, 0u);
+    z[rr][0] += __uint_as_float(rv.x << 16); z[rr][1] += __uint_as_float(rv.x & 0xFFFF0000u);
+    z[rr][2] += __uint_as_float(rv.y << 16); z[rr][3] += __uint_as_float(rv.y & 0xFFFF0000u);
     if (a.z_save && live && write) *(uint2*)(a.z_save + (int64_t)row * BN + c) = make_uint2(pack_bf2(z[rr][0], z[rr][1]), pack_bf2(z[rr][2], z[rr][3]));
     s[rr] = z[rr][0] + z[rr][1] + z[rr][2] + z[rr][3];
   }
@@ -121,6 +140,7 @@
   __shared__ __attribute__((aligned(16))) unsigned char smem[SMEM];
   const int tid = threadIdx.x, lane = tid & 63, wave = tid >> 6;
   const int l15 = lane & 15, lg = lane >> 4;
+  const uint2x64 rng = ln_rng(a);
   const int m0 = blockIdx.x * BM;
   const int M = a.M, K = a.K;
   const int K8 = (K + 7) & ~7;
@@ -130,11 +150,7 @@
   const int c = lane * 4;
 
   uint2 resv[RW];
-#pragma unroll
-  for (int rr = 0; rr < RW; ++rr) {
-    const int row = m0 + wave * RW + rr;
-    resv[rr] = (a.res && row < M) ? *(const uint2*)(a.res + (int64_t)row * BN + c) : make_uint2(0u, 0u);
-  }
+  ln_rows_res<RW>(a, m0, wave, lane, resv);
 
   const int prow = lane >> 3, kch = ((lane & 7) ^ (lane >> 3)) * 8;
   const int a_row = m0 + (wave & 3) * 8 + prow;
@@ -166,6 +182,9 @@
 #pragma unroll
   for (int t = 0; t < NSTAGE - 1; ++t)
     if (t < nk) issue_tile(t);
+  __builtin_amdgcn_sched_barrier(0);
+  const unsigned kb = ln_rows_keep<RW>(a, rng, m0, wave, lane);
+  __builtin_amdgcn_sched_barrier(0);
 
   for (int kt = 0; kt < nk; ++kt) {
     const int younger = nk - 1 - kt;
@@ -210,7 +229,7 @@
       for (int r = 0; r < 4; ++r) cs[(i * 16 + lg * 4 + r) * CS_LD + wave * WC + j * 16 + l15] = acc[i][j][r];
   __syncthreads();
 
-  ln_rows_epilogue<RW>(a, cs, m0, wave, lane, resv);
+  ln_rows_epilogue<RW>(a, cs, m0, wave, lane, resv, kb);
 }
 
 
@@ -226,6 +245,7 @@
   const int part = SPLIT > 1 ? (int)blockIdx.x % SPLIT : 0;
   const int m0 = (SPLIT > 1 ? (int)blockIdx.x / SPLIT : (int)blockIdx.x) * BM;
   const int M = a.M;
+  const uint2x64 rng = ln_rng(a);
   WL_STAMP(0);
   const __amdgpu_buffer_rsrc_t wres = weights_rsrc(a.W, CIN * BN * 2);
   const int wlane = (wave * CT) * 1024 + lane * 16;
@@ -233,6 +253,7 @@
   bf16x8 wa[KH][CT], wb[KH][CT], wc[KH][CT];
   auto load_w = [&](int g, bf16x8 (&w)[KH][CT]) __attribute__((always_inline)) { frags_load<KH, CT>(w, wres, wlane, g * KH * kstep_bytes, kstep_bytes); };
   uint2 resv[RW];
+  unsigned kb;
   {
     constexpr int NCH = (TT * CH8 + NT - 1) / NT;
     uint4 xv[NCH];
@@ -240,22 +261,21 @@
     for (int it = 0; it < NCH; ++it) {
       const int idx = it * NT + tid;
       const int row = idx / CH8, ch = idx - row * CH8;
-      xv[it] = make_uint4(0, 0, 0, 0);
-      if (idx < TT * CH8 && m0 + row < M) xv[it] = *(const uint4*)(a.A + (int64_t)(m0 + row) * a.lda + ch * 8);
+      static_assert((TT * CH8) % NT == 0, "every thread has a chunk in every pass");
+      xv[it] = *(const uint4*)(a.A + (int64_t)min(m0 + row, M - 1) * a.lda + ch * 8);
     }
     load_w(0, wa);
     if (1 < NS) load_w(1, wb);
     if (2 < NS) load_w(2, wc);
-#pragma unroll
-    for (int rr = 0; rr < RW; ++rr) {
-      const int row = m0 + wave * RW + rr;
-      resv[rr] = (a.res && row < M) ? *(const uint2*)(a.res + (int64_t)row * BN + lane * 4) : make_uint2(0u, 0u);
-    }
+    ln_rows_res<RW>(a, m0, wave, lane, resv);
+    __builtin_amdgcn_sched_barrier(0);
+    kb = ln_rows_keep<RW>(a, rng, m0, wave, lane);
+    __builtin_amdgcn_sched_barrier(0);
 #pragma unroll
     for (int it = 0; it < NCH; ++it) {
       const int idx = it * NT + tid;
       const int row = idx / CH8, ch = idx - row * CH8;
-      if (idx < TT * CH8) *(uint4*)(smem + row * RS + ch * 16) = xv[it];
+      *(uint4*)(smem + row * RS + ch * 16) = m0 + row < M ? xv[it] : make_uint4(0, 0, 0, 0);
     }
   }
   WL_STAMP(1);
@@ -304,7 +324,7 @@
 #pragma unroll
     for (int cc = 0; cc < CT; ++cc) *(f32x4*)(cs + (i * 16 + l15) * CS_LD + (wave * CT + cc) * 16 + q * 4) = acc[cc][i];
   __syncthreads();
-  ln_rows_epilogue<RW>(a, cs, m0, wave, lane, resv, PROJ ? ptile : nullptr, part == 0);
+  ln_rows_epilogue<RW>(a, cs, m0, wave, lane, resv, kb, PROJ ? ptile : nullptr, part == 0);
   WL_STAMP(5);
   if (PROJ) {
     __syncthreads();
diff --git a/tts_king_amd/csrc/layernorm.hip b/tts_king_amd/csrc/layernorm.hip
--- a/tts_king_amd/csrc/layernorm.hip
+++ b/tts_king_amd/csrc/layernorm.hip
@@ -35,14 +35,6 @@
 __device__ __forceinline__ void store4(bf16_t* p, const float v[4]) {
   *(uint2*)p = make_uint2(pack_bf2(v[0], v[1]), pack_bf2(v[2], v[3]));
 }
-__device__ __forceinline__ void drop4(float v[4], uint64_t seed, uint64_t step, unsigned site, unsigned e4, unsigned thr, float scale) {
-  const uint4 b = Philox::gen(make_uint2((unsigned)seed, (unsigned)(seed >> 32)),
-                              make_uint4(e4, site, (unsigned)step, (unsigned)(step >> 32)));
-  v[0] = b.x >= thr ? v[0] * scale : 0.f;
-  v[1] = b.y >= thr ? v[1] * scale : 0.f;
-  v[2] = b.z >= thr ? v[2] * scale : 0.f;
-  v[3] = b.w >= thr ? v[3] * scale : 0.f;
-}
 
 __global__ __launch_bounds__(256) void ln_fwd_kernel(const LnArgs a) {
   const int lane = threadIdx.x & 63;
@@ -63,7 +55,7 @@
       const int c = j * 256 + lane * 4;
       load4(a.y + (int64_t)row * D + c, z[j]);
       if (a.p_pre > 0.f)
-        drop4(z[j], seed, step, site_pre, (unsigned)(((int64_t)lrow * D + c) >> 2), keep_threshold(a.p_pre), 1.f / (1.f - a.p_pre));
+        drop4(z[j], keep4(seed, step, site_pre, (unsigned)(((int64_t)lrow * D + c) >> 2), keep_threshold(a.p_pre)), 1.f / (1.f - a.p_pre));
       if (a.res) {
         float r[4];
         load4(a.res + (int64_t)row * D + c, r);
@@ -97,7 +89,7 @@
 #pragma unroll
       for (int e = 0; e < 4; ++e) o[e] = (z[j][e] - mean) * rstd * g[e] + bt[e];
       if (a.p_post > 0.f)
-        drop4(o, seed, step, site_post, (unsigned)(((int64_t)lrow * D + c) >> 2), keep_threshold(a.p_post), 1.f / (1.f - a.p_post));
+        drop4(o, keep4(seed, step, site_post, (unsigned)(((int64_t)lrow * D + c) >> 2), keep_threshold(a.p_post)), 1.f / (1.f - a.p_post));
       if (masked) o[0] = o[1] = o[2] = o[3] = 0.f;
       if (a.out) store4(a.out + (int64_t)row * D + c, o);
       if (a.head_w) {
@@ -211,6 +203,7 @@
                              __uint_as_float(cur.z[j].y << 16), __uint_as_float(cur.z[j].y & 0xFFFF0000u)};
         float d[4] = {cur.d[j][0], cur.d[j][1], cur.d[j][2], cur.d[j][3]};
         const f32x4 gm = *(const f32x4*)(gamma + c);
+        const unsigned kpost = a.p_post > 0.f ? keep4(seed, step, site_post, (unsigned)(((int64_t)lrow * D + c) >> 2), keep_threshold(a.p_post)) : 0u;
 #pragma unroll
         for (int e = 0; e < 4; ++e) xh[j][e] = (zz[e] - mean) * rstd;
         if (head) {
@@ -218,13 +211,11 @@
           float o[4];
 #pragma unroll
           for (int e = 0; e < 4; ++e) { o[e] = xh[j][e] * gm[e] + bt[e]; d[e] += dh * w[e]; }
-          if (a.p_post > 0.f)
-            drop4(o, seed, step, site_post, (unsigned)(((int64_t)lrow * D + c) >> 2), keep_threshold(a.p_post), 1.f / (1.f - a.p_post));
+          if (a.p_post > 0.f) drop4(o, kpost, 1.f / (1.f - a.p_post));
 #pragma unroll
           for (int e = 0; e < 4; ++e) dhw[j][e] += dh * o[e];
         }
-        if (a.p_post > 0.f)
-          drop4(d, seed, step, site_post, (unsigned)(((int64_t)lrow * D + c) >> 2), keep_threshold(a.p_post), 1.f / (1.f - a.p_post));
+        if (a.p_post > 0.f) drop4(d, kpost, 1.f / (1.f - a.p_post));
 #pragma unroll
         for (int e = 0; e < 4; ++e) {
           dg[j][e] += d[e] * xh[j][e];
@@ -253,7 +244,7 @@
         }
         if (a.dz) store4(a.dz + (int64_t)row * D + c, dzv);
         if (a.p_pre > 0.f) {
-          drop4(dzv, seed, step, site_pre, (unsigned)(((int64_t)lrow * D + c) >> 2), keep_threshold(a.p_pre), 1.f / (1.f - a.p_pre));
+          drop4(dzv, keep4(seed, step, site_pre, (unsigned)(((int64_t)lrow * D + c) >> 2), keep_threshold(a.p_pre)), 1.f / (1.f - a.p_pre));
           if (a.dy) store4(a.dy + (int64_t)row * D + c, dzv);
         }
 #pragma unroll
@@ -304,6 +295,9 @@
 __device__ __forceinline__ uint4 pack8f(const float* v) {
   return make_uint4(pack_bf2(v[0], v[1]), pack_bf2(v[2], v[3]), pack_bf2(v[4], v[5]), pack_bf2(v[6], v[7]));
 }
+__device__ __forceinline__ void hold(uint4& v) { asm volatile("" : "+v"(v.x), "+v"(v.y), "+v"(v.z), "+v"(v.w)); }
+__device__ __forceinline__ void hold(f32x4& v) { asm volatile("" : "+v"(v)); }
+__device__ __forceinline__ void hold(float& v) { asm volatile("" : "+v"(v)); }
 __device__ __forceinline__ float group16_sum(float v) { return quad16_sum(v); }
 
 __device__ __forceinline__ void lnb256_row(const LnBwdArgs& a, int row, int c0, const float gam[16], uint64_t seed, uint64_t step,
@@ -316,40 +310,61 @@
   float zz[16], d[16];
 #pragma unroll
   for (int e = 0; e < 16; ++e) { zz[e] = 0.f; d[e] = 0.f; }
-  float mean = 0.f, rstd = 0.f;
-  if (live) {
-    const bf16_t* zp = a.z + (int64_t)row * D + c0;
-    unpack8(*(const uint4*)zp, zz); unpack8(*(const uint4*)(zp + 8), zz + 8);
-    mean = a.mean[row]; rstd = a.rstd[row];
-    if (!masked) {
-      if (dl || a.slabs) {
-        if (dl) {
+  const bool slabbed = dl || a.slabs, use = live && !masked;
+  const int64_t ro = (int64_t)(live ? row : a.rows - 1) * D + c0;
+  uint4 zr[2] = {*(const uint4*)(a.z + ro), *(const uint4*)(a.z + ro + 8)};
+  float mean = a.mean[live ? row : a.rows - 1], rstd = a.rstd[live ? row : a.rows - 1];
+  const float* sp = a.slabs ? a.slabs + ro : nullptr;
+  const bool slab0 = !dl && a.slabs && a.nsplit > 0;
+  f32x4 s0[4];
+  if (dl) {
+#pragma unroll
+    for (int i = 0; i < 4; ++i) s0[i] = *(const f32x4*)(dl + c0 + 4 * i);
+  } else {
+    const float* s0p = slab0 ? sp : a.gamma + c0;
+#pragma unroll
+    for (int i = 0; i < 4; ++i) s0[i] = *(const f32x4*)(s0p + 4 * i);
+  }
+  const bf16_t* up = slabbed ? (a.R ? a.R : a.z) : a.dout;
+  uint4 ur[2] = {*(const uint4*)(up + ro), *(const uint4*)(up + ro + 8)};
+  __builtin_amdgcn_sched_barrier(0);
+  unsigned kb = 0;
+  if (a.p_pre > 0.f) {
+#pragma unroll
+    for (int i = 0; i < 4; ++i) kb |= keep4(seed, step, a.site_pre, (unsigned)(((int64_t)row * D + c0 + 4 * i) >> 2), thr) << (4 * i);
+  }
+  __builtin_amdgcn_sched_barrier(0);
+  hold(zr[0]); hold(zr[1]); hold(mean); hold(rstd); hold(ur[0]); hold(ur[1]);
+#pragma unroll
+  for (int i = 0; i < 4; ++i) hold(s0[i]);
+  if (!live) { mean = 0.f; rstd = 0.f; }
+  if (live) { unpack8(zr[0], zz); unpack8(zr[1], zz + 8); }
+  if (use) {
+    if (slabbed) {
+      if (dl) {
+#pragma unroll
+        for (int i = 0; i < 4; ++i) { d[4 * i] = s0[i][0]; d[4 * i + 1] = s0[i][1]; d[4 * i + 2] = s0[i][2]; d[4 * i + 3] = s0[i][3]; }
+      } else {
+        if (slab0) {
+#pragma unroll
+          for (int i = 0; i < 4; ++i) { d[4 * i] += s0[i][0]; d[4 * i + 1] += s0[i][1]; d[4 * i + 2] += s0[i][2]; d[4 * i + 3] += s0[i][3]; }
+        }
+        for (int q = 1; q < a.nsplit; ++q) {
 #pragma unroll
           for (int i = 0; i < 4; ++i) {
-            const f32x4 t = *(const f32x4*)(dl + c0 + 4 * i);
-            d[4 * i] = t[0]; d[4 * i + 1] = t[1]; d[4 * i + 2] = t[2]; d[4 * i + 3] = t[3];
+            const f32x4 t = *(const f32x4*)(sp + q * a.slab_stride + 4 * i);
+            d[4 * i] += t[0]; d[4 * i + 1] += t[1]; d[4 * i + 2] += t[2]; d[4 * i + 3] += t[3];
           }
-        } else {
-          const float* sp = a.slabs + (int64_t)row * D + c0;
-          for (int q = 0; q < a.nsplit; ++q) {
-#pragma unroll
-            for (int i = 0; i < 4; ++i) {
-              const f32x4 t = *(const f32x4*)(sp + q * a.slab_stride + 4 * i);
-              d[4 * i] += t[0]; d[4 * i + 1] += t[1]; d[4 * i + 2] += t[2]; d[4 * i + 3] += t[3];
-            }
-          }
-        }
-        if (a.R) {
-          float r[16];
-          const bf16_t* rp = a.R + (int64_t)row * D + c0;
-          unpack8(*(const uint4*)rp, r); unpack8(*(const uint4*)(rp + 8), r + 8);
-#pragma unroll
-          for (int e = 0; e < 16; ++e) d[e] += r[e];
-        }
-      } else {
-        const bf16_t* dp = a.dout + (int64_t)row * D + c0;
-        unpack8(*(const uint4*)dp, d); unpack8(*(const uint4*)(dp + 8), d + 8);
-      }
+        }
+      }
+      if (a.R) {
+        float r[16];
+        unpack8(ur[0], r); unpack8(ur[1], r + 8);
+#pragma unroll
+        for (int e = 0; e < 16; ++e) d[e] += r[e];
+      }
+    } else {
+      unpack8(ur[0], d); unpack8(ur[1], d + 8);
     }
   }
   float xh[16], g[16];
@@ -372,7 +387,7 @@
   }
   if (a.p_pre > 0.f) {
 #pragma unroll
-    for (int i = 0; i < 4; ++i) drop4(dzv + 4 * i, seed, step, a.site_pre, (unsigned)(((int64_t)row * D + c0 + 4 * i) >> 2), thr, dscale);
+    for (int i = 0; i < 4; ++i) drop4(dzv + 4 * i, kb >> (4 * i), dscale);
     if (live && a.dy) {
       bf16_t* op = a.dy + (int64_t)row * D + c0;
       *(uint4*)op = pack8f(dzv); *(uint4*)(op + 8) = pack8f(dzv + 8);
@@ -567,11 +582,11 @@
   const int grp = lane >> 4, l = lane & 15, c0 = l * 16;
   const int m0 = tile * P32_TT;
   Proj32W W;
+  const uint64_t seed = a.rng ? a.rng[0] : 0, step = a.rng ? a.rng[1] : 0;
   LNB_STAMP(0);
   if (PRE) pre768_gemm(p.pre_x, p.pre_w, m0, a.rows, smem, dtile);
   LNB_STAMP(1);
   {
-    const uint64_t seed = a.rng ? a.rng[0] : 0, step = a.rng ? a.rng[1] : 0;
     const unsigned thr = keep_threshold(a.p_pre);
     const float dscale = a.p_pre > 0.f ? 1.f / (1.f - a.p_pre) : 1.f;
     float gam[16];
diff --git a/tts_king_amd/csrc/rowops.hip b/tts_king_amd/csrc/rowops.hip
--- a/tts_king_amd/csrc/rowops.hip
+++ b/tts_king_amd/csrc/rowops.hip
@@ -716,8 +716,8 @@
   const uint64_t seed = rng[0], step = rng[1];
   const unsigned thr = keep_threshold(p);
   for (int64_t i = blockIdx.x * 256ll + threadIdx.x; i < n4; i += (int64_t)gridDim.x * 256) {
-    const uint4 b = Philox::gen(make_uint2((unsigned)seed, (unsigned)(seed >> 32)), make_uint4((unsigned)i, site, (unsigned)step, (unsigned)(step >> 32)));
-    *(uchar4*)(keep + i * 4) = make_uchar4(b.x >= thr, b.y >= thr, b.z >= thr, b.w >= thr);
+    const unsigned nib = keep4(seed, step, site, (unsigned)i, thr);
+    *(uchar4*)(keep + i * 4) = make_uchar4(nib & 1u, (nib >> 1) & 1u, (nib >> 2) & 1u, (nib >> 3) & 1u);
   }
 }
 }
```

Measured after the change: 2.548 million, median of 6. 1.01x the previous value.
